# fixstars/cuda-bundle-adjustment

Measured on NVIDIA H100. Metric: LM edges/sec (10 iters), higher is better.
Workload: dtype f64

## Files before the change

### cuda-bundle-adjustment_b200/binding.py

```python
import ctypes as C
import dataclasses
import os

import numpy as np

HERE = os.path.dirname(os.path.abspath(__file__))
ROBUST_NONE, ROBUST_HUBER, ROBUST_TUKEY = 0, 1, 2
EDGE_MONOCULAR, EDGE_STEREO = 0, 1
PROFILE_ITEMS = ("0: Initialize Optimizer", "1: Build Structure", "2: Compute Error", "3: Build System",
                 "4: Schur Complement", "5: Symbolic Decomposition", "6: Numerical Decomposition", "7: Update Solution")


PCG_INFO_LEN = 16
PCG_INFO_FIELDS = ("kernel", "two_level", "aggs_per_cta", "G", "gs", "A", "maxRows", "capBlocks", "zhInSmem", "coarse_kernel",
                   "cinfo", "status", "iters", "coarse_rebuilds", "bj_retries", "bad_rebuilds")
PCG_KERNELS = ("none", "k_pcg", "k_pcg2", "k_pcg3", "k_pcg4", "k_pcg5", "k_pcg5_big", "k_pcg5t")
COARSE_KERNELS = ("none", "k_coarse_invert", "cluster2<8>", "cluster2<16>", "k_coarse_dense", "k_coarse_chol_cluster")


class CubaError(RuntimeError):
    pass


def library_path():
    return os.path.join(HERE, "libcuba_b200.so")


class _Config(C.Structure):
    _fields_ = [("device", C.c_int), ("use_fp32", C.c_int), ("pcg_max_iters", C.c_int), ("pcg_tol", C.c_double),
                ("deterministic", C.c_int), ("reserved", C.c_int * 7)]


class _Problem(C.Structure):
    _fields_ = [("Pall", C.c_int32), ("numP", C.c_int32), ("Lall", C.c_int32), ("numL", C.c_int32),
                ("q", C.c_void_p), ("t", C.c_void_p), ("cam", C.c_void_p), ("Xw", C.c_void_p),
                ("E2", C.c_int32), ("idx2", C.c_void_p), ("meas2", C.c_void_p), ("omega2", C.c_void_p),
                ("E3", C.c_int32), ("idx3", C.c_void_p), ("meas3", C.c_void_p), ("omega3", C.c_void_p)]


class _IterStat(C.Structure):
    _fields_ = [("iteration", C.c_int32), ("trials", C.c_int32), ("chi2", C.c_double), ("lambda_", C.c_double),
                ("pcg_iters", C.c_int32), ("pcg_failed", C.c_int32)]


class _Sizes(C.Structure):
    _fields_ = [(n, C.c_int32) for n in ("Pall", "numP", "Lall", "numL", "E2", "E3", "nhpl", "nblk", "nmul", "nblk_full")]


class _PoseBatch(C.Structure):
    _fields_ = [("B", C.c_int32), ("E2", C.c_int32), ("E3", C.c_int32), ("q", C.c_void_p), ("t", C.c_void_p), ("cam", C.c_void_p),
                ("ptr2", C.c_void_p), ("X2", C.c_void_p), ("meas2", C.c_void_p), ("omega2", C.c_void_p),
                ("ptr3", C.c_void_p), ("X3", C.c_void_p), ("meas3", C.c_void_p), ("omega3", C.c_void_p)]


class _PoseRound(C.Structure):
    _fields_ = [("iterations", C.c_int32), ("kernel_type", C.c_int32 * 2), ("delta", C.c_double * 2), ("restart", C.c_int32),
                ("chi2_mono", C.c_double), ("chi2_stereo", C.c_double), ("flags", C.c_int32)]


POSE_MAX_ROUNDS = 8


@dataclasses.dataclass
class PoseRound:
    iterations: int = 10
    kernel: tuple = (ROBUST_NONE, ROBUST_NONE)
    delta: tuple = (0.0, 0.0)
    restart: bool = True
    chi2_mono: float = 5.991
    chi2_stereo: float = 7.815
    depth: bool = False
    reinclude: bool = True


def orbslam2_pose_schedule():
    huber = dict(kernel=(ROBUST_HUBER, ROBUST_HUBER), delta=(5.991 ** 0.5, 7.815 ** 0.5))
    return [PoseRound(**(huber if r < 2 else {})) for r in range(4)]


class _Sim3Batch(C.Structure):
    _fields_ = [("B", C.c_int32), ("N", C.c_int32), ("ptr", C.c_void_p), ("q", C.c_void_p), ("t", C.c_void_p), ("s", C.c_void_p),
                ("cam1", C.c_void_p), ("cam2", C.c_void_p), ("fix_scale", C.c_void_p), ("X1", C.c_void_p), ("X2", C.c_void_p),
                ("obs1", C.c_void_p), ("obs2", C.c_void_p), ("omega1", C.c_void_p), ("omega2", C.c_void_p)]


class _Sim3Params(C.Structure):
    _fields_ = [("chi2", C.c_double), ("iterations", C.c_int32), ("iterations_bad", C.c_int32), ("iterations_good", C.c_int32),
                ("min_pairs", C.c_int32)]


@dataclasses.dataclass
class Sim3Params:
    chi2: float = 10.0
    iterations: int = 5
    iterations_bad: int = 10
    iterations_good: int = 5
    min_pairs: int = 10


_lib = None

_SYMBOLS = [
    "cuba_last_error", "cuba_version", "cuba_engine_create", "cuba_engine_destroy", "cuba_engine_set_robust_kernel",
    "cuba_comm_unique_id", "cuba_engine_set_comm", "cuba_engine_set_problem", "cuba_engine_set_structure_reuse", "cuba_engine_get_structure_reuses", "cuba_engine_set_state", "cuba_engine_get_sizes", "cuba_engine_reset_state", "cuba_engine_get_stream", "cuba_engine_flush_l2",
    "cuba_engine_optimize", "cuba_engine_get_state", "cuba_engine_get_chi2", "cuba_engine_set_edge_levels", "cuba_engine_get_edge_levels", "cuba_engine_classify_edges", "cuba_engine_optimize_poses", "cuba_engine_optimize_sim3", "cuba_engine_get_profile",
    "cuba_engine_get_launch_count", "cuba_get_transfer_bytes", "cuba_stage_linearize", "cuba_stage_max_diagonal", "cuba_stage_solve", "cuba_stage_update",
    "cuba_stage_commit", "cuba_stage_chi2", "cuba_debug_get_hpl_structure", "cuba_debug_get_hsc_structure",
    "cuba_debug_get_system", "cuba_debug_get_schur", "cuba_debug_get_delta", "cuba_debug_get_pcg_info", "cuba_debug_get_coarse", "cuba_debug_coarse_inverse", "cuba_debug_build_structure_host", "cuba_debug_pcg_partition", "cuba_debug_pcg5_plan", "cuba_debug_pcg5_plan_apc", "cuba_debug_dropin_problem", "cuba_debug_dropin_levels", "cuba_bench_stage",
]


def exported_symbols():
    return list(_SYMBOLS)


def load_library():
    global _lib
    if _lib is not None:
        return _lib
    path = library_path()
    if not os.path.exists(path):
        raise CubaError("%s not built: run `python -c 'import __graft_entry__ as g; g.build()'` (no CPU fallback exists)" % path)
    L = C.CDLL(path)
    L.cuba_last_error.restype = C.c_char_p
    vp, i, d = C.c_void_p, C.c_int, C.c_double
    sig = {
        "cuba_engine_create": [C.POINTER(_Config), C.POINTER(vp)],
        "cuba_engine_destroy": [vp],
        "cuba_engine_set_robust_kernel": [vp, i, i, d],
        "cuba_comm_unique_id": [vp],
        "cuba_engine_set_comm": [vp, i, i, vp],
        "cuba_engine_set_problem": [vp, C.POINTER(_Problem)],
        "cuba_engine_set_structure_reuse": [vp, i],
        "cuba_engine_get_structure_reuses": [vp, C.POINTER(C.c_longlong)],
        "cuba_engine_set_state": [vp, vp, vp, vp],
        "cuba_engine_get_sizes": [vp, C.POINTER(_Sizes)],
        "cuba_engine_reset_state": [vp],
        "cuba_engine_get_stream": [vp, C.POINTER(vp)],
        "cuba_engine_flush_l2": [vp],
        "cuba_engine_optimize": [vp, i, vp, C.POINTER(i)],
        "cuba_engine_get_state": [vp, vp, vp, vp],
        "cuba_engine_get_chi2": [vp, vp],
        "cuba_engine_set_edge_levels": [vp, vp],
        "cuba_engine_get_edge_levels": [vp, vp],
        "cuba_engine_classify_edges": [vp, d, d, i, vp],
        "cuba_engine_optimize_poses": [vp, C.POINTER(_PoseBatch), i, vp, vp, vp, vp, vp, vp, vp],
        "cuba_engine_optimize_sim3": [vp, C.POINTER(_Sim3Batch), C.POINTER(_Sim3Params), vp, vp, vp, vp, vp, vp, vp],
        "cuba_engine_get_profile": [vp, vp],
        "cuba_engine_get_launch_count": [vp, C.POINTER(C.c_longlong)],
        "cuba_get_transfer_bytes": [C.POINTER(C.c_longlong), C.POINTER(C.c_longlong)],
        "cuba_stage_linearize": [vp, C.POINTER(d)],
        "cuba_stage_max_diagonal": [vp, C.POINTER(d)],
        "cuba_stage_solve": [vp, d, C.POINTER(i), C.POINTER(i)],
        "cuba_stage_update": [vp, d, C.POINTER(d), C.POINTER(d)],
        "cuba_stage_commit": [vp, i],
        "cuba_stage_chi2": [vp, C.POINTER(d)],
        "cuba_debug_get_hpl_structure": [vp, vp, vp, vp],
        "cuba_debug_get_hsc_structure": [vp, vp, vp],
        "cuba_debug_get_system": [vp, vp, vp, vp, vp, vp],
        "cuba_debug_get_schur": [vp, vp, vp, vp],
        "cuba_debug_get_delta": [vp, vp, vp],
        "cuba_debug_get_pcg_info": [vp, vp, C.POINTER(d)],
        "cuba_debug_get_coarse": [vp, vp, vp, vp],
        "cuba_debug_coarse_inverse": [vp, vp, i, vp, vp],
        "cuba_debug_build_structure_host": [C.POINTER(_Problem), i, i, C.POINTER(_Sizes), vp, vp, vp, vp, vp, vp, vp, vp],
        "cuba_debug_pcg_partition": [C.POINTER(_Problem), i, i, vp],
        "cuba_debug_pcg5_plan": [C.POINTER(_Problem), i, i, i, vp],
        "cuba_debug_pcg5_plan_apc": [C.POINTER(_Problem), i, i, i, i, vp, C.POINTER(C.c_uint64)],
        "cuba_debug_dropin_problem": [vp, C.POINTER(_Problem)],
        "cuba_debug_dropin_levels": [vp, C.POINTER(C.POINTER(C.c_uint8)), C.POINTER(C.c_int32)],
        "cuba_bench_stage": [vp, i, i, i, d, C.POINTER(d)],
    }
    for name, args in sig.items():
        fn = getattr(L, name)
        fn.argtypes = args
        fn.restype = C.c_int
    _lib = L
    return L


def _check(rc):
    if rc != 0:
        raise CubaError("cuba error %d: %s" % (rc, load_library().cuba_last_error().decode()))


def _p(a):
    return None if a is None else a.ctypes.data_as(C.c_void_p)


def _problem_struct(prob):
    keep = [np.ascontiguousarray(prob.q, dtype=np.float64), np.ascontiguousarray(prob.t, dtype=np.float64),
            np.ascontiguousarray(prob.cam, dtype=np.float64), np.ascontiguousarray(prob.Xw, dtype=np.float64),
            np.ascontiguousarray(prob.idx2, dtype=np.int32), np.ascontiguousarray(prob.meas2, dtype=np.float64),
            np.ascontiguousarray(prob.omega2, dtype=np.float64), np.ascontiguousarray(prob.idx3, dtype=np.int32),
            np.ascontiguousarray(prob.meas3, dtype=np.float64), np.ascontiguousarray(prob.omega3, dtype=np.float64)]
    P = _Problem(prob.Pall, prob.numP, prob.Lall, prob.numL, _p(keep[0]), _p(keep[1]), _p(keep[2]), _p(keep[3]),
                 prob.E2, _p(keep[4]), _p(keep[5]), _p(keep[6]), prob.E3, _p(keep[7]), _p(keep[8]), _p(keep[9]))
    return P, keep


def transfer_bytes():
    a, b = C.c_longlong(0), C.c_longlong(0)
    _check(load_library().cuba_get_transfer_bytes(C.byref(a), C.byref(b)))
    return a.value, b.value


def build_structure_host(prob, rank=0, world=1):
    L = load_library()
    P, keep = _problem_struct(prob)
    sz = _Sizes()
    _check(L.cuba_debug_build_structure_host(C.byref(P), rank, world, C.byref(sz), None, None, None, None, None, None, None, None))
    out = {n: getattr(sz, n) for n, _ in _Sizes._fields_}
    arrs = {"hplColPtr": np.zeros(sz.numL + 1, np.int32), "hplRowInd": np.zeros(sz.nhpl, np.int32),
            "edge2Hpl": np.zeros(sz.E2 + sz.E3, np.int32), "hscRowPtr": np.zeros(sz.numP + 1, np.int32),
            "hscColInd": np.zeros(sz.nblk, np.int32), "fullRowPtr": np.zeros(sz.numP + 1, np.int32),
            "fullColInd": np.zeros(sz.nblk_full, np.int32), "shard": np.zeros(4, np.int32)}
    _check(L.cuba_debug_build_structure_host(C.byref(P), rank, world, C.byref(sz), *[_p(arrs[k]) for k in
           ("hplColPtr", "hplRowInd", "edge2Hpl", "hscRowPtr", "hscColInd", "fullRowPtr", "fullColInd", "shard")]))
    out.update(arrs)
    return out


def pcg_partition_host(prob, n_ctas=148, max_aggregates=74):
    L = load_library()
    P, keep = _problem_struct(prob)
    info = np.zeros(8, np.int32)
    _check(L.cuba_debug_pcg_partition(C.byref(P), int(n_ctas), int(max_aggregates), _p(info)))
    return dict(zip(("G", "gs", "A", "needMax", "maxRows", "blkMax", "maxNeedAgg", "coarse_list_size"), (int(v) for v in info)))


def pcg5_plan_host(prob, world=1, num_sms=148, max_aggregates=74):
    L = load_library()
    P, keep = _problem_struct(prob)
    info = np.zeros(8, np.int32)
    _check(L.cuba_debug_pcg5_plan(C.byref(P), int(world), int(num_sms), int(max_aggregates), _p(info)))
    return dict(zip(("ok", "G", "gs", "A", "needMax", "maxRows", "maxNeedAgg", "halo_rows"), (int(v) for v in info)))


def pcg5_plan_apc_host(prob, aggs_per_cta, world=1, num_sms=132, max_aggregates=148):
    L = load_library()
    P, keep = _problem_struct(prob)
    info = np.zeros(8, np.int32)
    h = C.c_uint64(0)
    _check(L.cuba_debug_pcg5_plan_apc(C.byref(P), int(world), int(num_sms), int(max_aggregates), int(aggs_per_cta), _p(info), C.byref(h)))
    out = dict(zip(("ok", "G", "gs", "A", "needMax", "maxRows", "maxNeedAgg", "halo_rows"), (int(v) for v in info)))
    out["hash"] = int(h.value)
    return out


class Engine:

    def __init__(self, device=-1, use_fp32=False, pcg_max_iters=0, pcg_tol=0.0, pcg_variant=0, structure_on_host=False, jh_variant=0, schur_variant=0,
                 coarse_refresh=0, two_level_switch=0, max_aggregates=0):
        self.L = load_library()
        res = (C.c_int * 7)()
        res[0] = int(pcg_variant)
        res[1] = int(bool(structure_on_host))
        res[2] = int(jh_variant)
        res[3] = int(schur_variant)
        res[4] = int(coarse_refresh)
        res[5] = int(two_level_switch)
        res[6] = int(max_aggregates)
        cfg = _Config(device, 2 if use_fp32 == "mixed" else int(use_fp32), int(pcg_max_iters), float(pcg_tol), 1, res)
        h = C.c_void_p()
        _check(self.L.cuba_engine_create(C.byref(cfg), C.byref(h)))
        self.h = h
        self.sizes = None
        self._stats = []

    def close(self):
        if getattr(self, "h", None):
            self.L.cuba_engine_destroy(self.h)
            self.h = None

    def __del__(self):
        try:
            self.close()
        except Exception:
            pass

    def set_robust_kernels(self, kernel_type, delta, edge_type):
        _check(self.L.cuba_engine_set_robust_kernel(self.h, int(edge_type), int(kernel_type), float(delta)))

    def set_comm(self, rank, world, unique_id=None):
        buf = None if unique_id is None else (C.c_char * 128).from_buffer_copy(bytes(unique_id))
        _check(self.L.cuba_engine_set_comm(self.h, rank, world, buf))

    @staticmethod
    def comm_unique_id():
        buf = (C.c_char * 128)()
        _check(load_library().cuba_comm_unique_id(buf))
        return bytes(buf)

    def initialize(self, prob):
        P, keep = _problem_struct(prob)
        _check(self.L.cuba_engine_set_problem(self.h, C.byref(P)))
        sz = _Sizes()
        _check(self.L.cuba_engine_get_sizes(self.h, C.byref(sz)))
        self.sizes = {n: getattr(sz, n) for n, _ in _Sizes._fields_}
        self._stats = []
        return self.sizes

    def set_structure_reuse(self, enable):
        _check(self.L.cuba_engine_set_structure_reuse(self.h, int(bool(enable))))

    def structure_reuses(self):
        n = C.c_longlong(0)
        _check(self.L.cuba_engine_get_structure_reuses(self.h, C.byref(n)))
        return n.value

    def set_state(self, q, t, Xw):
        q, t, Xw = (np.ascontiguousarray(a, dtype=np.float64) for a in (q, t, Xw))
        _check(self.L.cuba_engine_set_state(self.h, _p(q), _p(t), _p(Xw)))
# ... 58 lines not shown
    @staticmethod
    def _rounds_struct(rounds):
        rs = (_PoseRound * max(len(rounds), 1))()
        for k, r in enumerate(rounds):
            rs[k].iterations = int(r.iterations)
            rs[k].kernel_type[0], rs[k].kernel_type[1] = int(r.kernel[0]), int(r.kernel[1])
            rs[k].delta[0], rs[k].delta[1] = float(r.delta[0]), float(r.delta[1])
            rs[k].restart = int(bool(r.restart))
            rs[k].chi2_mono, rs[k].chi2_stereo = float(r.chi2_mono), float(r.chi2_stereo)
            rs[k].flags = (1 if r.depth else 0) | (2 if r.reinclude else 0)
        return rs

    def optimize_poses_flat(self, q, t, cam, ptr2, X2, meas2, omega2, ptr3, X3, meas3, omega3, rounds, B=None, E2=None, E3=None):
        f64 = lambda a, w: np.ascontiguousarray(np.asarray(a, dtype=np.float64).reshape(-1, w) if w > 1 else np.asarray(a, dtype=np.float64).reshape(-1))
        q, t, cam = f64(q, 4), f64(t, 3), f64(cam, 5)
        X2, meas2, omega2, X3, meas3, omega3 = f64(X2, 3), f64(meas2, 2), f64(omega2, 1), f64(X3, 3), f64(meas3, 3), f64(omega3, 1)
        ptr2 = np.ascontiguousarray(ptr2, dtype=np.int32); ptr3 = np.ascontiguousarray(ptr3, dtype=np.int32)
        B = len(q) if B is None else int(B)
        E2 = len(omega2) if E2 is None else int(E2)
        E3 = len(omega3) if E3 is None else int(E3)
        nb, R = max(B, 0), len(rounds)
        S = sum(max(int(r.iterations), 0) for r in rounds)
        out = dict(q=np.zeros((nb, 4)), t=np.zeros((nb, 3)), levels=np.zeros(max(E2, 0) + max(E3, 0), np.uint8),
                   counts=np.zeros((nb, R, 4), np.int32), stats=(_IterStat * max(nb * S, 1))(), nstats=np.zeros((nb, R), np.int32))
        batch = _PoseBatch(B, E2, E3, _p(q), _p(t), _p(cam), _p(ptr2), _p(X2), _p(meas2), _p(omega2), _p(ptr3), _p(X3), _p(meas3), _p(omega3))
        _check(self.L.cuba_engine_optimize_poses(self.h, C.byref(batch), R, self._rounds_struct(rounds), _p(out["q"]), _p(out["t"]),
                                                 _p(out["levels"]), _p(out["counts"]), out["stats"], _p(out["nstats"])))
        st = np.frombuffer(out["stats"], dtype=np.dtype([("iteration", "<i4"), ("trials", "<i4"), ("chi2", "<f8"), ("lambda_", "<f8"),
                                                          ("pcg_iters", "<i4"), ("pcg_failed", "<i4")]))
        out["stats"] = st[:nb * S].reshape(nb, S).copy()
        return out

    def optimize_poses(self, frames, rounds):
        n2 = np.array([len(f.omega2) for f in frames], np.int64); n3 = np.array([len(f.omega3) for f in frames], np.int64)
        ptr2 = np.concatenate([[0], np.cumsum(n2)]); ptr3 = np.concatenate([[0], np.cumsum(n3)])
        cat = lambda name, w: np.concatenate([np.asarray(getattr(f, name), np.float64).reshape(-1, w) for f in frames]) if frames else np.zeros((0, w))
        r = self.optimize_poses_flat(cat("q", 4), cat("t", 3), cat("cam", 5), ptr2, cat("X2", 3), cat("meas2", 2), cat("omega2", 1).ravel(),
                                     ptr3, cat("X3", 3), cat("meas3", 3), cat("omega3", 1).ravel(), rounds)
        off = np.concatenate([[0], np.cumsum([int(x.iterations) for x in rounds])])
        E2 = int(ptr2[-1])
        res = []
        for b in range(len(frames)):
            stats = []
            for k in range(len(rounds)):
                rows = r["stats"][b, off[k]:off[k] + r["nstats"][b, k]]
                stats.append([dict(iteration=int(s["iteration"]), trials=int(s["trials"]), chi2=float(s["chi2"]), lambda_=float(s["lambda_"]),
                                   pcg_iters=int(s["pcg_iters"]), pcg_failed=int(s["pcg_failed"])) for s in rows])
            res.append(dict(q=r["q"][b], t=r["t"][b], counts=r["counts"][b], stats=stats,
                            levels=np.concatenate([r["levels"][ptr2[b]:ptr2[b + 1]], r["levels"][E2 + ptr3[b]:E2 + ptr3[b + 1]]])))
        return res

    def optimize_sim3_flat(self, ptr, q, t, s, cam1, cam2, fix_scale, X1, X2, obs1, obs2, omega1, omega2, params=None, B=None, N=None):
        params = Sim3Params() if params is None else params
        f64 = lambda a, w: np.ascontiguousarray(np.asarray(a, dtype=np.float64).reshape(-1, w) if w > 1 else np.asarray(a, dtype=np.float64).reshape(-1))
        q, t, s, cam1, cam2 = f64(q, 4), f64(t, 3), f64(s, 1), f64(cam1, 4), f64(cam2, 4)
        X1, X2, obs1, obs2, omega1, omega2 = f64(X1, 3), f64(X2, 3), f64(obs1, 2), f64(obs2, 2), f64(omega1, 1), f64(omega2, 1)
        ptr = np.ascontiguousarray(ptr, dtype=np.int32)
        fix = None if fix_scale is None else np.ascontiguousarray(fix_scale, dtype=np.int32)
        B = len(s) if B is None else int(B)
        N = len(omega1) if N is None else int(N)
        nb = max(B, 0)
        S = max(int(params.iterations), 0) + max(int(params.iterations_bad), int(params.iterations_good), 0)
        out = dict(q=np.zeros((nb, 4)), t=np.zeros((nb, 3)), s=np.zeros(nb), levels=np.zeros(max(N, 0), np.uint8),
                   ninliers=np.zeros(nb, np.int32), stats=(_IterStat * max(nb * S, 1))(), nstats=np.zeros((nb, 2), np.int32))
        batch = _Sim3Batch(B, N, _p(ptr), _p(q), _p(t), _p(s), _p(cam1), _p(cam2), _p(fix), _p(X1), _p(X2), _p(obs1), _p(obs2),
                           _p(omega1), _p(omega2))
        prm = _Sim3Params(float(params.chi2), int(params.iterations), int(params.iterations_bad), int(params.iterations_good),
                          int(params.min_pairs))
        _check(self.L.cuba_engine_optimize_sim3(self.h, C.byref(batch), C.byref(prm), _p(out["q"]), _p(out["t"]), _p(out["s"]),
                                                _p(out["levels"]), _p(out["ninliers"]), out["stats"], _p(out["nstats"])))
        st = np.frombuffer(out["stats"], dtype=np.dtype([("iteration", "<i4"), ("trials", "<i4"), ("chi2", "<f8"), ("lambda_", "<f8"),
                                                          ("pcg_iters", "<i4"), ("pcg_failed", "<i4")]))
        out["stats"] = st[:nb * S].reshape(nb, S).copy()
        return out

    def optimize_sim3(self, problems, params=None):
        params = Sim3Params() if params is None else params
        n = np.array([len(p.omega1) for p in problems], np.int64)
        ptr = np.concatenate([[0], np.cumsum(n)])
        cat = lambda name, w: np.concatenate([np.asarray(getattr(p, name), np.float64).reshape(-1, w) for p in problems]) if problems else np.zeros((0, w))
        r = self.optimize_sim3_flat(ptr, cat("q", 4), cat("t", 3), cat("s", 1).ravel(), cat("cam1", 4), cat("cam2", 4),
                                    np.array([int(bool(p.fix_scale)) for p in problems], np.int32), cat("X1", 3), cat("X2", 3),
                                    cat("obs1", 2), cat("obs2", 2), cat("omega1", 1).ravel(), cat("omega2", 1).ravel(), params)
        off = (0, int(params.iterations))
        res = []
        for b in range(len(problems)):
            stats = []
            for k in range(2):
                rows = r["stats"][b, off[k]:off[k] + r["nstats"][b, k]]
                stats.append([dict(iteration=int(x["iteration"]), trials=int(x["trials"]), chi2=float(x["chi2"]), lambda_=float(x["lambda_"]),
                                   pcg_iters=int(x["pcg_iters"]), pcg_failed=int(x["pcg_failed"])) for x in rows])
            res.append(dict(q=r["q"][b], t=r["t"][b], s=float(r["s"][b]), levels=r["levels"][ptr[b]:ptr[b + 1]].copy(),
                            ninliers=int(r["ninliers"][b]), stats=stats))
        return res

    def launch_count(self):
        n = C.c_longlong(0)
        _check(self.L.cuba_engine_get_launch_count(self.h, C.byref(n)))
        return n.value

    def linearize(self):
        v = C.c_double(0)
        _check(self.L.cuba_stage_linearize(self.h, C.byref(v)))
        return v.value

    def max_diagonal(self):
        v = C.c_double(0)
        _check(self.L.cuba_stage_max_diagonal(self.h, C.byref(v)))
        return v.value

    def solve(self, lam):
        it, ok = C.c_int(0), C.c_int(0)
        _check(self.L.cuba_stage_solve(self.h, float(lam), C.byref(it), C.byref(ok)))
        return it.value, bool(ok.value)

    def update(self, lam):
        chi, sc = C.c_double(0), C.c_double(0)
        _check(self.L.cuba_stage_update(self.h, float(lam), C.byref(chi), C.byref(sc)))
        return chi.value, sc.value

    def commit(self, accept):
        _check(self.L.cuba_stage_commit(self.h, int(bool(accept))))

    def chi2(self):
        v = C.c_double(0)
        _check(self.L.cuba_stage_chi2(self.h, C.byref(v)))
        return v.value

    def hpl_structure(self):
        s = self.sizes
        colPtr = np.zeros(s["numL"] + 1, np.int32); rowInd = np.zeros(s["nhpl"], np.int32); e2h = np.zeros(s["E2"] + s["E3"], np.int32)
        _check(self.L.cuba_debug_get_hpl_structure(self.h, _p(colPtr), _p(rowInd), _p(e2h)))
        return colPtr, rowInd, e2h

    def hsc_structure(self):
        s = self.sizes
        rowPtr = np.zeros(s["numP"] + 1, np.int32); colInd = np.zeros(s["nblk"], np.int32)
        _check(self.L.cuba_debug_get_hsc_structure(self.h, _p(rowPtr), _p(colInd)))
        return rowPtr, colInd

    def system(self):
        s = self.sizes
        Hpp = np.zeros((s["numP"], 36)); bp = np.zeros((s["numP"], 6)); Hll = np.zeros((s["numL"], 9)); bl = np.zeros((s["numL"], 3))
        Hpl = np.zeros((s["nhpl"], 18))
        _check(self.L.cuba_debug_get_system(self.h, _p(Hpp), _p(bp), _p(Hll), _p(bl), _p(Hpl)))
        return Hpp, bp, Hll, bl, Hpl

    def schur(self):
        s = self.sizes
        Hsc = np.zeros((s["nblk"], 36)); bsc = np.zeros((s["numP"], 6)); inv = np.zeros((s["numL"], 9))
        _check(self.L.cuba_debug_get_schur(self.h, _p(Hsc), _p(bsc), _p(inv)))
        return Hsc, bsc, inv

    def delta(self):
        s = self.sizes
        xp = np.zeros((s["numP"], 6)); xl = np.zeros((s["numL"], 3))
        _check(self.L.cuba_debug_get_delta(self.h, _p(xp), _p(xl)))
        return xp, xl

    def pcg_info(self):
        info = np.zeros(PCG_INFO_LEN, np.int32)
        lam = C.c_double(0)
        _check(self.L.cuba_debug_get_pcg_info(self.h, _p(info), C.byref(lam)))
        out = dict(zip(PCG_INFO_FIELDS, (int(v) for v in info)))
        out["kernel"] = PCG_KERNELS[out["kernel"]]
        out["coarse_kernel"] = COARSE_KERNELS[out["coarse_kernel"]]
        out["two_level"] = bool(out["two_level"])
        out["coarse_lambda"] = lam.value
        return out

    def coarse(self):
        A = self.pcg_info()["A"]
        agg = np.zeros(self.sizes["numP"], np.int32); AcP = np.zeros((A * (A + 1) // 2, 36)); AcInv = np.zeros((6 * A, 6 * A), np.float32)
        _check(self.L.cuba_debug_get_coarse(self.h, _p(agg), _p(AcP), _p(AcInv)))
        return agg, AcP, AcInv

    def coarse_inverse(self, AcP):
        AcP = np.ascontiguousarray(AcP, dtype=np.float64)
        nb = AcP.shape[0]
        A = int(round(((8 * nb + 1) ** 0.5 - 1) / 2))
        assert A * (A + 1) // 2 == nb and AcP.shape[1:] == (36,), AcP.shape
        AcInv = np.zeros((6 * A, 6 * A), np.float32)
        info = C.c_int(-1)
        _check(self.L.cuba_debug_coarse_inverse(self.h, _p(AcP), A, _p(AcInv), C.byref(info)))
        return AcInv, info.value

    def bench_stage(self, stage, reps=10, flush_l2=True, lam=1.0):
        ms = C.c_double(0)
        _check(self.L.cuba_bench_stage(self.h, int(stage), int(reps), int(bool(flush_l2)), float(lam), C.byref(ms)))
        return ms.value
```

### cuda-bundle-adjustment_b200/build.py

```python
import os
import subprocess

HERE = os.path.dirname(os.path.abspath(__file__))
CSRC = os.path.join(HERE, "csrc")
LIB = os.path.join(HERE, "libcuba_b200.so")
SOURCES = ["cuba_engine.cu", "cuba_structure.cpp", "cuba_api.cpp"]
HEADERS = ["cuba_kernels.cuh", "cuba_jh4.cuh", "cuba_levels.cuh", "cuba_pose_batch.cuh", "cuba_sim3_batch.cuh", "cuba_schur3.cuh", "cuba_schur5.cuh", "cuba_pcg2.cuh", "cuba_pcg3.cuh", "cuba_pcg4.cuh", "cuba_pcg5.cuh", "cuba_pcg5t.cuh", "cuba_coarse_dense.cuh", "cuba_peer_reduce.cuh", "cuba_schur2.cuh", "cuba_structure_gpu.cuh", "cuba_math.cuh", "cuba_structure.h",
           "../../include/cuba_b200.h", "../../include/cuba_b200_levels.h", "../../include/cuba_b200_pose.h", "../../include/cuba_b200_sim3.h", "../../include/cuda_bundle_adjustment.h", "../../include/cuda_bundle_adjustment_types.h"]
NVCC = os.environ.get("NVCC", "/usr/local/cuda/bin/nvcc")
FLAGS = (["-DCUBA_JH4_DEBUG"] if os.environ.get("CUBA_JH4_DEBUG") else []) + ["-O3", "-std=c++17", "-gencode", "arch=compute_90a,code=sm_90a", "-lineinfo",
         "-Xcompiler", "-fPIC,-Wall,-Wno-unused-function", "-shared"]


def needs_build():
    if not os.path.exists(LIB):
        return True
    t = os.path.getmtime(LIB)
    deps = [os.path.join(CSRC, s) for s in SOURCES + HEADERS]
    return any(os.path.exists(d) and os.path.getmtime(d) > t for d in deps)


def build(force=False, verbose=False):
    if not force and not needs_build():
        return LIB
    srcs = [os.path.join(CSRC, s) for s in SOURCES if os.path.exists(os.path.join(CSRC, s))]
    cmd = [NVCC] + FLAGS + (["-Xptxas", "-v"] if verbose else []) + ["-I", os.path.join(HERE, "..", "include"), "-o", LIB] + srcs + ["-ldl"]
    res = subprocess.run(cmd, capture_output=True, text=True)
    if res.returncode != 0:
        raise RuntimeError("nvcc failed:\n" + res.stdout + res.stderr)
    if verbose:
        print(res.stdout + res.stderr)
    return LIB


if __name__ == "__main__":
    import sys
    print(build(force=True, verbose="-v" in sys.argv))
```

### cuda-bundle-adjustment_b200/csrc/cuba_engine.cu

```cuda
#include <cuda_runtime.h>
#include <dlfcn.h>

#include <algorithm>
#include <chrono>
#include <cmath>
#include <cstdio>
#include <cstring>
#include <memory>
#include <string>
#include <vector>

#include "../../include/cuba_b200.h"
#include "cuba_kernels.cuh"
#include "cuba_pcg2.cuh"
#include "cuba_pcg3.cuh"
#include "cuba_pcg4.cuh"
#include "cuba_pcg5.cuh"
#include "cuba_pcg5t.cuh"
#include "cuba_coarse_dense.cuh"
#include "cuba_peer_reduce.cuh"
#include "cuba_schur2.cuh"
#include "cuba_jh4.cuh"
#include "cuba_levels.cuh"
#include "cuba_pose_batch.cuh"
#include "cuba_sim3_batch.cuh"
#include "cuba_schur3.cuh"
#include "cuba_schur5.cuh"
#include "cuba_structure.h"
#include "cuba_structure_gpu.cuh"

namespace cuba_b200 {

static thread_local std::string g_err;
static int fail(int code, const std::string& msg) { g_err = msg; return code; }

#define CUDA_TRY(expr)                                                                                      \
	do {                                                                                                    \
		cudaError_t _e = (expr);                                                                            \
		if (_e != cudaSuccess) {                                                                            \
			char _b[512];                                                                                   \
			snprintf(_b, sizeof(_b), "%s:%d: %s -> %s", __FILE__, __LINE__, #expr, cudaGetErrorString(_e)); \
			return fail(CUBA_ERR_CUDA, _b);                                                                 \
		}                                                                                                   \
	} while (0)

#define KLAUNCH(kernel, n, ...)                                                             \
	do {                                                                                     \
		if ((n) > 0) {                                                                       \
			kernel<<<sgpu::grid_for(n), sgpu::BLK, 0, stream>>>(__VA_ARGS__);                 \
			launches++;                                                                      \
			CUDA_TRY(cudaGetLastError());                                                    \
		}                                                                                    \
	} while (0)

static thread_local long long g_h2dBytes = 0, g_d2hBytes = 0;

struct PinnedArena {
	char* p = nullptr; size_t cap = 0, off = 0;
	~PinnedArena() { if (p) cudaFreeHost(p); }
	void reset() { off = 0; }
	void* put(const void* src, size_t bytes)
	{
		const size_t o = (off + 255) & ~(size_t)255;
		if (o + bytes > cap) {
			if (off != 0) return nullptr;
			if (p) cudaFreeHost(p);
			cap = std::max<size_t>(2 * (o + bytes), (size_t)1 << 20);
			if (cudaMallocHost((void**)&p, cap) != cudaSuccess) { p = nullptr; cap = 0; return nullptr; }
		}
		memcpy(p + o, src, bytes);
		off = o + bytes;
		return p + o;
	}
};

struct PinnedBuf {
	char* p = nullptr; size_t cap = 0;
	PinnedBuf() {}
	PinnedBuf(const PinnedBuf&) = delete;
	PinnedBuf& operator=(const PinnedBuf&) = delete;
	~PinnedBuf() { if (p) cudaFreeHost(p); }
	cudaError_t grow(size_t bytes)
	{
		if (p && bytes <= cap) return cudaSuccess;
		if (p) cudaFreeHost(p);
		p = nullptr; cap = 0;
		const cudaError_t e = cudaMallocHost((void**)&p, std::max<size_t>(bytes, 256));
		if (e == cudaSuccess) cap = std::max<size_t>(bytes, 256);
		else p = nullptr;
		return e;
	}
};

template <typename U>
struct DBuf {
	U* p = nullptr; size_t n = 0, cap = 0;
	bool view = false;
	DBuf() {}
	DBuf(const DBuf&) = delete;
	DBuf& operator=(const DBuf&) = delete;
	~DBuf() { release(); }
	void release() { if (p && !view) cudaFree(p); p = nullptr; n = 0; cap = 0; view = false; }
	void alias(U* q, size_t count) { release(); p = q; n = count; cap = count; view = true; }
	cudaError_t alloc(size_t count)
	{
		if (p && count <= cap && !view) { n = count; return cudaSuccess; }
		release();
		n = count; cap = count ? count : 1;
		return cudaMalloc((void**)&p, sizeof(U) * cap);
	}
	cudaError_t upload(const U* h, size_t count, cudaStream_t s)
	{
		cudaError_t e = alloc(count);
		if (e != cudaSuccess || !count) return e;
		g_h2dBytes += (long long)(sizeof(U) * count);
		return cudaMemcpyAsync(p, h, sizeof(U) * count, cudaMemcpyHostToDevice, s);
	}
	cudaError_t upload(const std::vector<U>& h, cudaStream_t s) { return upload(h.data(), h.size(), s); }
	cudaError_t upload(const std::vector<U>& h, cudaStream_t s, PinnedArena& arena)
	{
		const void* src = h.empty() ? nullptr : arena.put(h.data(), sizeof(U) * h.size());
		return upload(src ? (const U*)src : h.data(), h.size(), s);
	}
	operator U*() const { return p; }
};

struct Nccl {
	void* lib = nullptr;
	typedef struct { char internal[128]; } UniqueId;
	int (*GetUniqueId)(UniqueId*) = nullptr;
	int (*CommInitRank)(void**, int, UniqueId, int) = nullptr;
	int (*CommDestroy)(void*) = nullptr;
	int (*AllReduce)(const void*, void*, size_t, int, int, void*, cudaStream_t) = nullptr;
	int (*AllGather)(const void*, void*, size_t, int, void*, cudaStream_t) = nullptr;
	int (*Broadcast)(const void*, void*, size_t, int, int, void*, cudaStream_t) = nullptr;
	int (*GroupStart)() = nullptr;
	int (*GroupEnd)() = nullptr;
	const char* (*GetErrorString)(int) = nullptr;
	bool load(std::string& why)
	{
		if (lib) return true;
		const char* names[] = { "libnccl.so.2", "libnccl.so" };
		for (const char* nme : names) { lib = dlopen(nme, RTLD_NOW | RTLD_GLOBAL); if (lib) break; }
		if (!lib) { why = std::string("dlopen libnccl.so.2 failed: ") + dlerror(); return false; }
		GetUniqueId = (int (*)(UniqueId*))dlsym(lib, "ncclGetUniqueId");
		CommInitRank = (int (*)(void**, int, UniqueId, int))dlsym(lib, "ncclCommInitRank");
		CommDestroy = (int (*)(void*))dlsym(lib, "ncclCommDestroy");
		AllReduce = (int (*)(const void*, void*, size_t, int, int, void*, cudaStream_t))dlsym(lib, "ncclAllReduce");
		AllGather = (int (*)(const void*, void*, size_t, int, void*, cudaStream_t))dlsym(lib, "ncclAllGather");
		Broadcast = (int (*)(const void*, void*, size_t, int, int, void*, cudaStream_t))dlsym(lib, "ncclBroadcast");
		GroupStart = (int (*)())dlsym(lib, "ncclGroupStart");
		GroupEnd = (int (*)())dlsym(lib, "ncclGroupEnd");
		GetErrorString = (const char* (*)(int))dlsym(lib, "ncclGetErrorString");
		if (!GetUniqueId || !CommInitRank || !CommDestroy || !AllReduce || !AllGather || !Broadcast || !GroupStart || !GroupEnd) { why = "libnccl lacks expected symbols"; return false; }
		return true;
	}
};
static Nccl g_nccl;
enum { NCCL_INT8 = 0, NCCL_FLOAT32 = 7, NCCL_FLOAT64 = 8, NCCL_SUM = 0, NCCL_MAX = 2 };

struct Scalars { double v[8]; unsigned long long maxdiag; PcgStatus pcg; };

struct DevGuard {
	int prev = -1, dev;
	explicit DevGuard(int d) : dev(d) { if (cudaGetDevice(&prev) != cudaSuccess) prev = -1; if (prev != dev) cudaSetDevice(dev); }
	~DevGuard() { if (prev >= 0 && prev != dev) cudaSetDevice(prev); }
};

struct EngineBase {
	virtual ~EngineBase() {}
	cuba_config cfg{};
	int rk_type[2] = { 0, 0 };
	double rk_delta[2] = { 0, 0 };
	int rank = 0, world = 1;
	bool structureReuse = true;
	long long structureReuses = 0;
	int devOrdinal = 0;
	void* comm = nullptr;
	bool haveProblem = false;
	long long launches = 0;
	double prof[CUBA_PROF_NUM] = { 0 };

	virtual int set_problem(const cuba_problem* p) = 0;
	virtual int set_state(const double* q, const double* t, const double* Xw) = 0;
	virtual int get_sizes(cuba_sizes* out) const = 0;
	virtual int reset_state() = 0;
	virtual int get_stream(void** s) = 0;
	virtual int flush_l2() = 0;
	virtual int optimize(int niter, cuba_iter_stat* stats, int* nstats) = 0;
	virtual int get_state(double* q, double* t, double* Xw) = 0;
	virtual int get_chi2(double* out) = 0;
	virtual int get_profile(double* sec) = 0;
	virtual int stage_linearize(double* chi) = 0;
	virtual int stage_max_diagonal(double* md) = 0;
	virtual int stage_solve(double lambda, int* iters, int* ok) = 0;
	virtual int stage_update(double lambda, double* chi, double* scale) = 0;
	virtual int stage_commit(int accept) = 0;
	virtual int stage_chi2(double* chi) = 0;
	virtual int dbg_hpl_structure(int32_t* colPtr, int32_t* rowInd, int32_t* e2h) = 0;
	virtual int dbg_hsc_structure(int32_t* rowPtr, int32_t* colInd) = 0;
	virtual int dbg_system(double* Hpp, double* bp, double* Hll, double* bl, double* Hpl) = 0;
	virtual int dbg_schur(double* Hsc, double* bsc, double* invHll) = 0;
	virtual int dbg_delta(double* xp, double* xl) = 0;
	virtual int bench_stage(int stage, int reps, int flush, double lambda, double* ms) = 0;
	virtual int dbg_pcg_timing(long long* out, int maxCtas) = 0;
	virtual int dbg_pcg_info(int32_t* info, double* coarseLambda) = 0;
	virtual int dbg_coarse(int32_t* rowAgg, double* AcP, float* AcInv) = 0;
	virtual int dbg_coarse_inverse(const double* AcP, int A, float* AcInv, int* info) = 0;
	virtual int set_edge_levels(const uint8_t* levels) = 0;
	virtual int get_edge_levels(uint8_t* levels) = 0;
	virtual int classify_edges(double chi2Mono, double chi2Stereo, int flags, int32_t* counts) = 0;
	virtual int optimize_poses(const cuba_pose_batch* bt, const pb::Schedule& s, double* qOut, double* tOut, uint8_t* levelsOut,
		int32_t* counts, cuba_iter_stat* stats, int32_t* nstats) = 0;
	virtual int optimize_sim3(const cuba_sim3_batch* bt, const s3::Params& p, double* qOut, double* tOut, double* sOut, uint8_t* levelsOut,
		int32_t* ninliers, cuba_iter_stat* stats, int32_t* nstats) = 0;
};

template <typename T>
struct Engine : EngineBase {
	Structure S;
	cudaStream_t stream = nullptr;
	int numSMs = 0;
	int ntiles = 0, nPoseBlocks = 0, nChiBlocks = 0;
	int tileSize = TILE;
	int jhMinBlocks = 2;
	bool jhV2 = true;
	bool jhV3 = true;
	int jh3Grid = 0, nChiLin = 0;
	bool jhV4 = true;
	int ntW = 0, jh4Grid = 0, jh4HasBig = 0, jh4MinB = 4, jh4Nst = 2;
	const void* jh4AttrSet = nullptr;
	int* jh4Host = nullptr;
	bool jh4Pending = false;
	DBuf<int> w_levels, w_start, w_pieces, w_base, w_tilePose, w_tilePieces, w_pieceCount, w_flag;
	DBuf<jh4::WTile> w_tile;
	DBuf<jh4::Rec> w_rec;
	DBuf<double> w_bigPartial;
	DBuf<TileInfo> tileInfo;
	bool useSchur2 = true;
	bool useSchur5 = false;
	int s5Ntiles = 0;
	DBuf<int> s5TileLm;
	DBuf<TileInfo> s5TileInfo;
	DBuf<int4> s5SegRec;
	DBuf<unsigned int> s5Off;
	int s2Nseg = 0, s2Nvalid = 0;
	DBuf<unsigned long long> s2_key, s2_keyS, s2_key3, s2_key3S;
	DBuf<int> s2_val, s2_valS, s2_head, s2_segId, s2_segStart, s2_segTile, s2_segDest, s2_val3, s2_val3S, s2_segRank, s2_rankDest, s2_tileSegPtr, s2_destSegPtr, s2_p2i, s2_p2j;
	DBuf<schur2::Counts> s2_counts;
	DBuf<T> s2_partial;
	DBuf<int> tilePose0, tilePoseN;
	int cur = 0;
	bool trialValid = false;
	DBuf<T> pose[2], Xw[2], cam, pose0, Xw0;
	DBuf<T> e_mx, e_my, e_mz, e_om, p_mx, p_my, p_mz, p_om;
	DBuf<int> tilePtr;
	DBuf<int> e_ip, e_il, e_hpl, e_user, lmPtr, tileLm, hplLm, posePtr, p_il;
	DBuf<T> Hpp, bp, Hll, bl, Hpl, invHll, fVal, bsc, xp, xl;
	DBuf<T> uVal;
	DBuf<float> HplF;
	bool mixed = false;
	bool upperReduce = false;
	DBuf<int> prodPtr, prodI, prodJ, prodL, blkRow, blkCol, u2f, u2fT, fRowPtr, fColInd;
	bool useSchur3 = true;
	DBuf<T> pr, pz, pq, pp0, pp1, Minv;
	DBuf<double> pcgPartial;
	int pcgGrid = 0;
	DBuf<T> fHat, Linv, vR0, vR1, vS0, vS1, vW0, vW1, vP, vY;
	DBuf<int> fLocal, ctaRow, needPtr, needCol;
	DBuf<double> pcg2Partial;
	DBuf<GridBar> gridBar;
	DBuf<long long> pcgTiming;
	DBuf<unsigned long long> llFlags;
	int pcg2Grid = 0, pcg2Cap = 0, pcg2NeedMax = 0, pcg2MaxRows = 0;
	DBuf<T> cZx, cZhat;
	DBuf<float> cAcInv;
	DBuf<double> cAcP, cPart, cU, cLp, cLd, cWp;
	DBuf<int> cAggRow, cNaPtr, cNaList, cNeedAgg, cInfo, cRowOf, cCbPtr, cCbList;
	int pcg4A = 0, pcg4Gs = 1, pcg4MaxNeedAgg = 0, pcg4Cap = 0, pcg4SliceInSmem = 0, pcg4ZhInSmem = 0;
	size_t pcg4Smem = 0, pcg4InvSmem = 0;
	bool pcg4Ok = false, tlActive = false, pcg4Cluster = false;
	PinnedArena arena;
	bool coarseValid = false;
	int coarseAge = 0;
	double coarseLambda = 0, curLambda = 0;
	bool pcg3Ok = false;
	size_t pcg2Smem = 0;
	DBuf<double> chiPartial, scalePartialL, scalePartialP, chiSq;
	bool lvOn = false;
	long long lvIncluded = 0;
	DBuf<T> e_om0;
	DBuf<unsigned char> lvLevel;
	DBuf<int> lvPartial;
	DBuf<double> lvCount;
	DBuf<double> pbIn, pbOut;
	PinnedBuf pbHostIn, pbHostOut;
	DBuf<double> s3In, s3Out;
	PinnedBuf s3HostIn, s3HostOut;
	DBuf<Scalars> dScal;
	Scalars* hScal = nullptr;
	DBuf<double> flushBuf;
	std::vector<std::pair<int, std::pair<cudaEvent_t, cudaEvent_t>>> profEvents;
	std::vector<cudaEvent_t> eventPool;

	~Engine() override
	{
		DevGuard guard(devOrdinal);
		if (stream) cudaStreamSynchronize(stream);
		p5CloseMappings(); uCloseMappings();
		for (auto& pe : profEvents) { cudaEventDestroy(pe.second.first); cudaEventDestroy(pe.second.second); }
		for (auto ev : eventPool) cudaEventDestroy(ev);
		if (hScal) cudaFreeHost(hScal);
		if (hMeta) cudaFreeHost(hMeta);
		if (jh4Host) cudaFreeHost(jh4Host);
		if (stream) cudaStreamDestroy(stream);
		if (comm && g_nccl.CommDestroy) g_nccl.CommDestroy(comm);
	}

	int init()
	{
		int ndev = 0;
		cudaError_t e = cudaGetDeviceCount(&ndev);
		if (e != cudaSuccess || ndev <= 0)
			return fail(CUBA_ERR_CUDA, std::string("no CUDA device available (") + cudaGetErrorString(e) + "); this library has no CPU fallback");
		if (cfg.device >= 0) CUDA_TRY(cudaSetDevice(cfg.device));
		int dev = 0;
		CUDA_TRY(cudaGetDevice(&dev));
		devOrdinal = dev;
		CUDA_TRY(cudaDeviceGetAttribute(&numSMs, cudaDevAttrMultiProcessorCount, dev));
		CUDA_TRY(cudaStreamCreateWithFlags(&stream, cudaStreamNonBlocking));
		CUDA_TRY(cudaMallocHost((void**)&hScal, sizeof(Scalars)));
		memset(hScal, 0, sizeof(Scalars));
		CUDA_TRY(dScal.alloc(1));
		CUDA_TRY(cudaMemsetAsync(dScal.p, 0, sizeof(Scalars), stream));
		return CUBA_OK;
	}

	cudaEvent_t newEvent()
	{
		cudaEvent_t ev;
		if (!eventPool.empty()) { ev = eventPool.back(); eventPool.pop_back(); return ev; }
		cudaEventCreate(&ev);
		return ev;
	}
	struct ProfScope {
		Engine* e; int item; cudaEvent_t a, b;
		ProfScope(Engine* e_, int item_) : e(e_), item(item_) { a = e->newEvent(); b = e->newEvent(); cudaEventRecord(a, e->stream); }
		~ProfScope() { cudaEventRecord(b, e->stream); e->profEvents.push_back({ item, { a, b } }); }
	};
	void resolveProfile()
	{
		cudaStreamSynchronize(stream);
		for (auto& pe : profEvents) {
			float ms = 0;
			if (cudaEventElapsedTime(&ms, pe.second.first, pe.second.second) == cudaSuccess) prof[pe.first] += 1e-3 * ms;
			eventPool.push_back(pe.second.first); eventPool.push_back(pe.second.second);
		}
		profEvents.clear();
	}

	RobustParams rkParams() const
	{
		RobustParams r;
		for (int i = 0; i < 2; i++) { r.type[i] = rk_type[i]; r.delta[i] = rk_delta[i]; }
		return r;
	}

	int allreduce(void* buf, size_t count, bool isT)
	{
		if (world <= 1 || !comm) return CUBA_OK;
		const int dt = isT ? (sizeof(T) == 8 ? NCCL_FLOAT64 : NCCL_FLOAT32) : NCCL_FLOAT64;
		const int rc = g_nccl.AllReduce(buf, buf, count, dt, NCCL_SUM, comm, stream);
		if (rc != 0) return fail(CUBA_ERR_COMM, std::string("ncclAllReduce failed: ") + (g_nccl.GetErrorString ? g_nccl.GetErrorString(rc) : "?"));
		return CUBA_OK;
	}

	DBuf<double> rawQ, rawT, rawC, rawX;
	int upload_state(const double* q, const double* t, const double* c, const double* X)
	{
		const int Pall = S.Pall, Lall = S.Lall;
		CUDA_TRY(rawQ.upload(q, 4 * (size_t)Pall, stream)); CUDA_TRY(rawT.upload(t, 3 * (size_t)Pall, stream));
		CUDA_TRY(rawX.upload(X, 3 * (size_t)Lall, stream));
		if (c) CUDA_TRY(rawC.upload(c, 5 * (size_t)Pall, stream));
		CUDA_TRY(pose0.alloc(8 * (size_t)Pall)); CUDA_TRY(Xw0.alloc(4 * (size_t)Lall));
		for (int b = 0; b < 2; b++) { CUDA_TRY(pose[b].alloc(8 * (size_t)Pall)); CUDA_TRY(Xw[b].alloc(4 * (size_t)Lall)); }
		if (c) CUDA_TRY(cam.alloc(8 * (size_t)Pall));
		const int n = std::max(Pall, Lall);
		if (n > 0) {
			k_pack_state<T><<<(n + 255) / 256, 256, 0, stream>>>(rawQ.p, rawT.p, c ? rawC.p : nullptr, rawX.p, Pall, Lall,
				pose0.p, pose[0].p, pose[1].p, c ? cam.p : nullptr, Xw0.p, Xw[0].p, Xw[1].p);
			launches++;
			CUDA_TRY(cudaGetLastError());
		}
		return CUBA_OK;
	}

	std::vector<std::pair<const char*, std::chrono::steady_clock::time_point>> marks;
	void tmark(const char* name) { if (markOn) marks.push_back({ name, std::chrono::steady_clock::now() }); }
	bool markOn = false;
	int set_problem(const cuba_problem* p) override
	{
		markOn = getenv("CUBA_SETUP_TIMING") != nullptr; marks.clear(); tmark("start");
		if (!p) return fail(CUBA_ERR_INVALID, "set_problem: null problem");
		if (p->Pall < 0 || p->Lall < 0 || p->numP < 0 || p->numL < 0 || p->numP > p->Pall || p->numL > p->Lall || p->E2 < 0 || p->E3 < 0)
			return fail(CUBA_ERR_INVALID, "set_problem: invalid sizes");
		if ((p->Pall > 0 && (!p->q || !p->t || !p->cam)) || (p->Lall > 0 && !p->Xw) || (p->E2 > 0 && (!p->idx2 || !p->meas2 || !p->omega2)) ||
			(p->E3 > 0 && (!p->idx3 || !p->meas3 || !p->omega3)))
			return fail(CUBA_ERR_INVALID, "set_problem: null array with a non-zero count");
		const auto t0 = std::chrono::steady_clock::now();
		lastPcgKernel = CUBA_PCG_KERNEL_NONE; p5Rebuilds = 0; bjRetries = 0;
		lvOn = false;
		if (structureReuse && reusable && haveProblem && cfg.reserved[1] != 1 && same_topology(p)) {
			int rc = refresh_values(p); if (rc) return rc;
			structureReuses++;
			prof[CUBA_PROF_BUILD_STRUCTURE] += std::chrono::duration<double>(std::chrono::steady_clock::now() - t0).count();
			return CUBA_OK;
		}
// ... 161 lines not shown
	int build_on_gpu(const cuba_problem* p)
	{
		using namespace sgpu;
		S = Structure();
		const int Pall = p->Pall, numP = p->numP, Lall = p->Lall, numL = p->numL, E2 = p->E2, E3 = p->E3, E = E2 + E3;
		S.Pall = Pall; S.numP = numP; S.Lall = Lall; S.numL = numL; S.E2 = E2; S.E3 = E3; S.E = E;
		CUDA_TRY(g_idx2.upload(p->idx2, 2 * (size_t)E2, stream)); CUDA_TRY(g_idx3.upload(p->idx3, 2 * (size_t)E3, stream));
		CUDA_TRY(g_meas2.upload(p->meas2, 2 * (size_t)E2, stream)); CUDA_TRY(g_meas3.upload(p->meas3, 3 * (size_t)E3, stream));
		CUDA_TRY(g_om2.upload(p->omega2, (size_t)E2, stream)); CUDA_TRY(g_om3.upload(p->omega3, (size_t)E3, stream));
		CUDA_TRY(g_meta.alloc(1));
		CUDA_TRY(cudaMemsetAsync(g_meta.p, 0, sizeof(Meta), stream));
		CUDA_TRY(g_key.alloc(E)); CUDA_TRY(g_keyS.alloc(E)); CUDA_TRY(g_val.alloc(E)); CUDA_TRY(g_valS.alloc(E));
		KLAUNCH(k_make_keys, E, E2, g_idx2.p, E3, g_idx3.p, Pall, numP, Lall, numL, g_key.p, g_val.p, g_meta.p);
		int rc = sortPairs(g_key.p, g_keyS.p, g_val.p, g_valS.p, E, 32 + bits_for((unsigned long long)std::max(Lall, 1))); if (rc) return rc;
		CUDA_TRY(g_lmPtrG.alloc((size_t)Lall + 1));
		KLAUNCH(k_ptr_from_high, Lall + 1, g_keyS.p, E, Lall, g_lmPtrG.p);
		KLAUNCH(k_check_nonempty, numL, g_lmPtrG.p, numL, g_meta.p);
		CUDA_TRY(g_ff.alloc(E)); CUDA_TRY(g_hplG.alloc(E));
		KLAUNCH(k_flag_freefree, E, g_keyS.p, E, numP, numL, g_ff.p);
		rc = exclusiveSum(g_ff.p, g_hplG.p, E); if (rc) return rc;
		k_shard_meta<<<1, 32, 0, stream>>>(g_lmPtrG.p, Lall, E, rank, world, g_ff.p, g_hplG.p, g_meta.p);
		launches++;
		CUDA_TRY(cudaGetLastError());
		tmark("queued to sync 1");
		rc = fetchMeta(); if (rc) return rc;
		tmark("sync 1");
		S.nhpl = hMeta->nhpl; S.lmBeg = hMeta->lmBeg; S.lmEnd = hMeta->lmEnd; S.eLocal = hMeta->kEnd - hMeta->kBeg;
		S.hplBase = hMeta->hplBase; S.nhplLocal = hMeta->hplEnd - hMeta->hplBase;
		for (int r = 0; r < 9; r++) shardBound[r] = hMeta->bounds[r];
		shardBoundValid = true;
		const int kBeg = hMeta->kBeg, kEnd = hMeta->kEnd, eL = S.eLocal, nhpl = S.nhpl;
		savedKBeg = kBeg;
		CUDA_TRY(g_hplRowInd.alloc(nhpl)); CUDA_TRY(g_hplLmG.alloc(nhpl)); CUDA_TRY(g_edge2Hpl.alloc(E)); CUDA_TRY(g_hplColPtr.alloc((size_t)numL + 1));
		KLAUNCH(k_hpl_global, E, g_keyS.p, g_valS.p, g_ff.p, g_hplG.p, E, g_hplRowInd.p, g_hplLmG.p, g_edge2Hpl.p);
		KLAUNCH(k_hpl_colptr, numL + 1, g_lmPtrG.p, g_hplG.p, E, numL, nhpl, g_hplColPtr.p);
		CUDA_TRY(e_user.alloc(eL)); CUDA_TRY(e_ip.alloc(eL)); CUDA_TRY(e_il.alloc(eL)); CUDA_TRY(e_hpl.alloc(eL));
		CUDA_TRY(e_mx.alloc(eL)); CUDA_TRY(e_my.alloc(eL)); CUDA_TRY(e_mz.alloc(eL)); CUDA_TRY(e_om.alloc(eL));
		KLAUNCH(k_edge_stream<T>, eL, g_keyS.p, g_valS.p, g_ff.p, g_hplG.p, kBeg, eL, S.hplBase, E2, g_meas2.p, g_om2.p, g_meas3.p, g_om3.p,
			e_user.p, e_ip.p, e_il.p, e_hpl.p, e_mx.p, e_my.p, e_mz.p, e_om.p);
		CUDA_TRY(lmPtr.alloc((size_t)Lall + 1));
		KLAUNCH(k_local_lmptr, Lall + 1, g_lmPtrG.p, Lall, kBeg, kEnd, lmPtr.p);
		CUDA_TRY(hplLm.alloc(S.nhplLocal));
		if (S.nhplLocal > 0) CUDA_TRY(cudaMemcpyAsync(hplLm.p, g_hplLmG.p + S.hplBase, sizeof(int) * (size_t)S.nhplLocal, cudaMemcpyDeviceToDevice, stream));
		CUDA_TRY(tilePtr.alloc((size_t)numL + 2));
		KLAUNCH(k_tile_ptr, numL + 2, lmPtr.p, numL, eL, tilePtr.p);
		const int tb = std::min(S.lmBeg, numL), te = std::min(S.lmEnd, numL) + (S.lmEnd > numL ? 1 : 0);
		const int window = tileSize == 128 ? JH3_WINDOW : tileSize - 16;
		const int nt = (eL + window - 1) / window;
		CUDA_TRY(tileLm.alloc((size_t)nt + 1));
		KLAUNCH(k_tiles, nt + 1, tilePtr.p, tb, te, window, nt, tileLm.p);
		ntiles = nt;
		CUDA_TRY(g_k32.alloc(eL)); CUDA_TRY(g_k32S.alloc(eL)); CUDA_TRY(g_pval.alloc(eL)); CUDA_TRY(g_psrc.alloc(eL));
		KLAUNCH(k_pose_keys, eL, e_ip.p, eL, numP, g_k32.p, g_pval.p);
		rc = sortPairs(g_k32.p, g_k32S.p, g_pval.p, g_psrc.p, eL, bits_for((unsigned long long)numP)); if (rc) return rc;
		CUDA_TRY(posePtr.alloc((size_t)numP + 1));
		KLAUNCH(k_ptr_from_u32, numP + 1, g_k32S.p, eL, numP, posePtr.p);
		CUDA_TRY(p_il.alloc(eL)); CUDA_TRY(p_mx.alloc(eL)); CUDA_TRY(p_my.alloc(eL)); CUDA_TRY(p_mz.alloc(eL)); CUDA_TRY(p_om.alloc(eL));
		KLAUNCH(k_pose_stream<T>, eL, g_psrc.p, posePtr.p, numP, eL, e_ip.p, e_il.p, e_mx.p, e_my.p, e_mz.p, e_om.p, p_il.p, p_mx.p, p_my.p, p_mz.p, p_om.p);
		CUDA_TRY(g_cnt.alloc((size_t)nhpl + 1)); CUDA_TRY(g_off.alloc((size_t)nhpl + 1));
		CUDA_TRY(cudaMemsetAsync(g_cnt.p, 0, sizeof(int) * ((size_t)nhpl + 1), stream));
		KLAUNCH(k_prod_count, nhpl, g_hplLmG.p, g_hplColPtr.p, nhpl, g_cnt.p);
		rc = exclusiveSum(g_cnt.p, g_off.p, nhpl + 1); if (rc) return rc;
		long long nmul = 0;
		{
			int last = 0;
			CUDA_TRY(cudaMemcpyAsync(&last, g_off.p + nhpl, sizeof(int), cudaMemcpyDeviceToHost, stream));
			tmark("queued to sync 2");
			CUDA_TRY(cudaStreamSynchronize(stream));
			tmark("sync 2");
			nmul = last;
		}
		S.nmul = nmul;
		const long long N = nmul + numP;
		if (N > 0x7fffffffLL) return fail(CUBA_ERR_INVALID, "build_structure: more than 2^31 block products");
		S.nmulLocal = N;
		CUDA_TRY(g_pkey.alloc((size_t)N)); CUDA_TRY(g_pkeyS.alloc((size_t)N)); CUDA_TRY(g_pkeyVal.alloc((size_t)N)); CUDA_TRY(g_pvalS.alloc((size_t)N));
		CUDA_TRY(g_pi.alloc((size_t)N)); CUDA_TRY(g_pj.alloc((size_t)N));
		KLAUNCH(k_prod_emit, nhpl, g_hplLmG.p, g_hplColPtr.p, g_hplRowInd.p, g_off.p, nhpl, S.lmBeg, S.lmEnd, S.hplBase, g_pkey.p, g_pkeyVal.p, g_pi.p, g_pj.p);
		KLAUNCH(k_prod_diag, numP, numP, nmul, g_pkey.p, g_pkeyVal.p, g_pi.p, g_pj.p);
		rc = sortPairs(g_pkey.p, g_pkeyS.p, g_pkeyVal.p, g_pvalS.p, (int)N, 32 + bits_for((unsigned long long)std::max(numP, 1))); if (rc) return rc;
		CUDA_TRY(g_head.alloc((size_t)N + 1)); CUDA_TRY(g_blkId.alloc((size_t)N + 1));
		KLAUNCH(k_heads, N, g_pkeyS.p, (int)N, g_head.p);
		rc = exclusiveSum(g_head.p, g_blkId.p, (int)N); if (rc) return rc;
		k_nblk<<<1, 32, 0, stream>>>(g_head.p, g_blkId.p, (int)N, g_meta.p);
		launches++;
		tmark("queued to sync 3");
		rc = fetchMeta(); if (rc) return rc;
		tmark("sync 3");
		const int nblk = hMeta->nblk;
		S.nblk = nblk;
		CUDA_TRY(blkRow.alloc(nblk)); CUDA_TRY(blkCol.alloc(nblk)); CUDA_TRY(prodPtr.alloc((size_t)nblk + 1));
		CUDA_TRY(prodI.alloc((size_t)N)); CUDA_TRY(prodJ.alloc((size_t)N));
		KLAUNCH(k_blocks, N + 1, g_pkeyS.p, g_pvalS.p, g_head.p, g_blkId.p, g_pi.p, g_pj.p, (int)N, blkRow.p, blkCol.p, prodPtr.p, prodI.p, prodJ.p);
		CUDA_TRY(g_hscRowPtr.alloc((size_t)numP + 1));
		KLAUNCH(k_rowptr_from_rows, numP + 1, blkRow.p, nblk, numP, g_hscRowPtr.p);
		int* dLocalCount = nullptr;
		if (world > 1) {
			CUDA_TRY(g_head.alloc((size_t)N + 1)); CUDA_TRY(g_blkId.alloc((size_t)N + 1));
			KLAUNCH(k_local_flag, N + 1, prodI.p, prodJ.p, (int)N, g_head.p);
			rc = exclusiveSum(g_head.p, g_blkId.p, (int)N + 1); if (rc) return rc;
			KLAUNCH(k_compact_products, N, prodI.p, prodJ.p, g_head.p, g_blkId.p, (int)N, g_pi.p, g_pj.p);
			KLAUNCH(k_remap_ptr, nblk + 1, g_blkId.p, nblk, prodPtr.p);
			CUDA_TRY(cudaMemcpyAsync(prodI.p, g_pi.p, sizeof(int) * (size_t)N, cudaMemcpyDeviceToDevice, stream));
			CUDA_TRY(cudaMemcpyAsync(prodJ.p, g_pj.p, sizeof(int) * (size_t)N, cudaMemcpyDeviceToDevice, stream));
			dLocalCount = g_blkId.p + N;
		}
		const int nfull = 2 * nblk - numP;
		S.nfull = nfull;
		CUDA_TRY(g_fkey.alloc(2 * (size_t)nblk)); CUDA_TRY(g_fkeyS.alloc(2 * (size_t)nblk)); CUDA_TRY(g_fval.alloc(2 * (size_t)nblk)); CUDA_TRY(g_fvalS.alloc(2 * (size_t)nblk));
		KLAUNCH(k_full_entries, nblk, blkRow.p, blkCol.p, nblk, numP, g_fkey.p, g_fval.p);
		rc = sortPairs(g_fkey.p, g_fkeyS.p, g_fval.p, g_fvalS.p, 2 * nblk, 32 + bits_for((unsigned long long)std::max(numP, 1))); if (rc) return rc;
		CUDA_TRY(fColInd.alloc(nfull)); CUDA_TRY(u2f.alloc(nblk)); CUDA_TRY(u2fT.alloc(nblk)); CUDA_TRY(fRowPtr.alloc((size_t)numP + 1));
		KLAUNCH(k_full_finish, nfull, g_fkeyS.p, g_fvalS.p, nfull, blkRow.p, blkCol.p, fColInd.p, u2f.p, u2fT.p);
		KLAUNCH(k_ptr_from_high, numP + 1, g_fkeyS.p, nfull, numP, fRowPtr.p);
		S.fRowPtr.resize((size_t)numP + 1); S.fColInd.resize(nfull);
		g_d2hBytes += (long long)(sizeof(int) * ((size_t)numP + 1 + nfull));
		CUDA_TRY(cudaMemcpyAsync(S.fRowPtr.data(), fRowPtr.p, sizeof(int) * ((size_t)numP + 1), cudaMemcpyDeviceToHost, stream));
		if (nfull > 0) CUDA_TRY(cudaMemcpyAsync(S.fColInd.data(), fColInd.p, sizeof(int) * (size_t)nfull, cudaMemcpyDeviceToHost, stream));
		int localCount = (int)N;
		if (dLocalCount) CUDA_TRY(cudaMemcpyAsync(&localCount, dLocalCount, sizeof(int), cudaMemcpyDeviceToHost, stream));
		tmark("queued to sync 4");
		CUDA_TRY(cudaStreamSynchronize(stream));
		tmark("sync 4");
		S.nmulLocal = localCount;
		return CUBA_OK;
	}

	int ensureHostStructure()
	{
		if (hostStructureValid) return CUBA_OK;
		auto dl = [&](std::vector<int>& dst, const int* src, size_t n) -> cudaError_t {
			dst.resize(n);
			return n ? cudaMemcpyAsync(dst.data(), src, sizeof(int) * n, cudaMemcpyDeviceToHost, stream) : cudaSuccess;
		};
		CUDA_TRY(dl(S.hplColPtr, g_hplColPtr.p, (size_t)S.numL + 1)); CUDA_TRY(dl(S.hplRowInd, g_hplRowInd.p, S.nhpl));
		CUDA_TRY(dl(S.edge2Hpl, g_edge2Hpl.p, S.E)); CUDA_TRY(dl(S.hscRowPtr, g_hscRowPtr.p, (size_t)S.numP + 1));
		CUDA_TRY(dl(S.hscColInd, blkCol.p, S.nblk)); CUDA_TRY(dl(S.u2f, u2f.p, S.nblk)); CUDA_TRY(dl(S.u2fT, u2fT.p, S.nblk));
		CUDA_TRY(cudaStreamSynchronize(stream));
		hostStructureValid = true;
		return CUBA_OK;
	}

	int alloc_system()
	{
		const int eL = S.eLocal;
		const size_t nP = S.numP, nL = S.numL;
		CUDA_TRY(Hpp.alloc(42 * nP + 2)); bp.alias(Hpp.p + 36 * nP, 6 * nP);
		CUDA_TRY(Hll.alloc(9 * nL)); CUDA_TRY(bl.alloc(3 * nL));
		mixed = cfg.use_fp32 == 2 && sizeof(T) == 8 && jhV4;
		if (mixed) { CUDA_TRY(HplF.alloc(20 * (size_t)std::max(S.nhplLocal, 1))); CUDA_TRY(Hpl.alloc(1)); }
		else CUDA_TRY(Hpl.alloc(18 * (size_t)S.nhplLocal));
		CUDA_TRY(invHll.alloc(9 * nL));
		CUDA_TRY(fVal.alloc(36 * (size_t)S.nfull + 6 * nP)); bsc.alias(fVal.p + 36 * (size_t)S.nfull, 6 * nP);
		upperReduce = world > 1 && (cfg.reserved[3] == 0 || cfg.reserved[3] == 3 || cfg.use_fp32 == 2) && S.numP > 0 && S.numL > 0;
		if (upperReduce) {
			uCount = 36 * (size_t)S.nblk + 6 * nP;
			const size_t need = ((uCount + 1) & ~(size_t)1) + 64;
			if (!uVal.p || need > uVal.cap) {
				if (uMappedFor) { CUDA_TRY(cudaStreamSynchronize(stream)); uCloseMappings(); }
				CUDA_TRY(uVal.alloc(std::max(need, (size_t)1 << 18)));
				CUDA_TRY(cudaMemsetAsync(uVal.p, 0, sizeof(T) * uVal.cap, stream));
				uEpoch = 0;
			}
			bsc.alias(uVal.p + 36 * (size_t)S.nblk, 6 * nP);
			uPeerOk = false;
			if (!getenv("CUBA_NCCL_HSC") && comm) {
				CUDA_TRY(cudaMemsetAsync(uVal.p + ((uCount + 1) & ~(size_t)1), 0, sizeof(T) * 64, stream));
				uEpoch = 0;
				int rcx = allreduce(&dScal.p->v[7], 1, false); if (rcx) return rcx;
				bool ok = false;
				rcx = ipcExchange((void*)uVal.p, uPeerBase, uMappedFor, ok); if (rcx) return rcx;
				uPeerOk = ok;
				CUDA_TRY(gridBar.alloc(1));
			}
		}
		CUDA_TRY(xp.alloc(6 * nP)); CUDA_TRY(xl.alloc(3 * nL));
		CUDA_TRY(pr.alloc(6 * nP)); CUDA_TRY(pz.alloc(6 * nP)); CUDA_TRY(pq.alloc(6 * nP)); CUDA_TRY(pp0.alloc(6 * nP)); CUDA_TRY(pp1.alloc(6 * nP));
		CUDA_TRY(Minv.alloc(36 * nP));
		if (nL) CUDA_TRY(cudaMemsetAsync(Hll.p, 0, sizeof(T) * 9 * nL, stream));
		if (nL) CUDA_TRY(cudaMemsetAsync(bl.p, 0, sizeof(T) * 3 * nL, stream));
		if (nL) CUDA_TRY(cudaMemsetAsync(xl.p, 0, sizeof(T) * 3 * nL, stream));
		if (nP) CUDA_TRY(cudaMemsetAsync(xp.p, 0, sizeof(T) * 6 * nP, stream));
		if (nP) CUDA_TRY(cudaMemsetAsync(Hpp.p, 0, sizeof(T) * 36 * nP, stream));
		if (nP) CUDA_TRY(cudaMemsetAsync(bp.p, 0, sizeof(T) * 6 * nP, stream));
		CUDA_TRY(tilePose0.alloc((size_t)std::max(ntiles, 1))); CUDA_TRY(tilePoseN.alloc((size_t)std::max(ntiles, 1)));
		if (ntiles > 0) {
			k_tile_info<<<ntiles, 128, 0, stream>>>(tilePtr.p, tileLm.p, e_ip.p, ntiles, tilePose0.p, tilePoseN.p);
			launches++;
			CUDA_TRY(cudaGetLastError());
			CUDA_TRY(tileInfo.alloc((size_t)ntiles));
			k_tile_info3<<<ntiles, 128, 0, stream>>>(tilePtr.p, tileLm.p, e_ip.p, e_hpl.p, S.eLocal, S.nhplLocal, ntiles, tileInfo.p);
			launches++;
			CUDA_TRY(cudaGetLastError());
		}
		CUDA_TRY(cudaFuncSetAttribute(k_linearize_landmark3, cudaFuncAttributeMaxDynamicSharedMemorySize, (int)sizeof(Jh3Smem)));
		jh3Grid = std::max(1, std::min(ntiles, numSMs * 4));
		useSchur2 = cfg.reserved[3] == 2 && S.numP > 0 && S.numL > 0 && ntiles > 0;
		useSchur5 = cfg.reserved[3] == 5 && cfg.reserved[1] != 1 && sizeof(T) == 8 && S.numP > 0 && S.numL > 0 && ntiles > 0 && S.eLocal > 0;
		useSchur3 = cfg.reserved[3] == 0 || cfg.reserved[3] == 3 || cfg.reserved[3] == 4 || cfg.use_fp32 == 2;
		if (cfg.use_fp32 == 2) { useSchur2 = false; useSchur5 = false; }
		if (useSchur3 && S.nmulLocal > 0) {
			CUDA_TRY(prodL.alloc((size_t)S.nmulLocal));
			KLAUNCH(schur3::k_prod_landmark, S.nmulLocal, prodI.p, hplLm.p, (int)S.nmulLocal, prodL.p);
		}
		if (useSchur5) {
			const int tb5 = std::min(S.lmBeg, S.numL), te5 = std::min(S.lmEnd, S.numL) + (S.lmEnd > S.numL ? 1 : 0);
			s5Ntiles = (S.eLocal + schur5::WINDOW - 1) / schur5::WINDOW;
			CUDA_TRY(s5TileLm.alloc((size_t)s5Ntiles + 1)); CUDA_TRY(s5TileInfo.alloc((size_t)s5Ntiles));
			KLAUNCH(sgpu::k_tiles, s5Ntiles + 1, tilePtr.p, tb5, te5, schur5::WINDOW, s5Ntiles, s5TileLm.p);
			k_tile_info3<<<s5Ntiles, 128, 0, stream>>>(tilePtr.p, s5TileLm.p, e_ip.p, e_hpl.p, S.eLocal, S.nhplLocal, s5Ntiles, s5TileInfo.p);
			launches++;
			CUDA_TRY(cudaGetLastError());
			int rc = setup_schur2(s5TileInfo.p, s5Ntiles); if (rc) return rc;
			if (useSchur5) {
				CUDA_TRY(s5SegRec.alloc((size_t)std::max(s2Nseg, 1)));
				KLAUNCH(schur5::k_seg_records, s2Nseg, s2_segStart.p, s2_segDest.p, s2_segRank.p, s2_segTile.p, blkRow.p, blkCol.p, s5TileInfo.p, s2_p2i.p, s2_p2j.p, s2Nseg, s5SegRec.p);
				CUDA_TRY(s5Off.alloc((size_t)std::max(s2Nvalid, 1)));
				KLAUNCH(schur5::k_prod_offsets, s2Nvalid, s2_segStart.p, s2_segTile.p, s5TileInfo.p, s2_p2i.p, s2_p2j.p, s2Nseg, s2Nvalid, s5Off.p);
				CUDA_TRY(cudaFuncSetAttribute(schur5::k_schur_tiles_mma, cudaFuncAttributeMaxDynamicSharedMemorySize, (int)sizeof(schur5::Smem)));
			}
		}
		else if (useSchur2) { int rc = setup_schur2(tileInfo.p, ntiles); if (rc) return rc; }
		tmark("alloc + tile info queued");
		if (jhV4) { int rc = setup_jh4(); if (rc) return rc; }
		tmark("jh4 queued");
		if (S.numP > 0) { int rc = setup_pcg2(); if (rc) return rc; }
		if (S.numP > 0 && S.numL > 0) { int rc = setup_pcg5(); if (rc) return rc; }
		tmark("pcg partition (host)");
		if (jhV4) { int rc = setup_jh4_finish(); if (rc) return rc; }
		tmark("jh4 finish");
		nChiLin = jhV4 ? jh4Grid : (jhV3 ? jh3Grid : ntiles);
		nPoseBlocks = (S.numP + RED_BLOCK - 1) / RED_BLOCK;
		nChiBlocks = std::max(1, std::min((eL + RED_BLOCK - 1) / RED_BLOCK, numSMs * 8));
		CUDA_TRY(chiPartial.alloc((size_t)std::max(std::max(ntiles, nChiBlocks), jh4Grid) + 1));
		CUDA_TRY(scalePartialL.alloc((size_t)std::max(ntiles, (S.numL + RED_BLOCK - 1) / RED_BLOCK) + 1));
		CUDA_TRY(scalePartialP.alloc((size_t)nPoseBlocks + 1));
		CUDA_TRY(chiSq.alloc((size_t)S.E));
		{
			int perSM = 0;
			CUDA_TRY(cudaOccupancyMaxActiveBlocksPerMultiprocessor(&perSM, k_pcg<T>, PCG_BLOCK, 0));
			if (perSM < 1) return fail(CUBA_ERR_CUDA, "k_pcg cannot be resident");
			const int wantWarps = std::max(1, S.numP);
			const int wantBlocks = (wantWarps + PCG_BLOCK / 32 - 1) / (PCG_BLOCK / 32);
			pcgGrid = std::max(1, std::min(wantBlocks, numSMs * std::min(perSM, 2)));
			CUDA_TRY(pcgPartial.alloc(2 * (size_t)pcgGrid));
		}
		return CUBA_OK;
	}

	int set_state(const double* q, const double* t, const double* X) override
	{
		if (!haveProblem) return fail(CUBA_ERR_STATE, "set_state before set_problem");
		const int rc = upload_state(q, t, nullptr, X); if (rc) return rc;
		CUDA_TRY(cudaStreamSynchronize(stream));
		trialValid = false;
		return CUBA_OK;
	}

	int reset_state() override
	{
		if (!haveProblem) return fail(CUBA_ERR_STATE, "reset_state before set_problem");
		for (int b = 0; b < 2; b++) {
			CUDA_TRY(cudaMemcpyAsync(pose[b].p, pose0.p, sizeof(T) * 8 * (size_t)S.Pall, cudaMemcpyDeviceToDevice, stream));
			CUDA_TRY(cudaMemcpyAsync(Xw[b].p, Xw0.p, sizeof(T) * 4 * (size_t)S.Lall, cudaMemcpyDeviceToDevice, stream));
		}
		trialValid = false;
		return CUBA_OK;
	}
	int get_stream(void** s) override { *s = (void*)stream; return CUBA_OK; }
	int flush_l2() override
	{
		const size_t flushN = (size_t)40 << 20;
		CUDA_TRY(flushBuf.alloc(flushN));
		k_fill<<<numSMs * 8, 256, 0, stream>>>(flushBuf.p, flushN, 1.0);
		launches++;
		CUDA_TRY(cudaGetLastError());
		return CUBA_OK;
	}

	int get_sizes(cuba_sizes* o) const override
	{
		if (!haveProblem) return fail(CUBA_ERR_STATE, "get_sizes before set_problem");
		o->Pall = S.Pall; o->numP = S.numP; o->Lall = S.Lall; o->numL = S.numL; o->E2 = S.E2; o->E3 = S.E3;
		o->nhpl = S.nhpl; o->nblk = S.nblk; o->nmul = (int32_t)S.nmul; o->nblk_full = S.nfull;
		return CUBA_OK;
	}

	ChiArgs<T> chiArgs(int buf)
	{
		ChiArgs<T> a;
		a.pose = pose[buf]; a.cam = cam; a.Xw = Xw[buf];
		a.mx = e_mx; a.my = e_my; a.mz = e_mz; a.om = e_om; a.ip = e_ip; a.il = e_il;
		a.E = S.eLocal; a.rk = rkParams(); a.chiPartial = chiPartial;
		return a;
	}

	int launch_linearize_landmark()
	{
		if (ntiles <= 0) return CUBA_OK;
		LinLmArgs<T> a;
		a.pose = pose[cur]; a.cam = cam; a.Xw = Xw[cur];
		a.mx = e_mx; a.my = e_my; a.mz = e_mz; a.om = e_om; a.ip = e_ip; a.il = e_il; a.hpl = e_hpl;
		a.lmPtr = tilePtr; a.tileLm = tileLm; a.numP = S.numP; a.numL = S.numL;
		a.Hpl = Hpl; a.Hll = Hll; a.bl = bl; a.chiPartial = chiPartial; a.rk = rkParams();
		if (jhV4) {
			if constexpr (sizeof(T) == 8) {
				if (ntW <= 0) return CUBA_OK;
				jh4::Args b;
				b.pose = pose[cur]; b.cam = cam; b.Xw = Xw[cur];
				b.rec = w_rec; b.tile = w_tile; b.tilePose = w_tilePose; b.tilePieces = w_tilePieces; b.pieceCount = w_pieceCount; b.ntiles = ntW; b.numL = S.numL;
				b.Hpl = Hpl; b.HplF = mixed ? HplF.p : nullptr; b.Hll = Hll; b.bl = bl; b.bigPartial = w_bigPartial; b.chiPartial = chiPartial; b.rk = rkParams();
				const void* fn = nullptr; size_t smem = 0;
#define JH4_PICK(MB, NS, DB) { fn = (const void*)jh4::k_linearize_landmark4<MB, NS, DB>; smem = (size_t)NS * jh4::WARPS * sizeof(jh4::StageOf<MB, NS>); }
				int dbg = 0;
#ifdef CUBA_JH4_DEBUG
				dbg = getenv("CUBA_JH4_DBG") ? atoi(getenv("CUBA_JH4_DBG")) : 0;
				if (jh4Nst == 3) { switch (dbg) { case 1: JH4_PICK(4, 3, 1) break; case 2: JH4_PICK(4, 3, 2) break; case 4: JH4_PICK(4, 3, 4) break; case 6: JH4_PICK(4, 3, 6) break;
					case 7: JH4_PICK(4, 3, 7) break; case 8: JH4_PICK(4, 3, 8) break; case 15: JH4_PICK(4, 3, 15) break; default: dbg = 0; } }
				else { switch (dbg) { case 8: JH4_PICK(5, 2, 8) break; case 7: JH4_PICK(5, 2, 7) break; default: dbg = 0; } }
#endif
				if (mixed) { fn = (const void*)jh4::k_linearize_landmark4<4, 2, 0, true>; smem = (size_t)2 * jh4::WARPS * sizeof(jh4::StageOf<4, 2>); }
				if (!fn) {
					if (jh4Nst == 3) JH4_PICK(4, 3, 0)
					else if (jh4MinB == 4) JH4_PICK(4, 2, 0)
					else if (jh4MinB == 5) JH4_PICK(5, 2, 0)
					else JH4_PICK(6, 2, 0)
				}
				if (fn != jh4AttrSet) { CUDA_TRY(cudaFuncSetAttribute(fn, cudaFuncAttributeMaxDynamicSharedMemorySize, (int)smem)); jh4AttrSet = fn; }
				void* kargs[] = { (void*)&b };
				CUDA_TRY(cudaLaunchKernel(fn, dim3(jh4Grid), dim3(jh4::WARPS * 32), kargs, smem, stream));
#ifdef CUBA_JH4_DEBUG
				if (dbg & 8) {
					const int nw = jh4Grid * jh4::WARPS;
					std::vector<double> h(11 * (size_t)nw);
					cudaMemcpyAsync(h.data(), w_bigPartial.p, sizeof(double) * h.size(), cudaMemcpyDeviceToHost, stream);
					cudaStreamSynchronize(stream);
					double acc[8] = { 0 };
					for (int w = 0; w < nw; w++) for (int i = 0; i < 8; i++) acc[i] += h[8 * (size_t)w + i];
					static int once = 0;
					if (once++ == 3) {
						const char* nm[8] = { "cpasync_wait", "mbar_wait", "lds_inputs", "math+hpl_staging", "fence+bulk_store", "wait_read+issue", "reduce+stores", "rotate(descr)" };
						double tot = 0; for (int i = 0; i < 8; i++) tot += acc[i];
						for (int i = 0; i < 8; i++) fprintf(stderr, "jh4 phase %-18s %9.0f cycles/warp  %5.1f %%\n", nm[i], acc[i] / nw, 100 * acc[i] / tot);
						fprintf(stderr, "jh4 total %9.0f cycles/warp, %d warps, %d tiles\n", tot / nw, nw, ntW);
						double s0 = 1e300, s1 = 0, l0 = 1e300, l1 = 0, e0 = 1e300, e1 = 0;
						for (int w = 0; w < nw; w++) {
							const double* g = h.data() + 8 * (size_t)nw + 3 * (size_t)w;
							s0 = std::min(s0, g[0]); s1 = std::max(s1, g[0]); l0 = std::min(l0, g[1]); l1 = std::max(l1, g[1]); e0 = std::min(e0, g[2]); e1 = std::max(e1, g[2]);
						}
						fprintf(stderr, "jh4 globaltimer (ns, rel. first start): start %.0f..%.0f  loop entry %.0f..%.0f  loop exit %.0f..%.0f\n", 0.0, s1 - s0, l0 - s0, l1 - s0, e0 - s0, e1 - s0);
					}
				}
#endif
			}
		}
		else if (jhV3) {
			if constexpr (sizeof(T) == 8) {
				LinLm3Args b;
				b.base = a; b.info = tileInfo; b.ntiles = ntiles;
				k_linearize_landmark3<<<jh3Grid, JH3_TL, sizeof(Jh3Smem), stream>>>(b);
			}
		}
		else if (jhV2) {
			LinLm2Args<T> b;
			b.base = a; b.tilePose0 = tilePose0; b.tilePoseN = tilePoseN; b.eLocal = S.eLocal; b.nhplLocal = S.nhplLocal;
			k_linearize_landmark2<T><<<ntiles, JH2_TL, 0, stream>>>(b);
		}
		else if (tileSize == 128 && jhMinBlocks >= 6) k_linearize_landmark<T, 128, 6><<<ntiles, 128, 0, stream>>>(a);
		else if (tileSize == 128) k_linearize_landmark<T, 128, 4><<<ntiles, 128, 0, stream>>>(a);
		else if (jhMinBlocks >= 3) k_linearize_landmark<T, 256, 3><<<ntiles, 256, 0, stream>>>(a);
		else k_linearize_landmark<T, 256, 2><<<ntiles, 256, 0, stream>>>(a);
		launches++;
		CUDA_TRY(cudaGetLastError());
		return CUBA_OK;
	}
	int launch_linearize_pose()
	{
		if (S.numP <= 0) return CUBA_OK;
		LinPoseArgs<T> a;
		a.pose = pose[cur]; a.cam = cam; a.Xw = Xw[cur];
		a.mx = p_mx; a.my = p_my; a.mz = p_mz; a.om = p_om; a.il = p_il; a.posePtr = posePtr;
		a.Hpp = Hpp; a.bp = bp; a.rk = rkParams();
		k_linearize_pose<T><<<S.numP, POSE_BLOCK, 0, stream>>>(a);
		launches++;
		CUDA_TRY(cudaGetLastError());
		return CUBA_OK;
	}
	int launch_sum(const double* p0, int n0, const double* p1, int n1, const double* p2, int n2, int slot)
	{
		k_sum_partials<<<1, RED_BLOCK, 0, stream>>>(p0, n0, p1, n1, p2, n2, &dScal.p->v[slot]);
		launches++;
		CUDA_TRY(cudaGetLastError());
		return CUBA_OK;
	}
	int fetchScalars()
	{
		g_d2hBytes += (long long)sizeof(Scalars);
		CUDA_TRY(cudaMemcpyAsync(hScal, dScal.p, sizeof(Scalars), cudaMemcpyDeviceToHost, stream));
		CUDA_TRY(cudaStreamSynchronize(stream));
		return CUBA_OK;
	}

	int stage_linearize(double* chi) override
	{
		if (!haveProblem) return fail(CUBA_ERR_STATE, "linearize before set_problem");
		{
			ProfScope ps(this, CUBA_PROF_BUILD_SYSTEM);
			int rc = launch_linearize_landmark(); if (rc) return rc;
			rc = launch_linearize_pose(); if (rc) return rc;
			rc = launch_sum(chiPartial, ntiles > 0 ? nChiLin : 0, nullptr, 0, nullptr, 0, 0); if (rc) return rc;
			if (world > 1) {
				if constexpr (sizeof(T) == 8) {
					T* slot = Hpp.p + 42 * (size_t)S.numP;
					CUDA_TRY(cudaMemcpyAsync(slot, &dScal.p->v[0], sizeof(double), cudaMemcpyDeviceToDevice, stream));
					rc = allreduce(Hpp.p, 42 * (size_t)S.numP + 1, true); if (rc) return rc;
					CUDA_TRY(cudaMemcpyAsync(&dScal.p->v[0], slot, sizeof(double), cudaMemcpyDeviceToDevice, stream));
				} else {
					if (S.numP > 0) { rc = allreduce(Hpp.p, 42 * (size_t)S.numP, true); if (rc) return rc; }
					rc = allreduce(&dScal.p->v[0], 1, false); if (rc) return rc;
				}
			}
		}
		int rc = fetchScalars(); if (rc) return rc;
		if (chi) *chi = hScal->v[0];
		return CUBA_OK;
	}

	int stage_chi2(double* chi) override
	{
		if (!haveProblem) return fail(CUBA_ERR_STATE, "chi2 before set_problem");
		int rc = launch_chi2(cur, 0); if (rc) return rc;
		rc = fetchScalars(); if (rc) return rc;
		if (chi) *chi = hScal->v[0];
		return CUBA_OK;
	}

	int launch_chi2(int buf, int slot, bool reduce = true)
	{
		ProfScope ps(this, CUBA_PROF_COMPUTE_ERROR);
		if (S.eLocal > 0) {
			k_chi2<T><<<nChiBlocks, RED_BLOCK, 0, stream>>>(chiArgs(buf));
			launches++;
			CUDA_TRY(cudaGetLastError());
		}
		int rc = launch_sum(chiPartial, S.eLocal > 0 ? nChiBlocks : 0, nullptr, 0, nullptr, 0, slot); if (rc) return rc;
		if (world > 1 && reduce) { rc = allreduce(&dScal.p->v[slot], 1, false); if (rc) return rc; }
		return CUBA_OK;
	}

	int stage_max_diagonal(double* md) override
	{
		if (!haveProblem) return fail(CUBA_ERR_STATE, "max_diagonal before set_problem");
		CUDA_TRY(cudaMemsetAsync(&dScal.p->maxdiag, 0, sizeof(unsigned long long), stream));
		const int n = S.numP * 6 + S.numL * 3;
		if (n > 0) {
			const int grid = std::max(1, std::min((n + 255) / 256, numSMs * 4));
			k_max_diagonal<T><<<grid, 256, 0, stream>>>(Hpp, S.numP, Hll, S.numL, &dScal.p->maxdiag);
			launches++;
			CUDA_TRY(cudaGetLastError());
		}
		if (world > 1) {
			const int rcn = comm ? g_nccl.AllReduce(&dScal.p->maxdiag, &dScal.p->maxdiag, 1, NCCL_FLOAT64, NCCL_MAX, comm, stream) : 0;
			if (rcn != 0) return fail(CUBA_ERR_COMM, "ncclAllReduce(max) failed");
		}
		int rc = fetchScalars(); if (rc) return rc;
		double m;
		memcpy(&m, &hScal->maxdiag, sizeof(double));
		if (md) *md = m;
		return CUBA_OK;
	}

	int launch_schur(T lambda)
	{
		ProfScope ps(this, CUBA_PROF_SCHUR_COMPLEMENT);
		if (useSchur2 || useSchur5) {
			schur2::TileArgs<T> ta;
			ta.Hpl = Hpl; ta.Hll = Hll; ta.bl = bl; ta.info = tileInfo; ta.hplLm = hplLm;
			ta.tileSegPtr = s2_tileSegPtr; ta.segStart = s2_segStart; ta.segDest = s2_segDest; ta.segRank = s2_segRank; ta.p2i = s2_p2i; ta.p2j = s2_p2j;
			ta.blkRow = blkRow; ta.blkCol = blkCol; ta.numL = S.numL; ta.lambda = lambda; ta.invHll = invHll; ta.partial = s2_partial;
			if (useSchur5) {
				if constexpr (sizeof(T) == 8) {
					schur5::Args sa;
					sa.Hpl = Hpl; sa.Hll = Hll; sa.bl = bl; sa.info = s5TileInfo; sa.hplLm = hplLm; sa.tileSegPtr = s2_tileSegPtr; sa.segRec = s5SegRec; sa.off = s5Off;
					sa.p2i = s2_p2i; sa.p2j = s2_p2j; sa.numL = S.numL; sa.lambda = lambda; sa.invHll = invHll; sa.partial = s2_partial;
					schur5::k_schur_tiles_mma<<<s5Ntiles, schur5::WARPS * 32, sizeof(schur5::Smem), stream>>>(sa);
				}
			}
			else schur2::k_schur_tiles<T><<<ntiles, schur2::TL, 0, stream>>>(ta);
			launches++;
			CUDA_TRY(cudaGetLastError());
			schur2::ReduceArgs<T> ra;
			ra.partial = s2_partial; ra.destSegPtr = s2_destSegPtr; ra.Hpp = Hpp; ra.bp = bp;
			ra.blkRow = blkRow; ra.blkCol = blkCol; ra.u2f = u2f; ra.u2fT = u2fT; ra.nblk = S.nblk; ra.lambda = lambda;
			ra.addDiag = rank == 0 ? 1 : 0; ra.fVal = fVal; ra.bsc = bsc;
			schur2::k_schur_reduce<T><<<(S.nblk + 3) / 4, 128, 0, stream>>>(ra);
			launches++;
			CUDA_TRY(cudaGetLastError());
			if (world > 1) {
				int rc = allreduce(fVal.p, 36 * (size_t)S.nfull + 6 * (size_t)S.numP, true); if (rc) return rc;
			}
			return CUBA_OK;
		}
		{
			const int l0 = std::min(S.lmBeg, S.numL), l1 = std::min(S.lmEnd, S.numL);
			if (l1 > l0) {
				k_inv_hll<T><<<(l1 - l0 + 255) / 256, 256, 0, stream>>>(Hll.p + 9 * (size_t)l0, l1 - l0, lambda, invHll.p + 9 * (size_t)l0);
				launches++;
				CUDA_TRY(cudaGetLastError());
			}
		}
		if (useSchur3 && S.numP > 0 && S.numL > 0) {
			schur3::Args<T> a;
			a.Hpl = Hpl; a.invHll = invHll; a.bl = bl; a.Hpp = Hpp; a.bp = bp;
			a.prodPtr = prodPtr; a.prodI = prodI; a.prodJ = prodJ; a.prodL = prodL;
			a.blkRow = blkRow; a.blkCol = blkCol; a.u2f = u2f; a.u2fT = u2fT; a.nblk = S.nblk;
			a.lambda = lambda; a.addDiag = rank == 0 ? 1 : 0; a.fVal = fVal; a.bsc = bsc; a.uVal = upperReduce ? uVal.p : nullptr;
			if (mixed) {
				if constexpr (sizeof(T) == 8) {
					schur3::Args<double, float> m;
					m.Hpl = HplF; m.invHll = invHll; m.bl = bl; m.Hpp = Hpp; m.bp = bp; m.prodPtr = prodPtr; m.prodI = prodI; m.prodJ = prodJ; m.prodL = prodL;
					m.blkRow = blkRow; m.blkCol = blkCol; m.u2f = u2f; m.u2fT = u2fT; m.nblk = S.nblk; m.lambda = lambda; m.addDiag = a.addDiag; m.fVal = fVal; m.bsc = bsc; m.uVal = a.uVal;
					schur3::k_schur3<double, float><<<(S.nblk + schur3::WARPS - 1) / schur3::WARPS, schur3::WARPS * 32, 0, stream>>>(m);
				}
			}
			else if (cfg.reserved[3] != 4) schur3::k_schur3<T><<<(S.nblk + schur3::WARPS - 1) / schur3::WARPS, schur3::WARPS * 32, 0, stream>>>(a);
			else schur3::k_schur4<T><<<(S.nblk + schur3::WARPS - 1) / schur3::WARPS, schur3::WARPS * 32, 0, stream>>>(a);
			launches++;
			CUDA_TRY(cudaGetLastError());
			if (upperReduce) {
				static const bool timing = getenv("CUBA_SCHUR_TIMING") != nullptr;
				cudaEvent_t ev[3];
				if (timing) { for (auto& e : ev) cudaEventCreate(&e); cudaEventRecord(ev[0], stream); }
				int rc = uPeerOk ? launch_peer_allreduce() : allreduce(uVal.p, 36 * (size_t)S.nblk + 6 * (size_t)S.numP, true); if (rc) return rc;
				if (timing) cudaEventRecord(ev[1], stream);
				KLAUNCH(schur3::k_expand_upper<T>, 36LL * S.nblk, uVal.p, u2f.p, u2fT.p, blkRow.p, blkCol.p, S.nblk, fVal.p);
				if (timing) {
					cudaEventRecord(ev[2], stream); cudaEventSynchronize(ev[2]);
					float a1 = 0, a2 = 0; cudaEventElapsedTime(&a1, ev[0], ev[1]); cudaEventElapsedTime(&a2, ev[1], ev[2]);
					static int count = 0;
					if (rank == 0 && (count++ % 16) == 8) fprintf(stderr, "schur split: all-reduce (%s) %.3f ms, expand %.3f ms, %zu elements\n", uPeerOk ? "peer" : "nccl", a1, a2, uCount);
					for (auto& e : ev) cudaEventDestroy(e);
				}
			}
			else if (world > 1) {
				int rc = allreduce(fVal.p, 36 * (size_t)S.nfull + 6 * (size_t)S.numP, true); if (rc) return rc;
			}
		}
		else if (S.numP > 0 && S.numL > 0) {
			SchurArgs<T> a;
			a.Hpl = Hpl; a.invHll = invHll; a.bl = bl; a.Hpp = Hpp; a.bp = bp;
			a.prodPtr = prodPtr; a.prodI = prodI; a.prodJ = prodJ; a.hplLm = hplLm;
			a.blkRow = blkRow; a.blkCol = blkCol; a.u2f = u2f; a.u2fT = u2fT; a.nblk = S.nblk;
			a.lambda = lambda; a.addDiag = rank == 0 ? 1 : 0; a.fVal = fVal; a.bsc = bsc;
			const int wpb = SCHUR_BLOCK / 32;
			k_schur<T><<<(S.nblk + wpb - 1) / wpb, SCHUR_BLOCK, 0, stream>>>(a);
			launches++;
			CUDA_TRY(cudaGetLastError());
			if (world > 1) {
				int rc = allreduce(fVal.p, 36 * (size_t)S.nfull + 6 * (size_t)S.numP, true); if (rc) return rc;
			}
		}
		return CUBA_OK;
	}

	int setup_jh4()
	{
		ntW = 0; jh4Grid = 0; jh4HasBig = 0;
		if constexpr (sizeof(T) == 8) {
			using namespace jh4;
			const int lb = S.lmBeg, N = S.lmEnd - S.lmBeg;
			if (N <= 0 || S.eLocal <= 0) return CUBA_OK;
			int K = 1;
			while ((1LL << K) <= (long long)N) K++;
			CUDA_TRY(w_levels.alloc((size_t)K * ((size_t)N + 1)));
			CUDA_TRY(w_start.alloc((size_t)N + 1)); CUDA_TRY(w_pieces.alloc((size_t)N + 1)); CUDA_TRY(w_base.alloc((size_t)N + 1));
			CUDA_TRY(w_flag.alloc(1));
			CUDA_TRY(cudaMemsetAsync(w_flag.p, 0, sizeof(int), stream));
			KLAUNCH(jh4::k_next, N + 1, lmPtr.p, lb, N, w_levels.p);
			for (int k = 1; k < K; k++)
				KLAUNCH(jh4::k_lift, N + 1, w_levels.p + (size_t)(k - 1) * ((size_t)N + 1), N, w_levels.p + (size_t)k * ((size_t)N + 1));
			KLAUNCH(jh4::k_starts, N + 1, w_levels.p, K, N, lmPtr.p, lb, w_start.p, w_pieces.p, w_flag.p);
			int rc = exclusiveSum(w_pieces.p, w_base.p, N + 1); if (rc) return rc;
			if (!jh4Host) CUDA_TRY(cudaMallocHost((void**)&jh4Host, 2 * sizeof(int)));
			CUDA_TRY(cudaMemcpyAsync(&jh4Host[0], w_base.p + N, sizeof(int), cudaMemcpyDeviceToHost, stream));
			CUDA_TRY(cudaMemcpyAsync(&jh4Host[1], w_flag.p, sizeof(int), cudaMemcpyDeviceToHost, stream));
			jh4Pending = true;
		}
		return CUBA_OK;
	}
	int setup_jh4_finish()
	{
		if (!jh4Pending) return CUBA_OK;
		jh4Pending = false;
		if constexpr (sizeof(T) == 8) {
			using namespace jh4;
			const int lb = S.lmBeg, N = S.lmEnd - S.lmBeg;
			CUDA_TRY(cudaStreamSynchronize(stream));
			const int big = jh4Host[1];
			ntW = jh4Host[0]; jh4HasBig = big;
			if (ntW <= 0) return CUBA_OK;
			CUDA_TRY(w_tile.alloc(ntW)); CUDA_TRY(w_rec.alloc(ntW)); CUDA_TRY(w_tilePose.alloc(32 * (size_t)ntW)); CUDA_TRY(w_tilePieces.alloc(ntW)); CUDA_TRY(w_pieceCount.alloc(ntW));
			CUDA_TRY(cudaMemsetAsync(w_pieceCount.p, 0, sizeof(int) * (size_t)ntW, stream));
			CUDA_TRY(w_bigPartial.alloc(std::max<size_t>(big ? 12 * (size_t)ntW : 12, 11 * (size_t)numSMs * 6 * jh4::WARPS)));
			KLAUNCH(jh4::k_emit, (long long)N * 32, w_start.p, w_pieces.p, w_base.p, N, lmPtr.p, lb, w_levels.p,
				e_mx.p, e_my.p, e_mz.p, e_om.p, e_ip.p, e_il.p, e_hpl.p, w_tile.p, w_rec.p, w_tilePose.p, w_tilePieces.p);
			jh4Grid = std::max(1, std::min((ntW + WARPS - 1) / WARPS, numSMs * jh4MinB));
		}
		return CUBA_OK;
	}

	int setup_schur2(const TileInfo* tinfo, int nt)
	{
		using namespace schur2;
		const int N = (int)S.nmulLocal, nblk = S.nblk;
		if (N <= 0) { useSchur2 = false; useSchur5 = false; return CUBA_OK; }
		CUDA_TRY(s2_key.alloc(N)); CUDA_TRY(s2_keyS.alloc(N)); CUDA_TRY(s2_val.alloc(N)); CUDA_TRY(s2_valS.alloc(N));
		CUDA_TRY(s2_head.alloc(N)); CUDA_TRY(s2_segId.alloc(N)); CUDA_TRY(s2_counts.alloc(1));
		KLAUNCH(schur2::k_keys, N, prodPtr.p, nblk, prodI.p, N, tinfo, nt, s2_key.p, s2_val.p);
		int rc = sortPairs(s2_key.p, s2_keyS.p, s2_val.p, s2_valS.p, N, 64); if (rc) return rc;
		KLAUNCH(schur2::k_heads, N, s2_keyS.p, N, s2_head.p);
		rc = exclusiveSum(s2_head.p, s2_segId.p, N); if (rc) return rc;
		schur2::k_counts<<<1, 32, 0, stream>>>(s2_keyS.p, s2_head.p, s2_segId.p, N, s2_counts.p);
		launches++;
		schur2::Counts hc;
		CUDA_TRY(cudaMemcpyAsync(&hc, s2_counts.p, sizeof(hc), cudaMemcpyDeviceToHost, stream));
		CUDA_TRY(cudaStreamSynchronize(stream));
		const int nseg = hc.nseg;
		s2Nseg = nseg; s2Nvalid = hc.nvalid;
		CUDA_TRY(s2_segStart.alloc((size_t)nseg + 1)); CUDA_TRY(s2_segTile.alloc(nseg)); CUDA_TRY(s2_segDest.alloc(nseg));
		CUDA_TRY(s2_key3.alloc(nseg)); CUDA_TRY(s2_key3S.alloc(nseg)); CUDA_TRY(s2_val3.alloc(nseg)); CUDA_TRY(s2_val3S.alloc(nseg));
		CUDA_TRY(s2_segRank.alloc(nseg)); CUDA_TRY(s2_rankDest.alloc(nseg));
		CUDA_TRY(s2_tileSegPtr.alloc((size_t)nt + 1)); CUDA_TRY(s2_destSegPtr.alloc((size_t)nblk + 1));
		CUDA_TRY(s2_p2i.alloc(N)); CUDA_TRY(s2_p2j.alloc(N));
		KLAUNCH(schur2::k_segments, N + 1, s2_keyS.p, s2_valS.p, s2_head.p, s2_segId.p, prodI.p, prodJ.p, N, nseg, hc.nvalid,
			s2_segStart.p, s2_segTile.p, s2_segDest.p, s2_p2i.p, s2_p2j.p, s2_key3.p, s2_val3.p);
		KLAUNCH(schur2::k_ptr_from_field, nt + 1, s2_segTile.p, nseg, nt, s2_tileSegPtr.p);
		rc = sortPairs(s2_key3.p, s2_key3S.p, s2_val3.p, s2_val3S.p, nseg, 32 + sgpu::bits_for((unsigned long long)std::max(nblk, 1))); if (rc) return rc;
		KLAUNCH(schur2::k_rank, nseg, s2_key3S.p, s2_val3S.p, nseg, s2_segRank.p, s2_rankDest.p);
		KLAUNCH(schur2::k_ptr_from_field, nblk + 1, s2_rankDest.p, nseg, nblk, s2_destSegPtr.p);
		CUDA_TRY(s2_partial.alloc((size_t)schur2::PW * std::max(nseg, 1)));
		return CUBA_OK;
	}

	int setup_pcg2()
	{
		const int numP = S.numP;
		int smemMax = 0;
		CUDA_TRY(cudaDeviceGetAttribute(&smemMax, cudaDevAttrMaxSharedMemoryPerBlockOptin, devOrdinal));
		const size_t budget = (size_t)smemMax > 8192 ? (size_t)smemMax - 6144 : 0;
		const size_t matBytes = (size_t)S.nfull * (36 * sizeof(T) + 4);
		int G = std::max((numP + 7) / 8, (int)((matBytes + budget - 1) / std::max<size_t>(budget, 1)));
		G = std::max(1, std::min(G, std::min(numSMs, numP)));
		PcgPartition& PP = hostPP;
		build_pcg_partition(numP, S.nfull, S.fRowPtr, S.fColInd, G, PP);
		const std::vector<int>& rows = PP.rows; const std::vector<int>& nptr = PP.nptr; const std::vector<int>& ncol = PP.ncol; const std::vector<int>& local = PP.local;
		const int needMax = PP.needMax, blkMax = PP.blkMax, maxRows = PP.maxRows;
		const size_t needBytes = (size_t)needMax * (12 * sizeof(T) + 8) + (size_t)maxRows * (12 * sizeof(T) + 4) + ((size_t)maxRows + 1) * 4
			+ (size_t)PCG3_CHUNK * 6 * sizeof(T);
		pcg3Ok = maxRows * 6 <= PCG3_BLOCK && 2 * G <= 2 * PCG3_BLOCK;
		size_t cap = budget > needBytes ? (budget - needBytes) / (36 * sizeof(T) + 4) : 0;
		cap = std::min<size_t>(cap, (size_t)blkMax);
		pcg2Grid = G; pcg2Cap = (int)cap; pcg2NeedMax = needMax; pcg2MaxRows = maxRows;
		pcg2Smem = (size_t)cap * 36 * sizeof(T) + needBytes + (size_t)cap * 4 + 16;
		CUDA_TRY(cudaFuncSetAttribute(k_pcg2<T>, cudaFuncAttributeMaxDynamicSharedMemorySize, (int)pcg2Smem));
		CUDA_TRY(cudaFuncSetAttribute(k_pcg3<T>, cudaFuncAttributeMaxDynamicSharedMemorySize, (int)pcg2Smem));
		CUDA_TRY(llFlags.alloc(2 * (2 * 6 * (size_t)numP) + 2 * (2 * PCG3_REPL * 2 * (size_t)G) + 2));
		int perSM = 0;
		CUDA_TRY(cudaOccupancyMaxActiveBlocksPerMultiprocessor(&perSM, k_pcg2<T>, PCG2_BLOCK, pcg2Smem));
		if (perSM < 1) return fail(CUBA_ERR_CUDA, "k_pcg2 cannot be resident with the requested shared memory");
		arena.reset();
		CUDA_TRY(ctaRow.upload(rows, stream, arena)); CUDA_TRY(needPtr.upload(nptr, stream, arena)); CUDA_TRY(needCol.upload(ncol, stream, arena));
		CUDA_TRY(fLocal.upload(local, stream, arena));
		const size_t n6 = 6 * (size_t)numP;
		CUDA_TRY(fHat.alloc(36 * (size_t)S.nfull)); CUDA_TRY(Linv.alloc(36 * (size_t)numP));
		CUDA_TRY(vR0.alloc(n6)); CUDA_TRY(vR1.alloc(n6)); CUDA_TRY(vS0.alloc(n6)); CUDA_TRY(vS1.alloc(n6));
		CUDA_TRY(vW0.alloc(n6)); CUDA_TRY(vW1.alloc(n6)); CUDA_TRY(vP.alloc(n6)); CUDA_TRY(vY.alloc(n6));
		CUDA_TRY(pcg2Partial.alloc(4 * (size_t)G));
		CUDA_TRY(gridBar.alloc(1));
		CUDA_TRY(cudaMemsetAsync(gridBar.p, 0, sizeof(GridBar), stream));
		tmark("  pcg2 partition + uploads");
		pcg4Ok = false;
		if (cfg.reserved[0] == 3 || sizeof(T) != 8 || numP > 80 * numSMs * (world > 1 && numP >= 2048 ? world : 1)) {
			const int maxAgg = (cfg.reserved[6] > 0 && cfg.reserved[6] < PCG4_MAXAGG) ? cfg.reserved[6] : PCG4_MAXAGG;
			CoarsePartition CP;
			build_coarse_partition(numP, PP, maxAgg, CP);
			const int gs = CP.gs, A = CP.A, nc = 6 * A;
			pcg4Cluster = A > PCG4_MAXAGG1;
			pcg4A = A; pcg4Gs = gs; pcg4MaxNeedAgg = CP.maxNeedAgg;
			size_t fixed4 = (size_t)needMax * (12 * sizeof(T) + 8) + (size_t)maxRows * (6 * sizeof(T) + 8) + 8 + 2 * (size_t)nc * sizeof(T)
				+ (size_t)pcg4MaxNeedAgg * (6 * sizeof(T) + 4) + 64;
			const size_t matAll = (size_t)blkMax * (36 * sizeof(T) + 4);
			const size_t zhBytes = (size_t)needMax * 36 * sizeof(T);
			const size_t sliceBytes = (((size_t)pcg4MaxNeedAgg * 6 * nc + 1) & ~(size_t)1) * sizeof(float);
			pcg4ZhInSmem = budget >= fixed4 + matAll + zhBytes ? 1 : 0;
			if (pcg4ZhInSmem) fixed4 += zhBytes;
			pcg4SliceInSmem = budget >= fixed4 + matAll + sliceBytes ? 1 : 0;
			if (pcg4SliceInSmem) fixed4 += sliceBytes;
			size_t cap4 = budget > fixed4 ? (budget - fixed4) / (36 * sizeof(T) + 4) : 0;
			cap4 = std::min<size_t>(cap4, (size_t)blkMax);
			pcg4Cap = (int)cap4;
			pcg4Smem = (size_t)cap4 * (36 * sizeof(T) + 4) + fixed4;
			if (getenv("CUBA_PCG_VERBOSE")) fprintf(stderr, "pcg4: G %d A %d gs %d needMax %d maxRows %d blkMax %d maxNeedAgg %d zhInSmem %d sliceInSmem %d cap %d smem %zu\n",
				G, A, gs, needMax, maxRows, blkMax, pcg4MaxNeedAgg, pcg4ZhInSmem, pcg4SliceInSmem, pcg4Cap, pcg4Smem);
			const size_t nblkPz = (size_t)A * (A + 1) / 2;
			pcg4InvSmem = pcg4Cluster ? (((nblkPz + PCG4_CL - 1) / PCG4_CL + 2 * (size_t)A) * 36 * sizeof(double) + 2 * nblkPz + 16)
			                          : ((nblkPz + 2 * (size_t)A) * 36 * sizeof(double));
			pcg4Ok = budget > fixed4 && nc + 64 <= PCG4_BLOCK && pcg4InvSmem + 1024 <= (size_t)smemMax && numP >= 2 * A;
			if (pcg4Ok) {
				CUDA_TRY(cudaFuncSetAttribute(k_pcg4<T>, cudaFuncAttributeMaxDynamicSharedMemorySize, (int)pcg4Smem));
				if (pcg4Cluster) CUDA_TRY(cudaFuncSetAttribute(k_coarse_chol_cluster, cudaFuncAttributeMaxDynamicSharedMemorySize, (int)pcg4InvSmem));
				else CUDA_TRY(cudaFuncSetAttribute(k_coarse_invert<T>, cudaFuncAttributeMaxDynamicSharedMemorySize, (int)pcg4InvSmem));
				int perSM4 = 0;
				CUDA_TRY(cudaOccupancyMaxActiveBlocksPerMultiprocessor(&perSM4, k_pcg4<T>, PCG4_BLOCK, pcg4Smem));
				if (perSM4 < 1) pcg4Ok = false;
			}
			if (pcg4Ok) {
				CUDA_TRY(cAggRow.upload(CP.aggRow, stream, arena)); CUDA_TRY(cNaPtr.upload(CP.naPtr, stream, arena)); CUDA_TRY(cNaList.upload(CP.naList, stream, arena));
				CUDA_TRY(cNeedAgg.upload(CP.needAgg, stream, arena));
				build_coarse_lists(numP, S.nfull, S.fRowPtr, S.fColInd, CP);
				CUDA_TRY(cRowOf.upload(CP.rowOf, stream, arena)); CUDA_TRY(cCbPtr.upload(CP.cbPtr, stream, arena)); CUDA_TRY(cCbList.upload(CP.cbList, stream, arena));
				CUDA_TRY(cZx.alloc(36 * (size_t)numP)); CUDA_TRY(cZhat.alloc(36 * (size_t)numP)); CUDA_TRY(cU.alloc(36 * (size_t)S.nfull));
				CUDA_TRY(cAcP.alloc((size_t)A * (A + 1) / 2 * 36)); CUDA_TRY(cAcInv.alloc((size_t)nc * nc));
				CUDA_TRY(cLp.alloc((size_t)A * (A + 1) / 2 * 36)); CUDA_TRY(cWp.alloc((size_t)A * (A + 1) / 2 * 36)); CUDA_TRY(cLd.alloc((size_t)A * 36));
				CUDA_TRY(cPart.alloc(2 * (size_t)G * PCG4_PSTRIDE)); CUDA_TRY(cInfo.alloc(1));
				CUDA_TRY(cudaMemsetAsync(cPart.p, 0, sizeof(double) * cPart.n, stream));
			}
			tlActive = false; coarseValid = false; coarseAge = 0;
		}
		return CUBA_OK;
	}

	int launch_pcg4()
	{
		ProfScope ps(this, CUBA_PROF_DECOMP_NUMERICAL);
		const int numP = S.numP, A = pcg4A, nblkP = A * (A + 1) / 2;
		KLAUNCH(k_coarse_basis<T>, numP, pose[cur].p, numP, cZx.p);
		const int refreshEvery = cfg.reserved[4] > 0 ? cfg.reserved[4] : 8;
		const double lamRatio = (coarseValid && coarseLambda > 0 && curLambda > 0) ? std::max(curLambda / coarseLambda, coarseLambda / curLambda) : 1.0;
		if (!coarseValid || coarseAge >= refreshEvery || lamRatio > 300.0) {
			KLAUNCH(k_coarse_project<T>, 36LL * S.nfull, fVal.p, cRowOf.p, fColInd.p, S.nfull, cZx.p, cU.p);
			KLAUNCH(k_coarse_assemble, (long long)nblkP * 36, cCbPtr.p, cCbList.p, cU.p, nblkP, cAcP.p);
			if (pcg4Cluster) {
				k_coarse_chol_cluster<<<PCG4_CL, 1024, pcg4InvSmem, stream>>>(cAcP.p, A, cLp.p, cLd.p, cAcInv.p, cInfo.p);
				k_coarse_trinv<<<A, 256, (size_t)A * 36 * sizeof(double), stream>>>(cLp.p, cLd.p, A, cWp.p, cInfo.p);
				k_coarse_wtw<<<(nblkP * 36 + 255) / 256, 256, 0, stream>>>(cWp.p, A, cAcInv.p, cInfo.p);
				launches += 2;
			}
			else k_coarse_invert<T><<<1, 1024, pcg4InvSmem, stream>>>(cAcP.p, A, cAcInv.p, cInfo.p);
			launches++;
			CUDA_TRY(cudaGetLastError());
			coarseValid = true; coarseAge = 0; coarseLambda = curLambda;
		}
		coarseAge++;
		Pcg4Args<T> b;
		Pcg2Args<T>& a = b.base;
		a.fRowPtr = fRowPtr; a.fColInd = fColInd; a.fLocal = fLocal; a.fVal = fVal; a.fHat = fHat;
		a.ctaRow = ctaRow; a.needPtr = needPtr; a.needCol = needCol; a.b = bsc; a.numP = S.numP; a.Linv = Linv;
		a.R0 = vR0; a.R1 = vR1; a.S0 = vS0; a.S1 = vS1; a.W0 = vW0; a.W1 = vW1; a.P = vP; a.Y = vY; a.x = xp;
		a.partial = pcg2Partial; a.bar = gridBar; a.capBlocks = pcg4Cap; a.needMax = pcg2NeedMax; a.maxRows = pcg2MaxRows;
		a.maxIters = cfg.pcg_max_iters > 0 ? cfg.pcg_max_iters : std::max(200, 40 * S.numP);
// ... 837 lines not shown
		a.ptr2 = (const int*)(pbIn.p + oPtr); a.ptr3 = a.ptr2 + B + 1;
		a.poseOut = pbOut.p;
		a.stats = stats ? (pb::IterStat*)(pbOut.p + oStat) : nullptr;
		a.counts = (int*)(pbOut.p + oInt); a.nstats = a.counts + 4 * B * R;
		a.level = (unsigned char*)(pbOut.p + oLev);
		pb::k_pose_batch<<<(unsigned)B, pb::BLOCK, 0, stream>>>(a, s);
		launches++;
		CUDA_TRY(cudaGetLastError());
		CUDA_TRY(cudaMemcpyAsync(pbHostOut.p, pbOut.p, sizeof(double) * nOut, cudaMemcpyDeviceToHost, stream));
		g_d2hBytes += (long long)(sizeof(double) * nOut);
		CUDA_TRY(cudaStreamSynchronize(stream));
		const double* o = (const double*)pbHostOut.p;
		for (size_t b = 0; b < B; b++) {
			for (int k = 0; k < 4; k++) qOut[4 * b + k] = o[8 * b + k];
			for (int k = 0; k < 3; k++) tOut[3 * b + k] = o[8 * b + 4 + k];
		}
		if (stats && nStat) memcpy(stats, o + oStat, sizeof(cuba_iter_stat) * nStat);
		const int32_t* oi = (const int32_t*)(o + oInt);
		if (counts) memcpy(counts, oi, sizeof(int32_t) * 4 * B * R);
		if (nstats) memcpy(nstats, oi + 4 * B * R, sizeof(int32_t) * B * R);
		if (levelsOut) {
			const unsigned char* lv = (const unsigned char*)(o + oLev);
			for (size_t b = 0; b < B; b++) {
				for (size_t i = (size_t)bt->ptr2[b]; i < (size_t)bt->ptr2[b + 1]; i++) levelsOut[i] = lv[(size_t)bt->ptr3[b] + i];
				for (size_t j = (size_t)bt->ptr3[b]; j < (size_t)bt->ptr3[b + 1]; j++) levelsOut[E2 + j] = lv[(size_t)bt->ptr2[b + 1] + j];
			}
		}
		return CUBA_OK;
	}

	int optimize_sim3(const cuba_sim3_batch* bt, const s3::Params& p, double* qOut, double* tOut, double* sOut, uint8_t* levelsOut,
		int32_t* ninliers, cuba_iter_stat* stats, int32_t* nstats) override
	{
		static_assert(sizeof(pb::IterStat) == sizeof(cuba_iter_stat) && sizeof(pb::IterStat) == 32, "cuba_iter_stat layout");
		const size_t B = (size_t)bt->B, N = (size_t)bt->N;
		if (B == 0) return CUBA_OK;
		const size_t nStat = stats ? B * (size_t)p.statPer : 0;
		const size_t oPair = s3::PROB * B, oPtr = oPair + s3::PAIR * N, nIn = oPtr + (B + 2) / 2;
		const size_t oStat = 8 * B, oInt = oStat + 4 * nStat, oLev = oInt + (3 * B + 1) / 2, nOut = oLev + (N + 7) / 8;
		CUDA_TRY(s3HostIn.grow(sizeof(double) * nIn)); CUDA_TRY(s3HostOut.grow(sizeof(double) * nOut));
		CUDA_TRY(s3In.alloc(nIn)); CUDA_TRY(s3Out.alloc(nOut));
		double* h = (double*)s3HostIn.p;
		for (size_t b = 0; b < B; b++) {
			double* d = h + s3::PROB * b;
			for (int k = 0; k < 4; k++) d[k] = bt->q[4 * b + k];
			for (int k = 0; k < 3; k++) d[4 + k] = bt->t[3 * b + k];
			d[7] = bt->s[b];
			for (int k = 0; k < 4; k++) { d[8 + k] = bt->cam1[4 * b + k]; d[12 + k] = bt->cam2[4 * b + k]; }
			d[16] = bt->fix_scale && bt->fix_scale[b] ? 1.0 : 0.0;
			d[17] = d[18] = d[19] = 0;
		}
		for (size_t i = 0; i < N; i++) {
			double* d = h + oPair + s3::PAIR * i;
			for (int k = 0; k < 3; k++) { d[k] = bt->X1[3 * i + k]; d[3 + k] = bt->X2[3 * i + k]; }
			d[6] = bt->obs1[2 * i]; d[7] = bt->obs1[2 * i + 1]; d[8] = bt->obs2[2 * i]; d[9] = bt->obs2[2 * i + 1];
			d[10] = bt->omega1[i]; d[11] = bt->omega2[i];
		}
		memcpy(h + oPtr, bt->ptr, sizeof(int32_t) * (B + 1));
		CUDA_TRY(cudaMemcpyAsync(s3In.p, h, sizeof(double) * nIn, cudaMemcpyHostToDevice, stream));
		g_h2dBytes += (long long)(sizeof(double) * nIn);
		s3::Args a;
		a.B = (int)B;
		a.prob = s3In.p; a.pair = s3In.p + oPair; a.ptr = (const int*)(s3In.p + oPtr);
		a.Sout = s3Out.p;
		a.stats = stats ? (pb::IterStat*)(s3Out.p + oStat) : nullptr;
		a.ninliers = (int*)(s3Out.p + oInt); a.nstats = a.ninliers + B;
		a.level = (unsigned char*)(s3Out.p + oLev);
		s3::k_sim3_batch<<<(unsigned)B, s3::BLOCK, 0, stream>>>(a, p);
		launches++;
		CUDA_TRY(cudaGetLastError());
		CUDA_TRY(cudaMemcpyAsync(s3HostOut.p, s3Out.p, sizeof(double) * nOut, cudaMemcpyDeviceToHost, stream));
		g_d2hBytes += (long long)(sizeof(double) * nOut);
		CUDA_TRY(cudaStreamSynchronize(stream));
		const double* o = (const double*)s3HostOut.p;
		for (size_t b = 0; b < B; b++) {
			for (int k = 0; k < 4; k++) qOut[4 * b + k] = o[8 * b + k];
			for (int k = 0; k < 3; k++) tOut[3 * b + k] = o[8 * b + 4 + k];
			sOut[b] = o[8 * b + 7];
		}
		if (stats && nStat) memcpy(stats, o + oStat, sizeof(cuba_iter_stat) * nStat);
		const int32_t* oi = (const int32_t*)(o + oInt);
		if (ninliers) memcpy(ninliers, oi, sizeof(int32_t) * B);
		if (nstats) memcpy(nstats, oi + B, sizeof(int32_t) * 2 * B);
		if (levelsOut && N) memcpy(levelsOut, (const unsigned char*)(o + oLev), N);
		return CUBA_OK;
	}

	int get_profile(double* sec) override
	{
		resolveProfile();
		for (int i = 0; i < CUBA_PROF_NUM; i++) sec[i] = prof[i];
		return CUBA_OK;
	}

	int dbg_hpl_structure(int32_t* colPtr, int32_t* rowInd, int32_t* e2h) override
	{
		if (!haveProblem) return fail(CUBA_ERR_STATE, "no problem");
		{ const int rc0 = ensureHostStructure(); if (rc0) return rc0; }
		if (colPtr) memcpy(colPtr, S.hplColPtr.data(), sizeof(int) * S.hplColPtr.size());
		if (rowInd) memcpy(rowInd, S.hplRowInd.data(), sizeof(int) * S.hplRowInd.size());
		if (e2h) memcpy(e2h, S.edge2Hpl.data(), sizeof(int) * S.edge2Hpl.size());
		return CUBA_OK;
	}
	int dbg_hsc_structure(int32_t* rowPtr, int32_t* colInd) override
	{
		if (!haveProblem) return fail(CUBA_ERR_STATE, "no problem");
		{ const int rc0 = ensureHostStructure(); if (rc0) return rc0; }
		if (rowPtr) memcpy(rowPtr, S.hscRowPtr.data(), sizeof(int) * S.hscRowPtr.size());
		if (colInd) memcpy(colInd, S.hscColInd.data(), sizeof(int) * S.hscColInd.size());
		return CUBA_OK;
	}
	int download(const T* d, size_t n, double* out)
	{
		std::vector<T> h(n);
		CUDA_TRY(cudaMemcpyAsync(h.data(), d, sizeof(T) * n, cudaMemcpyDeviceToHost, stream));
		CUDA_TRY(cudaStreamSynchronize(stream));
		for (size_t i = 0; i < n; i++) out[i] = (double)h[i];
		return CUBA_OK;
	}
	int dbg_system(double* oHpp, double* obp, double* oHll, double* obl, double* oHpl) override
	{
		if (!haveProblem) return fail(CUBA_ERR_STATE, "no problem");
		int rc;
		if (oHpp && (rc = download(Hpp, 36 * (size_t)S.numP, oHpp))) return rc;
		if (obp && (rc = download(bp, 6 * (size_t)S.numP, obp))) return rc;
		if (oHll && (rc = download(Hll, 9 * (size_t)S.numL, oHll))) return rc;
		if (obl && (rc = download(bl, 3 * (size_t)S.numL, obl))) return rc;
		if (oHpl) {
			memset(oHpl, 0, sizeof(double) * 18 * (size_t)S.nhpl);
			if (mixed) {
				std::vector<float> hf(20 * (size_t)S.nhplLocal);
				CUDA_TRY(cudaMemcpyAsync(hf.data(), HplF.p, sizeof(float) * hf.size(), cudaMemcpyDeviceToHost, stream));
				CUDA_TRY(cudaStreamSynchronize(stream));
				for (size_t b = 0; b < (size_t)S.nhplLocal; b++) for (int e = 0; e < 18; e++) oHpl[18 * ((size_t)S.hplBase + b) + e] = (double)hf[20 * b + e];
			}
			else if ((rc = download(Hpl, 18 * (size_t)S.nhplLocal, oHpl + 18 * (size_t)S.hplBase))) return rc;
		}
		return CUBA_OK;
	}
	int dbg_schur(double* oHsc, double* obsc, double* oinv) override
	{
		if (!haveProblem) return fail(CUBA_ERR_STATE, "no problem");
		int rc;
		if ((rc = ensureHostStructure())) return rc;
		if (oHsc) {
			std::vector<double> full(36 * (size_t)S.nfull);
			if ((rc = download(fVal, full.size(), full.data()))) return rc;
			for (int k = 0; k < S.nblk; k++) memcpy(oHsc + 36 * (size_t)k, full.data() + 36 * (size_t)S.u2f[k], sizeof(double) * 36);
		}
		if (obsc && (rc = download(bsc, 6 * (size_t)S.numP, obsc))) return rc;
		if (oinv && (rc = download(invHll, 9 * (size_t)S.numL, oinv))) return rc;
		return CUBA_OK;
	}
	int dbg_delta(double* oxp, double* oxl) override
	{
		if (!haveProblem) return fail(CUBA_ERR_STATE, "no problem");
		int rc;
		if (oxp && (rc = download(xp, 6 * (size_t)S.numP, oxp))) return rc;
		if (oxl && (rc = download(xl, 3 * (size_t)S.numL, oxl))) return rc;
		return CUBA_OK;
	}

	int dbg_pcg_timing(long long* out, int maxCtas) override
	{
		const int n = std::min(maxCtas, pcg2Grid);
		if (!pcgTiming.p || n <= 0) return 0;
		cudaMemcpyAsync(out, pcgTiming.p, sizeof(long long) * 8 * (size_t)n, cudaMemcpyDeviceToHost, stream);
		cudaStreamSynchronize(stream);
		return n;
	}

	int dbg_pcg_info(int32_t* info, double* coarseLambda) override
	{
		if (!haveProblem) return fail(CUBA_ERR_STATE, "no problem");
		CUDA_TRY(cudaStreamSynchronize(stream));
		PcgStatus ps{};
		CUDA_TRY(cudaMemcpy(&ps, &dScal.p->pcg, sizeof(ps), cudaMemcpyDeviceToHost));
		int last = -1, bad = 0;
		if (p5Ok && p5A > 0 && p5Rebuilds > 0) {
			const int nlog = (int)std::min<long long>(p5Rebuilds, P5_INFO_LOG);
			std::vector<int> log(nlog);
			CUDA_TRY(cudaMemcpy(log.data(), cInfo.p + 1, sizeof(int) * nlog, cudaMemcpyDeviceToHost));
			for (int v : log) if (v != 0) bad++;
			last = log[(int)((p5Rebuilds - 1) % P5_INFO_LOG)];
		}
		int coarseKernel = CUBA_COARSE_KERNEL_NONE;
		if (lastPcgTwoLevel && lastPcgKernel == CUBA_PCG_KERNEL_PCG4) coarseKernel = pcg4Cluster ? CUBA_COARSE_KERNEL_PCG4_CLUSTER : CUBA_COARSE_KERNEL_INVERT;
		else if (lastPcgTwoLevel && p5Ok)
			coarseKernel = p5Dense ? CUBA_COARSE_KERNEL_DENSE : p5Cluster == 16 ? CUBA_COARSE_KERNEL_CLUSTER16 : p5Cluster == 8 ? CUBA_COARSE_KERNEL_CLUSTER8 : CUBA_COARSE_KERNEL_INVERT;
		const bool tuned = p5Ok && p5Tuned;
		const int32_t v[CUBA_PCG_INFO_LEN] = {
			lastPcgKernel, lastPcgKernel != CUBA_PCG_KERNEL_NONE && lastPcgTwoLevel ? 1 : 0,
			p5Ok ? p5Apc : 0, p5Ok ? p5G : 0, p5Ok ? p5Gs : 0, p5Ok ? p5A : 0,
			p5Ok ? (tuned ? p5tDims.maxRows : p5Dims.maxRows) : 0, p5Ok ? (tuned ? p5tDims.capBlocks : p5Dims.capBlocks) : 0,
			p5Ok ? (tuned ? p5tDims.zhInSmem : p5Dims.zhInSmem) : 0,
			coarseKernel, last, ps.status, ps.iters, (int32_t)p5Rebuilds, (int32_t)bjRetries, bad };
		if (info) memcpy(info, v, sizeof(v));
		if (coarseLambda) *coarseLambda = p5CoarseValid ? p5CoarseLambda : 0.0;
		return CUBA_OK;
	}
	int dbg_coarse(int32_t* rowAgg, double* oAcP, float* oAcInv) override
	{
		if (!haveProblem) return fail(CUBA_ERR_STATE, "no problem");
		if (!p5Ok || p5A < 1 || !p5CoarseValid) return fail(CUBA_ERR_STATE, "debug_get_coarse: no coarse level of k_pcg5 has been built");
		const int A = p5A, nc = 6 * A;
		CUDA_TRY(cudaStreamSynchronize(stream));
		if (rowAgg) {
			std::vector<int> ptr(A + 1);
			CUDA_TRY(cudaMemcpy(ptr.data(), p5AggRow.p, sizeof(int) * (A + 1), cudaMemcpyDeviceToHost));
			for (int i = 0; i < S.numP; i++) rowAgg[i] = -1;
			for (int ag = 0; ag < A; ag++) for (int i = ptr[ag]; i < ptr[ag + 1] && i < S.numP; i++) rowAgg[i] = ag;
		}
		if (oAcP) CUDA_TRY(cudaMemcpy(oAcP, p5AcP.p, sizeof(double) * 36 * ((size_t)A * (A + 1) / 2), cudaMemcpyDeviceToHost));
		if (oAcInv) CUDA_TRY(cudaMemcpy(oAcInv, p5AcInv.p, sizeof(float) * (size_t)nc * nc, cudaMemcpyDeviceToHost));
		return CUBA_OK;
	}
	int dbg_coarse_inverse(const double* hAcP, int A, float* hAcInv, int* hInfo) override
	{
		if (A < 1 || !hAcP || !hAcInv || !hInfo) return fail(CUBA_ERR_INVALID, "debug_coarse_inverse: A < 1 or a NULL pointer");
		const size_t nc = 6 * (size_t)A, nblkP = (size_t)A * (A + 1) / 2;
		DBuf<double> dAcP, dT;
		DBuf<float> dInv;
		DBuf<int> dInfo;
		DBuf<GridBar> dBar;
		CUDA_TRY(dAcP.alloc(36 * nblkP)); CUDA_TRY(dInv.alloc(nc * nc)); CUDA_TRY(dInfo.alloc(1)); CUDA_TRY(dBar.alloc(1));
		CUDA_TRY(dT.alloc(2 * cdense::tiles((int)((nc + cdense::NB - 1) / cdense::NB)) * cdense::TT));
		CUDA_TRY(cudaMemcpyAsync(dAcP.p, hAcP, sizeof(double) * 36 * nblkP, cudaMemcpyHostToDevice, stream));
		CUDA_TRY(cudaMemsetAsync(dBar.p, 0, sizeof(GridBar), stream));
		CUDA_TRY(cudaMemsetAsync(dInfo.p, 0xff, sizeof(int), stream));
		int rc = launch_coarse_dense(dAcP, A, dT, dInv, dInfo, dBar); if (rc) return rc;
		CUDA_TRY(cudaMemcpyAsync(hAcInv, dInv.p, sizeof(float) * nc * nc, cudaMemcpyDeviceToHost, stream));
		CUDA_TRY(cudaMemcpyAsync(hInfo, dInfo.p, sizeof(int), cudaMemcpyDeviceToHost, stream));
		CUDA_TRY(cudaStreamSynchronize(stream));
		return CUBA_OK;
	}

	int bench_stage(int stage, int reps, int flush, double lambda, double* ms) override
	{
		if (!haveProblem) return fail(CUBA_ERR_STATE, "bench before set_problem");
		if (reps < 1) reps = 1;
		const size_t flushN = (size_t)40 << 20;
		if (flush) CUDA_TRY(flushBuf.alloc(flushN));
		cudaEvent_t a, b;
		CUDA_TRY(cudaEventCreate(&a)); CUDA_TRY(cudaEventCreate(&b));
		double total = 0;
		const T lam = (T)lambda;
		for (int r = 0; r < reps; r++) {
			if (flush) { k_fill<<<numSMs * 8, 256, 0, stream>>>(flushBuf.p, flushN, (double)r); launches++; }
			CUDA_TRY(cudaEventRecord(a, stream));
			int rc = CUBA_OK;
			switch (stage) {
			case 0: rc = launch_linearize_landmark(); if (!rc) rc = launch_linearize_pose(); break;
			case 1: rc = launch_linearize_landmark(); break;
			case 2: rc = launch_linearize_pose(); break;
			case 3: rc = launch_schur(lam); break;
			case 4: curLambda = lambda; rc = launch_pcg(); break;
			case 5: rc = launch_backsub(lam); if (!rc) rc = stage_update_nofetch(lam); break;
			case 6: rc = launch_chi2(cur, 0); break;
			case 7:
				if (!p5Ok || p5A < 1) rc = fail(CUBA_ERR_STATE, "bench_stage: no two-level k_pcg5 plan");
				else rc = launch_coarse_setup(p5A, p5Cluster, p5InvSmem, p5CbPtr, p5CbList, p5AcP, p5AcInv, p5Lp, p5Ld, p5Wp, p5Dense);
				break;
			default: rc = fail(CUBA_ERR_INVALID, "bench_stage: unknown stage");
			}
			if (rc) return rc;
			CUDA_TRY(cudaEventRecord(b, stream));
			CUDA_TRY(cudaEventSynchronize(b));
			float t = 0;
			CUDA_TRY(cudaEventElapsedTime(&t, a, b));
			total += t;
		}
		cudaEventDestroy(a); cudaEventDestroy(b);
		resolveProfile();
		if (ms) *ms = total / reps;
		return CUBA_OK;
	}
	int stage_update_nofetch(T lam)
	{
		if (S.numP > 0) {
			k_update_poses<T><<<nPoseBlocks, RED_BLOCK, 0, stream>>>(xp, bp, S.numP, lam, pose[cur], pose[cur ^ 1], scalePartialP);
			launches++;
			CUDA_TRY(cudaGetLastError());
		}
		return launch_chi2(cur ^ 1, 1);
	}
};

}

using namespace cuba_b200;

struct cuba_engine { std::unique_ptr<EngineBase> impl; };

extern "C" {

const char* cuba_last_error(void) { return g_err.c_str(); }
int cuba_version(void) { return 100; }

int cuba_engine_create(const cuba_config* cfg, cuba_engine** out)
{
	if (!out) return fail(CUBA_ERR_INVALID, "create: null out");
	cuba_config c;
	memset(&c, 0, sizeof(c));
	c.device = -1; c.deterministic = 1;
	if (cfg) c = *cfg;
	std::unique_ptr<EngineBase> impl;
// ... 53 lines not shown
int cuba_engine_set_state(cuba_engine* e, const double* q, const double* t, const double* Xw)
{
	ENGINE_OR_FAIL(e);
	if (!q || !t || !Xw) return fail(CUBA_ERR_INVALID, "set_state: null array");
	return e->impl->set_state(q, t, Xw);
}
int cuba_engine_reset_state(cuba_engine* e) { ENGINE_OR_FAIL(e); return e->impl->reset_state(); }
int cuba_engine_get_stream(cuba_engine* e, void** s) { ENGINE_OR_FAIL(e); if (!s) return fail(CUBA_ERR_INVALID, "null out"); return e->impl->get_stream(s); }
int cuba_engine_flush_l2(cuba_engine* e) { ENGINE_OR_FAIL(e); return e->impl->flush_l2(); }
int cuba_engine_get_sizes(const cuba_engine* e, cuba_sizes* out) { ENGINE_OR_FAIL(e); if (!out) return fail(CUBA_ERR_INVALID, "null out"); return e->impl->get_sizes(out); }
int cuba_engine_optimize(cuba_engine* e, int niter, cuba_iter_stat* stats, int* nstats) { ENGINE_OR_FAIL(e); return e->impl->optimize(niter, stats, nstats); }
int cuba_engine_get_state(cuba_engine* e, double* q, double* t, double* Xw) { ENGINE_OR_FAIL(e); return e->impl->get_state(q, t, Xw); }
int cuba_engine_get_chi2(cuba_engine* e, double* per_edge) { ENGINE_OR_FAIL(e); if (!per_edge) return fail(CUBA_ERR_INVALID, "null out"); return e->impl->get_chi2(per_edge); }
int cuba_engine_set_edge_levels(cuba_engine* e, const uint8_t* levels) { ENGINE_OR_FAIL(e); return e->impl->set_edge_levels(levels); }
int cuba_engine_get_edge_levels(cuba_engine* e, uint8_t* levels)
{
	ENGINE_OR_FAIL(e);
	if (!levels) return fail(CUBA_ERR_INVALID, "null out");
	return e->impl->get_edge_levels(levels);
}
int cuba_engine_classify_edges(cuba_engine* e, double chi2_mono, double chi2_stereo, int flags, int32_t* counts)
{
	ENGINE_OR_FAIL(e);
	if (flags & ~(CUBA_CLASSIFY_DEPTH | CUBA_CLASSIFY_REINCLUDE)) return fail(CUBA_ERR_INVALID, "classify_edges: unknown flag");
	return e->impl->classify_edges(chi2_mono, chi2_stereo, flags, counts);
}
static int pose_frames_ok(int B, int E, const int32_t* ptr, const double* X, const double* meas, const double* om, const char* what)
{
	if (E < 0) return fail(CUBA_ERR_INVALID, std::string("optimize_poses: negative edge count ") + what);
	if (!ptr) return fail(CUBA_ERR_INVALID, std::string("optimize_poses: null ptr") + what);
	if (ptr[0] != 0) return fail(CUBA_ERR_INVALID, std::string("optimize_poses: ptr") + what + "[0] != 0");
	for (int b = 0; b < B; b++)
		if (ptr[b + 1] < ptr[b]) return fail(CUBA_ERR_INVALID, std::string("optimize_poses: ptr") + what + " decreases");
	if (ptr[B] != E) return fail(CUBA_ERR_INVALID, std::string("optimize_poses: ptr") + what + "[B] is not the edge count");
	if (E > 0 && (!X || !meas || !om)) return fail(CUBA_ERR_INVALID, std::string("optimize_poses: null edge array ") + what);
	for (int i = 0; i < E; i++)
		if (!std::isfinite(om[i])) return fail(CUBA_ERR_INVALID, std::string("optimize_poses: non-finite omega") + what);
	return CUBA_OK;
}

int cuba_engine_optimize_poses(cuba_engine* e, const cuba_pose_batch* bt, int nrounds, const cuba_pose_round* rounds,
	double* q_out, double* t_out, uint8_t* levels_out, int32_t* counts, cuba_iter_stat* stats, int32_t* nstats)
{
	ENGINE_OR_FAIL(e);
	if (!bt) return fail(CUBA_ERR_INVALID, "optimize_poses: null batch");
	if (bt->B < 0) return fail(CUBA_ERR_INVALID, "optimize_poses: B < 0");
	if (nrounds < 1 || nrounds > CUBA_POSE_MAX_ROUNDS || !rounds) return fail(CUBA_ERR_INVALID, "optimize_poses: nrounds outside 1..CUBA_POSE_MAX_ROUNDS");
	static_assert(CUBA_POSE_MAX_ROUNDS == pb::MAX_ROUNDS, "round limit");
	pb::Schedule s;
	memset(&s, 0, sizeof(s));
	s.n = nrounds;
	long long off = 0;
	for (int r = 0; r < nrounds; r++) {
		const cuba_pose_round& R = rounds[r];
		if (R.iterations < 0) return fail(CUBA_ERR_INVALID, "optimize_poses: negative iterations");
		if (R.flags & ~(CUBA_CLASSIFY_DEPTH | CUBA_CLASSIFY_REINCLUDE)) return fail(CUBA_ERR_INVALID, "optimize_poses: unknown flag");
		for (int k = 0; k < 2; k++) {
			if (R.kernel_type[k] < CUBA_ROBUST_NONE || R.kernel_type[k] > CUBA_ROBUST_TUKEY) return fail(CUBA_ERR_INVALID, "optimize_poses: unknown kernel type");
			if (!std::isfinite(R.delta[k])) return fail(CUBA_ERR_INVALID, "optimize_poses: non-finite delta");
			s.rk[r].type[k] = R.kernel_type[k]; s.rk[r].delta[k] = R.delta[k];
		}
		s.r[r].iterations = R.iterations; s.r[r].restart = R.restart != 0; s.r[r].flags = R.flags;
		s.r[r].chi2[0] = R.chi2_mono; s.r[r].chi2[1] = R.chi2_stereo;
		s.statOff[r] = (int)off;
		off += R.iterations;
		if (off > INT32_MAX) return fail(CUBA_ERR_INVALID, "optimize_poses: too many iterations");
	}
	s.statOff[nrounds] = (int)off;
	const int B = bt->B;
	if (B == 0) return CUBA_OK;
	if (!bt->q || !bt->t || !bt->cam || !q_out || !t_out) return fail(CUBA_ERR_INVALID, "optimize_poses: null pose array");
	if ((long long)bt->E2 + bt->E3 > INT32_MAX) return fail(CUBA_ERR_INVALID, "optimize_poses: too many edges");
	int rc = pose_frames_ok(B, bt->E2, bt->ptr2, bt->X2, bt->meas2, bt->omega2, "2"); if (rc) return rc;
	rc = pose_frames_ok(B, bt->E3, bt->ptr3, bt->X3, bt->meas3, bt->omega3, "3"); if (rc) return rc;
	return e->impl->optimize_poses(bt, s, q_out, t_out, levels_out, counts, stats, nstats);
}

static bool all_finite(const double* p, size_t n)
{
	for (size_t i = 0; i < n; i++)
		if (!std::isfinite(p[i])) return false;
	return true;
}

int cuba_engine_optimize_sim3(cuba_engine* e, const cuba_sim3_batch* bt, const cuba_sim3_params* params, double* q_out, double* t_out,
	double* s_out, uint8_t* levels_out, int32_t* ninliers, cuba_iter_stat* stats, int32_t* nstats)
{
	ENGINE_OR_FAIL(e);
	if (!bt || !params) return fail(CUBA_ERR_INVALID, "optimize_sim3: null batch or params");
	const cuba_sim3_params& P = *params;
	if (!std::isfinite(P.chi2) || !(P.chi2 > 0)) return fail(CUBA_ERR_INVALID, "optimize_sim3: chi2 not finite and positive");
	if (P.iterations < 0 || P.iterations_bad < 0 || P.iterations_good < 0) return fail(CUBA_ERR_INVALID, "optimize_sim3: negative iterations");
	if (P.min_pairs < 0) return fail(CUBA_ERR_INVALID, "optimize_sim3: negative min_pairs");
	if ((long long)P.iterations + std::max(P.iterations_bad, P.iterations_good) > INT32_MAX)
		return fail(CUBA_ERR_INVALID, "optimize_sim3: too many iterations");
	if (bt->B < 0) return fail(CUBA_ERR_INVALID, "optimize_sim3: B < 0");
	if (bt->N < 0) return fail(CUBA_ERR_INVALID, "optimize_sim3: N < 0");
	const int B = bt->B;
	if (B == 0) return CUBA_OK;
	const size_t nb = (size_t)B, N = (size_t)bt->N;
	if (!bt->ptr) return fail(CUBA_ERR_INVALID, "optimize_sim3: null ptr");
	if (bt->ptr[0] != 0) return fail(CUBA_ERR_INVALID, "optimize_sim3: ptr[0] != 0");
	for (int b = 0; b < B; b++)
		if (bt->ptr[b + 1] < bt->ptr[b]) return fail(CUBA_ERR_INVALID, "optimize_sim3: ptr decreases");
	if (bt->ptr[B] != bt->N) return fail(CUBA_ERR_INVALID, "optimize_sim3: ptr[B] is not the pair count");
	if (!bt->q || !bt->t || !bt->s || !bt->cam1 || !bt->cam2 || !q_out || !t_out || !s_out)
		return fail(CUBA_ERR_INVALID, "optimize_sim3: null problem array");
	if (N > 0 && (!bt->X1 || !bt->X2 || !bt->obs1 || !bt->obs2 || !bt->omega1 || !bt->omega2))
		return fail(CUBA_ERR_INVALID, "optimize_sim3: null pair array");
	if (!all_finite(bt->q, 4 * nb) || !all_finite(bt->t, 3 * nb) || !all_finite(bt->s, nb) || !all_finite(bt->cam1, 4 * nb) ||
		!all_finite(bt->cam2, 4 * nb))
		return fail(CUBA_ERR_INVALID, "optimize_sim3: non-finite S12 or intrinsics");
	for (size_t b = 0; b < nb; b++)
		if (!(bt->s[b] > 0)) return fail(CUBA_ERR_INVALID, "optimize_sim3: s <= 0");
	if (!all_finite(bt->X1, 3 * N) || !all_finite(bt->X2, 3 * N) || !all_finite(bt->obs1, 2 * N) || !all_finite(bt->obs2, 2 * N) ||
		!all_finite(bt->omega1, N) || !all_finite(bt->omega2, N))
		return fail(CUBA_ERR_INVALID, "optimize_sim3: non-finite pair");
	s3::Params p;
	p.chi2 = P.chi2; p.delta = std::sqrt(P.chi2);
	p.iterations = P.iterations; p.iterationsBad = P.iterations_bad; p.iterationsGood = P.iterations_good; p.minPairs = P.min_pairs;
	p.statPer = P.iterations + std::max(P.iterations_bad, P.iterations_good);
	return e->impl->optimize_sim3(bt, p, q_out, t_out, s_out, levels_out, ninliers, stats, nstats);
}

int cuba_engine_get_profile(cuba_engine* e, double* sec) { ENGINE_OR_FAIL(e); if (!sec) return fail(CUBA_ERR_INVALID, "null out"); return e->impl->get_profile(sec); }
int cuba_debug_get_pcg_timing(cuba_engine* e, long long* out, int maxCtas)
{
	if (!e || !e->impl) return -1;
	DevGuard guard(e->impl->devOrdinal);
	return e->impl->dbg_pcg_timing(out, maxCtas);
}
int cuba_get_transfer_bytes(long long* h2d, long long* d2h) { if (h2d) *h2d = g_h2dBytes; if (d2h) *d2h = g_d2hBytes; return CUBA_OK; }
int cuba_engine_get_launch_count(cuba_engine* e, long long* count) { ENGINE_OR_FAIL(e); if (count) *count = e->impl->launches; return CUBA_OK; }

int cuba_stage_linearize(cuba_engine* e, double* chi2) { ENGINE_OR_FAIL(e); return e->impl->stage_linearize(chi2); }
int cuba_stage_max_diagonal(cuba_engine* e, double* md) { ENGINE_OR_FAIL(e); return e->impl->stage_max_diagonal(md); }
int cuba_stage_solve(cuba_engine* e, double lambda, int* iters, int* ok)
{
	ENGINE_OR_FAIL(e);
	int it = 0, k = 1;
	const int rc = e->impl->stage_solve(lambda, &it, &k);
	if (iters) *iters = it;
	if (ok) *ok = k;
	return rc;
}
int cuba_stage_update(cuba_engine* e, double lambda, double* chi, double* scale) { ENGINE_OR_FAIL(e); return e->impl->stage_update(lambda, chi, scale); }
int cuba_stage_commit(cuba_engine* e, int accept) { ENGINE_OR_FAIL(e); return e->impl->stage_commit(accept); }
int cuba_stage_chi2(cuba_engine* e, double* chi) { ENGINE_OR_FAIL(e); return e->impl->stage_chi2(chi); }

int cuba_debug_get_hpl_structure(cuba_engine* e, int32_t* colPtr, int32_t* rowInd, int32_t* e2h) { ENGINE_OR_FAIL(e); return e->impl->dbg_hpl_structure(colPtr, rowInd, e2h); }
int cuba_debug_get_hsc_structure(cuba_engine* e, int32_t* rowPtr, int32_t* colInd) { ENGINE_OR_FAIL(e); return e->impl->dbg_hsc_structure(rowPtr, colInd); }
int cuba_debug_get_system(cuba_engine* e, double* Hpp, double* bp, double* Hll, double* bl, double* Hpl) { ENGINE_OR_FAIL(e); return e->impl->dbg_system(Hpp, bp, Hll, bl, Hpl); }
int cuba_debug_get_schur(cuba_engine* e, double* Hsc, double* bsc, double* invHll) { ENGINE_OR_FAIL(e); return e->impl->dbg_schur(Hsc, bsc, invHll); }
int cuba_debug_get_delta(cuba_engine* e, double* xp, double* xl) { ENGINE_OR_FAIL(e); return e->impl->dbg_delta(xp, xl); }
int cuba_debug_get_pcg_info(cuba_engine* e, int32_t* info, double* coarse_lambda) { ENGINE_OR_FAIL(e); return e->impl->dbg_pcg_info(info, coarse_lambda); }
int cuba_debug_get_coarse(cuba_engine* e, int32_t* aggRow, double* AcP, float* AcInv) { ENGINE_OR_FAIL(e); return e->impl->dbg_coarse(aggRow, AcP, AcInv); }
int cuba_debug_coarse_inverse(cuba_engine* e, const double* AcP, int A, float* AcInv, int* info) { ENGINE_OR_FAIL(e); return e->impl->dbg_coarse_inverse(AcP, A, AcInv, info); }
int cuba_debug_build_structure_host(const cuba_problem* p, int rank, int world, cuba_sizes* sizes,
	int32_t* hplColPtr, int32_t* hplRowInd, int32_t* edge2Hpl, int32_t* hscRowPtr, int32_t* hscColInd,
	int32_t* fullRowPtr, int32_t* fullColInd, int32_t* shard)
{
	if (!p) return fail(CUBA_ERR_INVALID, "null problem");
	Structure S;
	const char* err = "";
	if (!build_structure(p->Pall, p->numP, p->Lall, p->numL, p->E2, p->idx2, p->E3, p->idx3, rank, world, TILE, S, &err))
		return fail(CUBA_ERR_INVALID, err);
	if (sizes) {
		sizes->Pall = S.Pall; sizes->numP = S.numP; sizes->Lall = S.Lall; sizes->numL = S.numL; sizes->E2 = S.E2; sizes->E3 = S.E3;
		sizes->nhpl = S.nhpl; sizes->nblk = S.nblk; sizes->nmul = (int32_t)S.nmul; sizes->nblk_full = S.nfull;
	}
	auto cp = [](int32_t* dst, const std::vector<int>& v) { if (dst && !v.empty()) memcpy(dst, v.data(), sizeof(int) * v.size()); };
	cp(hplColPtr, S.hplColPtr); cp(hplRowInd, S.hplRowInd); cp(edge2Hpl, S.edge2Hpl);
	cp(hscRowPtr, S.hscRowPtr); cp(hscColInd, S.hscColInd); cp(fullRowPtr, S.fRowPtr); cp(fullColInd, S.fColInd);
	if (shard) { shard[0] = S.lmBeg; shard[1] = S.lmEnd; shard[2] = S.eLocal; shard[3] = (int32_t)S.nmulLocal; }
	if ((int)S.tileLm.size() < 1 || S.tileLm.front() != S.lmBeg || S.tileLm.back() != S.lmEnd) return fail(CUBA_ERR_INVALID, "structure self-check: tiles");
	for (size_t t = 0; t + 1 < S.tileLm.size(); t++) {
		const int nl = S.tileLm[t + 1] - S.tileLm[t];
		const int ne = S.lmPtr[S.tileLm[t + 1]] - S.lmPtr[S.tileLm[t]];
		if (nl < 1 || nl > TILE || (ne > TILE && nl != 1)) return fail(CUBA_ERR_INVALID, "structure self-check: tile size");
	}
	for (int k = 0; k < S.nblk; k++)
		for (int n = S.prodPtr[k]; n < S.prodPtr[k + 1]; n++) {
			const int i = S.prodI[n] + S.hplBase, j = S.prodJ[n] + S.hplBase;
			if (S.hplRowInd[i] != S.blkRow[k] || S.hplRowInd[j] != S.blkCol[k] || S.hplLm[S.prodI[n]] != S.hplLm[S.prodJ[n]] || i > j)
				return fail(CUBA_ERR_INVALID, "structure self-check: product list");
		}
	return CUBA_OK;
}

int cuba_debug_pcg_partition(const cuba_problem* p, int nCtas, int maxAgg, int32_t* info)
{
	if (!p || nCtas < 1 || maxAgg < 1) return fail(CUBA_ERR_INVALID, "pcg_partition: bad arguments");
	Structure S;
	const char* err = "";
	if (!build_structure(p->Pall, p->numP, p->Lall, p->numL, p->E2, p->idx2, p->E3, p->idx3, 0, 1, TILE, S, &err)) return fail(CUBA_ERR_INVALID, err);
	if (S.numP < 1) return fail(CUBA_ERR_INVALID, "pcg_partition: no free pose");
	const int G = std::max(1, std::min(nCtas, S.numP));
	PcgPartition P; CoarsePartition C;
	build_pcg_partition(S.numP, S.nfull, S.fRowPtr, S.fColInd, G, P);
	build_coarse_partition(S.numP, P, maxAgg, C);
	build_coarse_lists(S.numP, S.nfull, S.fRowPtr, S.fColInd, C);
	const char* bad = check_pcg_partition(S.numP, S.nfull, S.fRowPtr, S.fColInd, P, C);
	if (bad) return fail(CUBA_ERR_INVALID, std::string("pcg_partition self-check: ") + bad);
	if (info) { info[0] = P.G; info[1] = C.gs; info[2] = C.A; info[3] = P.needMax; info[4] = P.maxRows; info[5] = P.blkMax; info[6] = C.maxNeedAgg; info[7] = (int32_t)C.cbList.size(); }
	return CUBA_OK;
}

int cuba_debug_pcg5_plan(const cuba_problem* p, int world, int numSMs, int maxAgg, int32_t* info)
{
	return cuba_debug_pcg5_plan_apc(p, world, numSMs, maxAgg, 1, info, nullptr);
}

int cuba_debug_pcg5_plan_apc(const cuba_problem* p, int world, int numSMs, int maxAgg, int aggsPerCta, int32_t* info, uint64_t* hash)
{
	if (!p || world < 1 || world > 8 || numSMs < 1 || maxAgg < 1 || aggsPerCta < 1 || aggsPerCta > 3) return fail(CUBA_ERR_INVALID, "pcg5_plan: bad arguments");
	Structure S;
	const char* err = "";
	if (!build_structure(p->Pall, p->numP, p->Lall, p->numL, p->E2, p->idx2, p->E3, p->idx3, 0, 1, TILE, S, &err)) return fail(CUBA_ERR_INVALID, err);
	Pcg5Plan plan;
	build_pcg5_plan(S.numP, S.nfull, S.fRowPtr, S.fColInd, world, numSMs, maxAgg, 2 * PCG5_BLOCK / 6, plan, nullptr, aggsPerCta);
	if (info) for (int i = 0; i < 8; i++) info[i] = 0;
	if (hash) *hash = 0;
	if (!plan.ok) return CUBA_OK;
	const char* bad = check_pcg5_plan(S.numP, S.nfull, S.fRowPtr, S.fColInd, plan);
	if (bad) return fail(CUBA_ERR_INVALID, std::string("pcg5_plan self-check: ") + bad);
	if (info) {
		int halo = 0;
		for (unsigned char m : plan.rowPeers) if (m) halo++;
		info[0] = 1; info[1] = plan.G; info[2] = plan.gs; info[3] = plan.A; info[4] = plan.P.needMax; info[5] = plan.P.maxRows; info[6] = plan.C.maxNeedAgg; info[7] = halo;
	}
	if (hash) {
		uint64_t h = 1469598103934665603ull;
		auto mix = [&h](const void* data, size_t bytes) {
			const unsigned char* b = (const unsigned char*)data;
			for (size_t i = 0; i < bytes; i++) { h ^= b[i]; h *= 1099511628211ull; }
		};
		auto vec = [&mix](const std::vector<int>& v) { const uint64_t n = v.size(); mix(&n, sizeof n); mix(v.data(), v.size() * sizeof(int)); };
		const int scal[] = { plan.G, plan.gs, plan.A, plan.P.needMax, plan.P.blkMax, plan.P.maxRows, plan.C.maxNeedAgg };
		mix(scal, sizeof scal);
		for (const std::vector<int>* v : { &plan.P.rows, &plan.P.nptr, &plan.P.ncol, &plan.P.local, &plan.C.aggRow, &plan.C.rowAgg, &plan.C.naPtr,
			&plan.C.naList, &plan.C.needAgg, &plan.C.rowOf, &plan.C.cbPtr, &plan.C.cbList }) vec(*v);
		mix(plan.rowPeers.data(), plan.rowPeers.size());
		*hash = h;
	}
	return CUBA_OK;
}

int cuba_bench_stage(cuba_engine* e, int stage, int reps, int flush, double lambda, double* ms) { ENGINE_OR_FAIL(e); return e->impl->bench_stage(stage, reps, flush, lambda, ms); }

}
```

### cuda-bundle-adjustment_b200/csrc/cuba_structure_gpu.cuh

```cuda
#pragma once

#include <cub/cub.cuh>
#include <cuda_runtime.h>
#include <stdint.h>

namespace cuba_b200 {
namespace sgpu {

constexpr int BLK = 256;
inline int grid_for(long long n) { return (int)((n + BLK - 1) / BLK); }

struct Meta {
	int error;
	int nhpl;
	int lmBeg, lmEnd, kBeg, kEnd, hplBase, hplEnd;
	long long nmul;
	int nblk;
	int npe;
	int bounds[9];
};

__global__ void k_make_keys(int E2, const int* __restrict__ idx2, int E3, const int* __restrict__ idx3, int Pall, int numP, int Lall, int numL,
	unsigned long long* key, int* val, Meta* meta)
{
// ... 87 lines not shown
	const int l = blockIdx.x * blockDim.x + threadIdx.x;
	if (l > numL) return;
	const int k = lmPtrG[l];
	hplColPtr[l] = k < E ? hplG[k] : nhpl;
}

template <typename T>
__global__ void k_edge_stream(const unsigned long long* __restrict__ keys, const int* __restrict__ val, const int* __restrict__ ff,
	const int* __restrict__ hplG, int kBeg, int eLocal, int hplBase, int E2,
	const double* __restrict__ meas2, const double* __restrict__ om2, const double* __restrict__ meas3, const double* __restrict__ om3,
	int* e_user, int* e_ip, int* e_il, int* e_hpl, T* mx, T* my, T* mz, T* om)
{
	const int e = blockIdx.x * blockDim.x + threadIdx.x;
	if (e >= eLocal) return;
	const int k = kBeg + e, u = val[k];
	const bool stereo = u >= E2;
	e_user[e] = u;
	e_ip[e] = (int)(keys[k] & 0xffffffffu) | (stereo ? (int)0x80000000u : 0);
	e_il[e] = (int)(keys[k] >> 32);
	e_hpl[e] = ff[k] ? hplG[k] - hplBase : -1 - (hplG[k] - hplBase);
	if (!stereo) { mx[e] = (T)meas2[2 * (size_t)u]; my[e] = (T)meas2[2 * (size_t)u + 1]; mz[e] = T(0); om[e] = (T)om2[u]; }
	else { const size_t s = (size_t)(u - E2); mx[e] = (T)meas3[3 * s]; my[e] = (T)meas3[3 * s + 1]; mz[e] = (T)meas3[3 * s + 2]; om[e] = (T)om3[s]; }
}

__global__ void k_local_lmptr(const int* __restrict__ lmPtrG, int Lall, int kBeg, int kEnd, int* lmPtr)
{
	const int l = blockIdx.x * blockDim.x + threadIdx.x;
	if (l > Lall) return;
	int v = lmPtrG[l];
	v = v < kBeg ? kBeg : (v > kEnd ? kEnd : v);
	lmPtr[l] = v - kBeg;
}

__global__ void k_tiles(const int* __restrict__ lmPtr, int lmBeg, int lmEnd, int tile, int nt, int* tileLm)
{
	const int t = blockIdx.x * blockDim.x + threadIdx.x;
	if (t > nt) return;
	if (t == nt) { tileLm[t] = lmEnd; return; }
	const int target = t * tile;
	int lo = lmBeg, hi = lmEnd;
	while (lo < hi) { const int mid = (lo + hi) >> 1; if (lmPtr[mid] < target) lo = mid + 1; else hi = mid; }
	tileLm[t] = lo;
}

__global__ void k_pose_keys(const int* __restrict__ e_ip, int eLocal, int numP, unsigned int* key, int* val)
{
	const int e = blockIdx.x * blockDim.x + threadIdx.x;
	if (e >= eLocal) return;
	const int ip = e_ip[e] & 0x7fffffff;
	key[e] = ip < numP ? (unsigned)ip : (unsigned)numP;
	val[e] = e;
}

template <typename T>
__global__ void k_pose_stream(const int* __restrict__ src, const int* __restrict__ posePtr, int numP, int eLocal,
	const int* __restrict__ e_ip, const int* __restrict__ e_il,
	const T* __restrict__ mx, const T* __restrict__ my, const T* __restrict__ mz, const T* __restrict__ om,
	int* p_il, T* pmx, T* pmy, T* pmz, T* pom)
{
	const int k = blockIdx.x * blockDim.x + threadIdx.x;
	if (k >= eLocal || k >= posePtr[numP]) return;
	const int e = src[k];
	p_il[k] = e_il[e] | (e_ip[e] & (int)0x80000000u);
	pmx[k] = mx[e]; pmy[k] = my[e]; pmz[k] = mz[e]; pom[k] = om[e];
}

__global__ void k_prod_count(const int* __restrict__ hplLmG, const int* __restrict__ hplColPtr, int nhpl, int* cnt)
{
	const int i = blockIdx.x * blockDim.x + threadIdx.x;
	if (i >= nhpl) return;
	cnt[i] = hplColPtr[hplLmG[i] + 1] - i;
}

__global__ void k_prod_emit(const int* __restrict__ hplLmG, const int* __restrict__ hplColPtr, const int* __restrict__ hplRowInd,
	const int* __restrict__ off, int nhpl, int lmBeg, int lmEnd, int hplBase, unsigned long long* pkey, int* pval, int* pi, int* pj)
{
	const int i = blockIdx.x * blockDim.x + threadIdx.x;
	if (i >= nhpl) return;
	const int l = hplLmG[i];
	const int cend = hplColPtr[l + 1];
	const bool local = l >= lmBeg && l < lmEnd;
	const unsigned long long hi = (unsigned long long)(unsigned)hplRowInd[i] << 32;
	int n = off[i];
	for (int j = i; j < cend; j++, n++) {
		pkey[n] = hi | (unsigned)hplRowInd[j];
		pval[n] = n;
		pi[n] = local ? i - hplBase : -1;
		pj[n] = j - hplBase;
	}
}

__global__ void k_prod_diag(int numP, long long nmul, unsigned long long* pkey, int* pval, int* pi, int* pj)
{
	const int p = blockIdx.x * blockDim.x + threadIdx.x;
	if (p >= numP) return;
	const long long n = nmul + p;
	pkey[n] = ((unsigned long long)(unsigned)p << 32) | (unsigned)p;
	pval[n] = (int)n; pi[n] = -1; pj[n] = -1;
}

__global__ void k_heads(const unsigned long long* __restrict__ keys, int n, int* head)
{
	const int i = blockIdx.x * blockDim.x + threadIdx.x;
	if (i >= n) return;
	head[i] = (i == 0 || keys[i] != keys[i - 1]) ? 1 : 0;
}

__global__ void k_nblk(const int* __restrict__ head, const int* __restrict__ blkId, int n, Meta* meta)
{
	if (blockIdx.x == 0 && threadIdx.x == 0) meta->nblk = n > 0 ? blkId[n - 1] + head[n - 1] : 0;
}

__global__ void k_blocks(const unsigned long long* __restrict__ keys, const int* __restrict__ pvalSorted, const int* __restrict__ head,
	const int* __restrict__ blkId, const int* __restrict__ pi, const int* __restrict__ pj, int n,
	int* blkRow, int* blkCol, int* prodPtr, int* prodI, int* prodJ)
{
	const int i = blockIdx.x * blockDim.x + threadIdx.x;
	if (i > n) return;
	if (i == n) { const int nb = n > 0 ? blkId[n - 1] + head[n - 1] : 0; prodPtr[nb] = n; return; }
	if (head[i]) { const int k = blkId[i]; blkRow[k] = (int)(keys[i] >> 32); blkCol[k] = (int)(keys[i] & 0xffffffffu); prodPtr[k] = i; }
	const int s = pvalSorted[i];
	prodI[i] = pi[s]; prodJ[i] = pj[s];
}

__global__ void k_local_flag(const int* __restrict__ prodI, const int* __restrict__ prodJ, int n, int* flag)
{
	const int i = blockIdx.x * blockDim.x + threadIdx.x;
	if (i > n) return;
	flag[i] = (i < n && (prodI[i] >= 0 || prodJ[i] < 0)) ? 1 : 0;
}
__global__ void k_compact_products(const int* __restrict__ prodI, const int* __restrict__ prodJ, const int* __restrict__ flag, const int* __restrict__ pos,
	int n, int* outI, int* outJ)
{
	const int i = blockIdx.x * blockDim.x + threadIdx.x;
	if (i >= n || !flag[i]) return;
	outI[pos[i]] = prodI[i]; outJ[pos[i]] = prodJ[i];
}
__global__ void k_remap_ptr(const int* __restrict__ pos, int nblk, int* prodPtr)
{
	const int k = blockIdx.x * blockDim.x + threadIdx.x;
	if (k > nblk) return;
	prodPtr[k] = pos[prodPtr[k]];
}

__global__ void k_rowptr_from_rows(const int* __restrict__ rows, int n, int numP, int* rowPtr)
{
	const int a = blockIdx.x * blockDim.x + threadIdx.x;
	if (a > numP) return;
	int lo = 0, hi = n;
	while (lo < hi) { const int mid = (lo + hi) >> 1; if (rows[mid] < a) lo = mid + 1; else hi = mid; }
	rowPtr[a] = lo;
}

__global__ void k_full_entries(const int* __restrict__ blkRow, const int* __restrict__ blkCol, int nblk, int numP, unsigned long long* key, int* val)
{
	const int k = blockIdx.x * blockDim.x + threadIdx.x;
	if (k >= nblk) return;
	const unsigned a = (unsigned)blkRow[k], b = (unsigned)blkCol[k];
	key[2 * (size_t)k] = ((unsigned long long)a << 32) | b; val[2 * (size_t)k] = k << 1;
	key[2 * (size_t)k + 1] = a == b ? ((unsigned long long)(unsigned)numP << 32) : (((unsigned long long)b << 32) | a);
	val[2 * (size_t)k + 1] = (k << 1) | 1;
}

__global__ void k_full_finish(const unsigned long long* __restrict__ key, const int* __restrict__ val, int nfull,
	const int* __restrict__ blkRow, const int* __restrict__ blkCol, int* fColInd, int* u2f, int* u2fT)
{
	const int p = blockIdx.x * blockDim.x + threadIdx.x;
	if (p >= nfull) return;
	fColInd[p] = (int)(key[p] & 0xffffffffu);
	const int k = val[p] >> 1;
	if (val[p] & 1) u2fT[k] = p;
	else { u2f[k] = p; if (blkRow[k] == blkCol[k]) u2fT[k] = p; }
}

inline int bits_for(unsigned long long maxValue)
{
	int b = 1;
	while (b < 64 && (maxValue >> b) != 0) b++;
	return b;
}

}
}
```

### include/cuba_b200.h

```cpp
#ifndef CUBA_B200_H
#define CUBA_B200_H

#include <stddef.h>
#include <stdint.h>

#ifdef __cplusplus
extern "C" {
#endif

#define CUBA_OK 0
#define CUBA_ERR_INVALID (-1)
#define CUBA_ERR_CUDA (-2)
#define CUBA_ERR_STATE (-3)
#define CUBA_ERR_COMM (-4)

#define CUBA_ROBUST_NONE 0
#define CUBA_ROBUST_HUBER 1
#define CUBA_ROBUST_TUKEY 2

#define CUBA_EDGE_MONOCULAR 0
#define CUBA_EDGE_STEREO 1

#define CUBA_PROF_INITIALIZE 0
#define CUBA_PROF_BUILD_STRUCTURE 1
// ... 8 lines not shown
typedef struct cuba_config {
	int device;
	int use_fp32;
	int pcg_max_iters;
	double pcg_tol;
	int deterministic;
	int reserved[7];
} cuba_config;

typedef struct cuba_problem {
	int32_t Pall, numP;
	int32_t Lall, numL;
	const double* q;
	const double* t;
	const double* cam;
	const double* Xw;
	int32_t E2;
	const int32_t* idx2;
	const double* meas2;
	const double* omega2;
	int32_t E3;
	const int32_t* idx3;
	const double* meas3;
	const double* omega3;
} cuba_problem;

typedef struct cuba_iter_stat {
	int32_t iteration;
	int32_t trials;
	double chi2;
	double lambda;
	int32_t pcg_iters;
	int32_t pcg_failed;
} cuba_iter_stat;

typedef struct cuba_sizes {
	int32_t Pall, numP, Lall, numL, E2, E3;
	int32_t nhpl;
	int32_t nblk;
	int32_t nmul;
	int32_t nblk_full;
} cuba_sizes;

typedef struct cuba_engine cuba_engine;

const char* cuba_last_error(void);
int cuba_version(void);

int cuba_engine_create(const cuba_config* cfg , cuba_engine** out);
int cuba_engine_destroy(cuba_engine* e);

int cuba_engine_set_robust_kernel(cuba_engine* e, int edge_type, int kernel_type, double delta);

int cuba_comm_unique_id(void* out128);
int cuba_engine_set_comm(cuba_engine* e, int rank, int world, const void* nccl_unique_id);

int cuba_engine_set_problem(cuba_engine* e, const cuba_problem* p);
int cuba_engine_set_structure_reuse(cuba_engine* e, int enable);
int cuba_engine_get_structure_reuses(cuba_engine* e, long long* count);
int cuba_engine_set_state(cuba_engine* e, const double* q, const double* t, const double* Xw);

int cuba_engine_reset_state(cuba_engine* e);

int cuba_engine_get_sizes(const cuba_engine* e, cuba_sizes* out);
int cuba_engine_get_stream(cuba_engine* e, void** stream);
int cuba_engine_flush_l2(cuba_engine* e);

int cuba_engine_optimize(cuba_engine* e, int niterations, cuba_iter_stat* stats, int* nstats);

int cuba_engine_get_state(cuba_engine* e, double* q, double* t, double* Xw);
int cuba_engine_get_chi2(cuba_engine* e, double* per_edge);
int cuba_engine_set_edge_levels(cuba_engine* e, const uint8_t* levels);
int cuba_engine_get_edge_levels(cuba_engine* e, uint8_t* levels);

#define CUBA_CLASSIFY_DEPTH 1
#define CUBA_CLASSIFY_REINCLUDE 2
int cuba_engine_classify_edges(cuba_engine* e, double chi2_mono, double chi2_stereo, int flags, int32_t* counts);

typedef struct cuba_pose_batch {
	int32_t B, E2, E3;
	const double* q;
	const double* t;
	const double* cam;
	const int32_t* ptr2;
	const double* X2;
	const double* meas2;
	const double* omega2;
	const int32_t* ptr3;
	const double* X3;
	const double* meas3;
	const double* omega3;
} cuba_pose_batch;

#define CUBA_POSE_MAX_ROUNDS 8
typedef struct cuba_pose_round {
	int32_t iterations;
	int32_t kernel_type[2];
	double delta[2];
	int32_t restart;
	double chi2_mono, chi2_stereo;
	int32_t flags;
} cuba_pose_round;

int cuba_engine_optimize_poses(cuba_engine* e, const cuba_pose_batch* batch, int nrounds, const cuba_pose_round* rounds,
	double* q_out, double* t_out, uint8_t* levels_out, int32_t* counts, cuba_iter_stat* stats, int32_t* nstats);

typedef struct cuba_sim3_batch {
	int32_t B, N;
	const int32_t* ptr;
	const double* q;
	const double* t;
	const double* s;
	const double* cam1;
	const double* cam2;
	const int32_t* fix_scale;
	const double* X1;
	const double* X2;
	const double* obs1;
	const double* obs2;
	const double* omega1;
	const double* omega2;
} cuba_sim3_batch;

#define CUBA_SIM3_DEFAULT_CHI2 10.0
#define CUBA_SIM3_DEFAULT_ITERATIONS 5
#define CUBA_SIM3_DEFAULT_ITERATIONS_BAD 10
#define CUBA_SIM3_DEFAULT_ITERATIONS_GOOD 5
#define CUBA_SIM3_DEFAULT_MIN_PAIRS 10
typedef struct cuba_sim3_params {
	double chi2;
	int32_t iterations, iterations_bad, iterations_good, min_pairs;
} cuba_sim3_params;

int cuba_engine_optimize_sim3(cuba_engine* e, const cuba_sim3_batch* batch, const cuba_sim3_params* params, double* q_out, double* t_out,
	double* s_out, uint8_t* levels_out, int32_t* ninliers, cuba_iter_stat* stats, int32_t* nstats);

int cuba_engine_get_profile(cuba_engine* e, double* seconds);
int cuba_engine_get_launch_count(cuba_engine* e, long long* count);

int cuba_get_transfer_bytes(long long* h2d, long long* d2h);

int cuba_stage_linearize(cuba_engine* e, double* chi2);
int cuba_stage_max_diagonal(cuba_engine* e, double* maxdiag);
int cuba_stage_solve(cuba_engine* e, double lambda, int* pcg_iters, int* ok);
int cuba_stage_update(cuba_engine* e, double lambda, double* chi2_trial, double* scale);
int cuba_stage_commit(cuba_engine* e, int accept);
int cuba_stage_chi2(cuba_engine* e, double* chi2);

int cuba_debug_get_hpl_structure(cuba_engine* e, int32_t* colPtr, int32_t* rowInd, int32_t* edge2Hpl);
int cuba_debug_get_hsc_structure(cuba_engine* e, int32_t* rowPtr, int32_t* colInd);
int cuba_debug_get_system(cuba_engine* e, double* Hpp , double* bp , double* Hll ,
	double* bl , double* Hpl );
int cuba_debug_get_schur(cuba_engine* e, double* Hsc , double* bsc , double* invHll );
int cuba_debug_get_delta(cuba_engine* e, double* xp , double* xl );

#define CUBA_PCG_INFO_LEN 16
#define CUBA_PCG_KERNEL_NONE 0
#define CUBA_PCG_KERNEL_PCG 1
#define CUBA_PCG_KERNEL_PCG2 2
#define CUBA_PCG_KERNEL_PCG3 3
#define CUBA_PCG_KERNEL_PCG4 4
#define CUBA_PCG_KERNEL_PCG5 5
#define CUBA_PCG_KERNEL_PCG5_BIG 6
#define CUBA_PCG_KERNEL_PCG5T 7
#define CUBA_COARSE_KERNEL_NONE 0
#define CUBA_COARSE_KERNEL_INVERT 1
#define CUBA_COARSE_KERNEL_CLUSTER8 2
#define CUBA_COARSE_KERNEL_CLUSTER16 3
#define CUBA_COARSE_KERNEL_DENSE 4
#define CUBA_COARSE_KERNEL_PCG4_CLUSTER 5
int cuba_debug_get_pcg_info(cuba_engine* e, int32_t* info, double* coarse_lambda);
int cuba_debug_get_coarse(cuba_engine* e, int32_t* aggRow, double* AcP, float* AcInv);
int cuba_debug_coarse_inverse(cuba_engine* e, const double* AcP, int A, float* AcInv, int* info);

int cuba_debug_build_structure_host(const cuba_problem* p, int rank, int world, cuba_sizes* sizes,
	int32_t* hplColPtr , int32_t* hplRowInd , int32_t* edge2Hpl ,
	int32_t* hscRowPtr , int32_t* hscColInd ,
	int32_t* fullRowPtr , int32_t* fullColInd ,
	int32_t* shard );

int cuba_debug_pcg_partition(const cuba_problem* p, int nCtas, int maxAgg, int32_t* info);

int cuba_debug_pcg5_plan(const cuba_problem* p, int world, int numSMs, int maxAgg, int32_t* info);
int cuba_debug_pcg5_plan_apc(const cuba_problem* p, int world, int numSMs, int maxAgg, int aggsPerCta, int32_t* info, uint64_t* hash);
int cuba_debug_dropin_problem(void* dropin, cuba_problem* out);
int cuba_debug_dropin_levels(void* dropin, const uint8_t** levels, int32_t* n);

int cuba_bench_stage(cuba_engine* e, int stage, int reps, int flush_l2, double lambda, double* avg_ms);

#ifdef __cplusplus
}
#endif
#endif
```

Before: 245.6 million.

## Add dynamic work-stealing Schur kernel and row-staged Schur6 variant

Adds a Schur-complement kernel that hands out Hsc blocks through a global atomic counter. When the product counts are skewed, blocks are ordered heaviest first to reduce load imbalance across warps. It also adds an opt-in row-based Schur kernel that stages W=Hpl*invHll rows in shared memory and splits rows into balanced work items. The cost is host-side setup with device-to-host copies and one atomic per block.

```diff
diff --git a/cuda-bundle-adjustment_b200/binding.py b/cuda-bundle-adjustment_b200/binding.py
--- a/cuda-bundle-adjustment_b200/binding.py
+++ b/cuda-bundle-adjustment_b200/binding.py
@@ -106,7 +106,7 @@
     "cuba_engine_optimize", "cuba_engine_get_state", "cuba_engine_get_chi2", "cuba_engine_set_edge_levels", "cuba_engine_get_edge_levels", "cuba_engine_classify_edges", "cuba_engine_optimize_poses", "cuba_engine_optimize_sim3", "cuba_engine_get_profile",
     "cuba_engine_get_launch_count", "cuba_get_transfer_bytes", "cuba_stage_linearize", "cuba_stage_max_diagonal", "cuba_stage_solve", "cuba_stage_update",
     "cuba_stage_commit", "cuba_stage_chi2", "cuba_debug_get_hpl_structure", "cuba_debug_get_hsc_structure",
-    "cuba_debug_get_system", "cuba_debug_get_schur", "cuba_debug_get_delta", "cuba_debug_get_pcg_info", "cuba_debug_get_coarse", "cuba_debug_coarse_inverse", "cuba_debug_build_structure_host", "cuba_debug_pcg_partition", "cuba_debug_pcg5_plan", "cuba_debug_pcg5_plan_apc", "cuba_debug_dropin_problem", "cuba_debug_dropin_levels", "cuba_bench_stage",
+    "cuba_debug_get_system", "cuba_debug_get_schur", "cuba_debug_get_schur_rows", "cuba_debug_get_delta", "cuba_debug_get_pcg_info", "cuba_debug_get_coarse", "cuba_debug_coarse_inverse", "cuba_debug_build_structure_host", "cuba_debug_pcg_partition", "cuba_debug_pcg5_plan", "cuba_debug_pcg5_plan_apc", "cuba_debug_dropin_problem", "cuba_debug_dropin_levels", "cuba_bench_stage",
 ]
 
 
@@ -159,6 +159,7 @@
         "cuba_debug_get_hsc_structure": [vp, vp, vp],
         "cuba_debug_get_system": [vp, vp, vp, vp, vp, vp],
         "cuba_debug_get_schur": [vp, vp, vp, vp],
+        "cuba_debug_get_schur_rows": [vp, vp, vp, vp, vp],
         "cuba_debug_get_delta": [vp, vp, vp],
         "cuba_debug_get_pcg_info": [vp, vp, C.POINTER(d)],
         "cuba_debug_get_coarse": [vp, vp, vp, vp],
@@ -523,6 +524,16 @@
         _check(self.L.cuba_debug_get_schur(self.h, _p(Hsc), _p(bsc), _p(inv)))
         return Hsc, bsc, inv
 
+    def schur_rows(self):
+        s = self.sizes
+        info = np.zeros(5, np.int32)
+        _check(self.L.cuba_debug_get_schur_rows(self.h, None, None, None, _p(info)))
+        if not info[0]:
+            return None, None, None, info
+        rowHplPtr = np.zeros(s["numP"] + 1, np.int32); rowHpl = np.zeros(s["nhpl"], np.int32); iloc = np.zeros(max(int(info[4]), 1), np.int32)
+        _check(self.L.cuba_debug_get_schur_rows(self.h, _p(rowHplPtr), _p(rowHpl), _p(iloc), _p(info)))
+        return rowHplPtr, rowHpl, iloc[:info[4]], info
+
     def delta(self):
         s = self.sizes
         xp = np.zeros((s["numP"], 6)); xl = np.zeros((s["numL"], 3))
diff --git a/cuda-bundle-adjustment_b200/build.py b/cuda-bundle-adjustment_b200/build.py
--- a/cuda-bundle-adjustment_b200/build.py
+++ b/cuda-bundle-adjustment_b200/build.py
@@ -5,7 +5,7 @@
 CSRC = os.path.join(HERE, "csrc")
 LIB = os.path.join(HERE, "libcuba_b200.so")
 SOURCES = ["cuba_engine.cu", "cuba_structure.cpp", "cuba_api.cpp"]
-HEADERS = ["cuba_kernels.cuh", "cuba_jh4.cuh", "cuba_levels.cuh", "cuba_pose_batch.cuh", "cuba_sim3_batch.cuh", "cuba_schur3.cuh", "cuba_schur5.cuh", "cuba_pcg2.cuh", "cuba_pcg3.cuh", "cuba_pcg4.cuh", "cuba_pcg5.cuh", "cuba_pcg5t.cuh", "cuba_coarse_dense.cuh", "cuba_peer_reduce.cuh", "cuba_schur2.cuh", "cuba_structure_gpu.cuh", "cuba_math.cuh", "cuba_structure.h",
+HEADERS = ["cuba_kernels.cuh", "cuba_jh4.cuh", "cuba_levels.cuh", "cuba_pose_batch.cuh", "cuba_sim3_batch.cuh", "cuba_schur3.cuh", "cuba_schur5.cuh", "cuba_schur6.cuh", "cuba_pcg2.cuh", "cuba_pcg3.cuh", "cuba_pcg4.cuh", "cuba_pcg5.cuh", "cuba_pcg5t.cuh", "cuba_coarse_dense.cuh", "cuba_peer_reduce.cuh", "cuba_schur2.cuh", "cuba_structure_gpu.cuh", "cuba_math.cuh", "cuba_structure.h",
            "../../include/cuba_b200.h", "../../include/cuba_b200_levels.h", "../../include/cuba_b200_pose.h", "../../include/cuba_b200_sim3.h", "../../include/cuda_bundle_adjustment.h", "../../include/cuda_bundle_adjustment_types.h"]
 NVCC = os.environ.get("NVCC", "/usr/local/cuda/bin/nvcc")
 FLAGS = (["-DCUBA_JH4_DEBUG"] if os.environ.get("CUBA_JH4_DEBUG") else []) + ["-O3", "-std=c++17", "-gencode", "arch=compute_90a,code=sm_90a", "-lineinfo",
diff --git a/cuda-bundle-adjustment_b200/csrc/cuba_engine.cu b/cuda-bundle-adjustment_b200/csrc/cuba_engine.cu
--- a/cuda-bundle-adjustment_b200/csrc/cuba_engine.cu
+++ b/cuda-bundle-adjustment_b200/csrc/cuba_engine.cu
@@ -26,6 +26,7 @@
 #include "cuba_sim3_batch.cuh"
 #include "cuba_schur3.cuh"
 #include "cuba_schur5.cuh"
+#include "cuba_schur6.cuh"
 #include "cuba_structure.h"
 #include "cuba_structure_gpu.cuh"
 
@@ -201,6 +202,7 @@
 	virtual int dbg_hsc_structure(int32_t* rowPtr, int32_t* colInd) = 0;
 	virtual int dbg_system(double* Hpp, double* bp, double* Hll, double* bl, double* Hpl) = 0;
 	virtual int dbg_schur(double* Hsc, double* bsc, double* invHll) = 0;
+	virtual int dbg_schur_rows(int32_t* rowHplPtr, int32_t* rowHpl, int32_t* prodIloc, int32_t* info) = 0;
 	virtual int dbg_delta(double* xp, double* xl) = 0;
 	virtual int bench_stage(int stage, int reps, int flush, double lambda, double* ms) = 0;
 	virtual int dbg_pcg_timing(long long* out, int maxCtas) = 0;
@@ -263,6 +265,15 @@
 	bool upperReduce = false;
 	DBuf<int> prodPtr, prodI, prodJ, prodL, blkRow, blkCol, u2f, u2fT, fRowPtr, fColInd;
 	bool useSchur3 = true;
+	bool useSchur6 = false;
+	DBuf<int> rowHplPtr, rowHpl, rowLm, prodIloc;
+	DBuf<int4> s6Work;
+	bool useSchurDyn = false;
+	DBuf<int> dynOrder, dynCounter;
+	int dynGrid = 0;
+	bool dynHeavyFirst = false;
+	int s6Items = 0, s6Cap = 0, s6Fallback = 0;
+	size_t s6Smem = 0;
 	DBuf<T> pr, pz, pq, pp0, pp1, Minv;
 	DBuf<double> pcgPartial;
 	int pcgGrid = 0;
@@ -730,7 +741,7 @@
 		else CUDA_TRY(Hpl.alloc(18 * (size_t)S.nhplLocal));
 		CUDA_TRY(invHll.alloc(9 * nL));
 		CUDA_TRY(fVal.alloc(36 * (size_t)S.nfull + 6 * nP)); bsc.alias(fVal.p + 36 * (size_t)S.nfull, 6 * nP);
-		upperReduce = world > 1 && (cfg.reserved[3] == 0 || cfg.reserved[3] == 3 || cfg.use_fp32 == 2) && S.numP > 0 && S.numL > 0;
+		upperReduce = world > 1 && (cfg.reserved[3] == 0 || cfg.reserved[3] == 3 || cfg.reserved[3] == 6 || cfg.reserved[3] == 9 || cfg.use_fp32 == 2) && S.numP > 0 && S.numL > 0;
 		if (upperReduce) {
 			uCount = 36 * (size_t)S.nblk + 6 * nP;
 			const size_t need = ((uCount + 1) & ~(size_t)1) + 64;
@@ -775,12 +786,16 @@
 		jh3Grid = std::max(1, std::min(ntiles, numSMs * 4));
 		useSchur2 = cfg.reserved[3] == 2 && S.numP > 0 && S.numL > 0 && ntiles > 0;
 		useSchur5 = cfg.reserved[3] == 5 && cfg.reserved[1] != 1 && sizeof(T) == 8 && S.numP > 0 && S.numL > 0 && ntiles > 0 && S.eLocal > 0;
-		useSchur3 = cfg.reserved[3] == 0 || cfg.reserved[3] == 3 || cfg.reserved[3] == 4 || cfg.use_fp32 == 2;
+		useSchur3 = cfg.reserved[3] == 0 || cfg.reserved[3] == 3 || cfg.reserved[3] == 4 || cfg.reserved[3] == 6 || cfg.reserved[3] == 9 || cfg.use_fp32 == 2;
 		if (cfg.use_fp32 == 2) { useSchur2 = false; useSchur5 = false; }
-		if (useSchur3 && S.nmulLocal > 0) {
+		useSchur6 = world == 1 && cfg.reserved[3] == 6 && S.numP > 0 && S.numL > 0 && S.nhplLocal > 0 && S.nmulLocal > 0;
+		if (useSchur6) { int rc = setup_schur6(); if (rc) return rc; }
+		else if (useSchur3 && S.nmulLocal > 0) {
 			CUDA_TRY(prodL.alloc((size_t)S.nmulLocal));
 			KLAUNCH(schur3::k_prod_landmark, S.nmulLocal, prodI.p, hplLm.p, (int)S.nmulLocal, prodL.p);
 		}
+		useSchurDyn = world == 1 && (cfg.reserved[3] == 0 || cfg.reserved[3] == 9) && !useSchur6 && S.numP > 0 && S.numL > 0 && S.nblk > 0;
+		if (useSchurDyn) { int rc = setup_schur_dyn(); if (rc) return rc; }
 		if (useSchur5) {
 			const int tb5 = std::min(S.lmBeg, S.numL), te5 = std::min(S.lmEnd, S.numL) + (S.lmEnd > S.numL ? 1 : 0);
 			s5Ntiles = (S.eLocal + schur5::WINDOW - 1) / schur5::WINDOW;
@@ -1087,20 +1102,45 @@
 				CUDA_TRY(cudaGetLastError());
 			}
 		}
-		if (useSchur3 && S.numP > 0 && S.numL > 0) {
+		if (useSchur6) {
+			auto fill = [&](auto& r) {
+				r.invHll = invHll; r.bl = bl; r.Hpp = Hpp; r.bp = bp;
+				r.prodPtr = prodPtr; r.prodIloc = prodIloc; r.prodJ = prodJ; r.rowHplPtr = rowHplPtr; r.rowHpl = rowHpl; r.rowLm = rowLm;
+				r.work = s6Work; r.blkCol = blkCol; r.u2f = u2f; r.u2fT = u2fT; r.cap = s6Cap;
+				r.lambda = lambda; r.addDiag = 1; r.fVal = fVal; r.bsc = bsc;
+			};
+			bool done = false;
+			if constexpr (sizeof(T) == 8) {
+				if (mixed) {
+					schur6::Args<double, float> m; fill(m); m.Hpl = HplF;
+					schur6::k_schur_rows<double, float><<<s6Items, schur6::WARPS * 32, s6Smem, stream>>>(m);
+					done = true;
+				}
+			}
+			if (!done) {
+				schur6::Args<T> a; fill(a); a.Hpl = Hpl;
+				schur6::k_schur_rows<T><<<s6Items, schur6::WARPS * 32, s6Smem, stream>>>(a);
+			}
+			launches++;
+			CUDA_TRY(cudaGetLastError());
+		}
+		else if (useSchur3 && S.numP > 0 && S.numL > 0) {
 			schur3::Args<T> a;
 			a.Hpl = Hpl; a.invHll = invHll; a.bl = bl; a.Hpp = Hpp; a.bp = bp;
 			a.prodPtr = prodPtr; a.prodI = prodI; a.prodJ = prodJ; a.prodL = prodL;
 			a.blkRow = blkRow; a.blkCol = blkCol; a.u2f = u2f; a.u2fT = u2fT; a.nblk = S.nblk;
 			a.lambda = lambda; a.addDiag = rank == 0 ? 1 : 0; a.fVal = fVal; a.bsc = bsc; a.uVal = upperReduce ? uVal.p : nullptr;
+			if (useSchurDyn) CUDA_TRY(cudaMemsetAsync(dynCounter.p, 0, sizeof(int), stream));
 			if (mixed) {
 				if constexpr (sizeof(T) == 8) {
 					schur3::Args<double, float> m;
 					m.Hpl = HplF; m.invHll = invHll; m.bl = bl; m.Hpp = Hpp; m.bp = bp; m.prodPtr = prodPtr; m.prodI = prodI; m.prodJ = prodJ; m.prodL = prodL;
 					m.blkRow = blkRow; m.blkCol = blkCol; m.u2f = u2f; m.u2fT = u2fT; m.nblk = S.nblk; m.lambda = lambda; m.addDiag = a.addDiag; m.fVal = fVal; m.bsc = bsc; m.uVal = a.uVal;
-					schur3::k_schur3<double, float><<<(S.nblk + schur3::WARPS - 1) / schur3::WARPS, schur3::WARPS * 32, 0, stream>>>(m);
+					if (useSchurDyn) schur3::k_schur_dyn<double, float><<<dynGrid, schur3::WARPS * 32, 0, stream>>>(m, dynOrder.p, dynCounter.p);
+					else schur3::k_schur3<double, float><<<(S.nblk + schur3::WARPS - 1) / schur3::WARPS, schur3::WARPS * 32, 0, stream>>>(m);
 				}
 			}
+			else if (useSchurDyn) schur3::k_schur_dyn<T><<<dynGrid, schur3::WARPS * 32, 0, stream>>>(a, dynOrder.p, dynCounter.p);
 			else if (cfg.reserved[3] != 4) schur3::k_schur3<T><<<(S.nblk + schur3::WARPS - 1) / schur3::WARPS, schur3::WARPS * 32, 0, stream>>>(a);
 			else schur3::k_schur4<T><<<(S.nblk + schur3::WARPS - 1) / schur3::WARPS, schur3::WARPS * 32, 0, stream>>>(a);
 			launches++;
@@ -1184,6 +1224,91 @@
 				e_mx.p, e_my.p, e_mz.p, e_om.p, e_ip.p, e_il.p, e_hpl.p, w_tile.p, w_rec.p, w_tilePose.p, w_tilePieces.p);
 			jh4Grid = std::max(1, std::min((ntW + WARPS - 1) / WARPS, numSMs * jh4MinB));
 		}
+		return CUBA_OK;
+	}
+
+	int setup_schur_dyn()
+	{
+		const int nblk = S.nblk;
+		std::vector<int> hProd((size_t)nblk + 1), order(nblk);
+		CUDA_TRY(cudaMemcpyAsync(hProd.data(), prodPtr.p, sizeof(int) * hProd.size(), cudaMemcpyDeviceToHost, stream));
+		CUDA_TRY(cudaStreamSynchronize(stream));
+		g_d2hBytes += (long long)(sizeof(int) * hProd.size());
+		int perSM = 0;
+		if (mixed) { if constexpr (sizeof(T) == 8) CUDA_TRY(cudaOccupancyMaxActiveBlocksPerMultiprocessor(&perSM, schur3::k_schur_dyn<double, float>, schur3::WARPS * 32, 0)); }
+		else CUDA_TRY(cudaOccupancyMaxActiveBlocksPerMultiprocessor(&perSM, schur3::k_schur_dyn<T, T>, schur3::WARPS * 32, 0));
+		dynGrid = std::max(1, std::min(numSMs * std::max(perSM, 1), (nblk + schur3::WARPS - 1) / schur3::WARPS));
+		for (int k = 0; k < nblk; k++) order[k] = k;
+		int maxCount = 0;
+		for (int k = 0; k < nblk; k++) maxCount = std::max(maxCount, hProd[k + 1] - hProd[k]);
+		dynHeavyFirst = 2.0 * maxCount * dynGrid * schur3::WARPS >= (double)hProd[nblk];
+		if (dynHeavyFirst)
+			std::stable_sort(order.begin(), order.end(), [&](int x, int y) { return hProd[x + 1] - hProd[x] > hProd[y + 1] - hProd[y]; });
+		CUDA_TRY(dynOrder.upload(order.data(), order.size(), stream));
+		CUDA_TRY(dynCounter.alloc(1));
+		CUDA_TRY(cudaStreamSynchronize(stream));
+		return CUBA_OK;
+	}
+
+	int setup_schur6()
+	{
+		using namespace sgpu;
+		const int nh = S.nhplLocal, numP = S.numP, nblk = S.nblk, N = (int)S.nmulLocal, eL = S.eLocal;
+		DBuf<unsigned int> key, keyS;
+		DBuf<int> val, pos, rowBlk;
+		CUDA_TRY(key.alloc(nh)); CUDA_TRY(keyS.alloc(nh)); CUDA_TRY(val.alloc(nh)); CUDA_TRY(pos.alloc(nh));
+		CUDA_TRY(rowHplPtr.alloc((size_t)numP + 1)); CUDA_TRY(rowHpl.alloc(nh)); CUDA_TRY(rowLm.alloc(nh)); CUDA_TRY(prodIloc.alloc((size_t)N)); CUDA_TRY(rowBlk.alloc((size_t)numP + 1));
+		KLAUNCH(k_hpl_row_keys, eL, e_ip.p, e_hpl.p, eL, key.p, val.p);
+		int rc = sortPairs(key.p, keyS.p, val.p, rowHpl.p, nh, bits_for((unsigned long long)numP)); if (rc) return rc;
+		KLAUNCH(k_ptr_from_u32, numP + 1, keyS.p, nh, numP, rowHplPtr.p);
+		KLAUNCH(k_hpl_row_pos, nh, keyS.p, rowHpl.p, rowHplPtr.p, hplLm.p, nh, pos.p, rowLm.p);
+		KLAUNCH(k_prod_iloc, N, prodI.p, pos.p, N, prodIloc.p);
+		KLAUNCH(k_rowptr_from_rows, numP + 1, blkRow.p, nblk, numP, rowBlk.p);
+		std::vector<int> hRowHpl((size_t)numP + 1), hRowBlk((size_t)numP + 1), hProd((size_t)nblk + 1);
+		CUDA_TRY(cudaMemcpyAsync(hRowHpl.data(), rowHplPtr.p, sizeof(int) * hRowHpl.size(), cudaMemcpyDeviceToHost, stream));
+		CUDA_TRY(cudaMemcpyAsync(hRowBlk.data(), rowBlk.p, sizeof(int) * hRowBlk.size(), cudaMemcpyDeviceToHost, stream));
+		CUDA_TRY(cudaMemcpyAsync(hProd.data(), prodPtr.p, sizeof(int) * hProd.size(), cudaMemcpyDeviceToHost, stream));
+		CUDA_TRY(cudaStreamSynchronize(stream));
+		g_d2hBytes += (long long)(sizeof(int) * (2 * ((size_t)numP + 1) + (size_t)nblk + 1));
+		int smemSM = 0, smemRes = 0, smemOptin = 0;
+		CUDA_TRY(cudaDeviceGetAttribute(&smemSM, cudaDevAttrMaxSharedMemoryPerMultiprocessor, devOrdinal));
+		CUDA_TRY(cudaDeviceGetAttribute(&smemRes, cudaDevAttrReservedSharedMemoryPerBlock, devOrdinal));
+		CUDA_TRY(cudaDeviceGetAttribute(&smemOptin, cudaDevAttrMaxSharedMemoryPerBlockOptin, devOrdinal));
+		const int per = schur6::staged_bytes<T>(), fixed = (int)sizeof(schur6::Smem<T>);
+		const int budget = std::min(smemSM / schur6::MIN_CTAS - smemRes, smemOptin) - fixed;
+		int maxRow = 0;
+		for (int a = 0; a < numP; a++) maxRow = std::max(maxRow, hRowHpl[a + 1] - hRowHpl[a]);
+		s6Cap = std::max(0, std::min(maxRow, budget / per));
+		s6Smem = (size_t)s6Cap * per;
+		const long long total = hProd[nblk];
+		const long long target = std::max(2048LL, total / std::max(1, numSMs * schur6::MIN_CTAS * 4));
+		std::vector<int4> items;
+		items.reserve((size_t)numP + 64);
+		s6Fallback = 0;
+		for (int a = 0; a < numP; a++) {
+			const int kb0 = hRowBlk[a], kb1 = hRowBlk[a + 1];
+			const int staged = hRowHpl[a + 1] - hRowHpl[a] <= s6Cap ? 1 : 0;
+			s6Fallback += 1 - staged;
+			const long long P = hProd[kb1] - hProd[kb0];
+			const long long pieces = std::min<long long>((P + target - 1) / target, kb1 - kb0);
+			int k = kb0;
+			for (long long q = 1; q <= pieces; q++) {
+				const long long end = hProd[kb0] + P * q / pieces;
+				int k2 = k + 1;
+				while (k2 < kb1 && hProd[k2] < end) k2++;
+				if (q == pieces) k2 = kb1;
+				items.push_back(make_int4(a, k, k2, staged));
+				k = k2;
+				if (k >= kb1) break;
+			}
+		}
+		s6Items = (int)items.size();
+		CUDA_TRY(s6Work.upload(items.data(), items.size(), stream));
+		if constexpr (sizeof(T) == 8) {
+			if (mixed) CUDA_TRY(cudaFuncSetAttribute(schur6::k_schur_rows<double, float>, cudaFuncAttributeMaxDynamicSharedMemorySize, (int)s6Smem));
+		}
+		if (!mixed) CUDA_TRY(cudaFuncSetAttribute(schur6::k_schur_rows<T, T>, cudaFuncAttributeMaxDynamicSharedMemorySize, (int)s6Smem));
+		CUDA_TRY(cudaStreamSynchronize(stream));
 		return CUBA_OK;
 	}
 
@@ -2327,6 +2452,17 @@
 		if (oinv && (rc = download(invHll, 9 * (size_t)S.numL, oinv))) return rc;
 		return CUBA_OK;
 	}
+	int dbg_schur_rows(int32_t* oRowHplPtr, int32_t* oRowHpl, int32_t* oProdIloc, int32_t* info) override
+	{
+		if (!haveProblem) return fail(CUBA_ERR_STATE, "no problem");
+		if (info) { info[0] = useSchur6 ? 1 : 0; info[1] = s6Cap; info[2] = s6Fallback; info[3] = s6Items; info[4] = useSchur6 ? (int)S.nmulLocal : 0; }
+		if (!useSchur6) return CUBA_OK;
+		if (oRowHplPtr) CUDA_TRY(cudaMemcpyAsync(oRowHplPtr, rowHplPtr.p, sizeof(int) * ((size_t)S.numP + 1), cudaMemcpyDeviceToHost, stream));
+		if (oRowHpl) CUDA_TRY(cudaMemcpyAsync(oRowHpl, rowHpl.p, sizeof(int) * (size_t)S.nhplLocal, cudaMemcpyDeviceToHost, stream));
+		if (oProdIloc) CUDA_TRY(cudaMemcpyAsync(oProdIloc, prodIloc.p, sizeof(int) * (size_t)S.nmulLocal, cudaMemcpyDeviceToHost, stream));
+		CUDA_TRY(cudaStreamSynchronize(stream));
+		return CUBA_OK;
+	}
 	int dbg_delta(double* oxp, double* oxl) override
 	{
 		if (!haveProblem) return fail(CUBA_ERR_STATE, "no problem");
@@ -2686,6 +2822,7 @@
 int cuba_debug_get_hsc_structure(cuba_engine* e, int32_t* rowPtr, int32_t* colInd) { ENGINE_OR_FAIL(e); return e->impl->dbg_hsc_structure(rowPtr, colInd); }
 int cuba_debug_get_system(cuba_engine* e, double* Hpp, double* bp, double* Hll, double* bl, double* Hpl) { ENGINE_OR_FAIL(e); return e->impl->dbg_system(Hpp, bp, Hll, bl, Hpl); }
 int cuba_debug_get_schur(cuba_engine* e, double* Hsc, double* bsc, double* invHll) { ENGINE_OR_FAIL(e); return e->impl->dbg_schur(Hsc, bsc, invHll); }
+int cuba_debug_get_schur_rows(cuba_engine* e, int32_t* rowHplPtr, int32_t* rowHpl, int32_t* prodIloc, int32_t* info) { ENGINE_OR_FAIL(e); return e->impl->dbg_schur_rows(rowHplPtr, rowHpl, prodIloc, info); }
 int cuba_debug_get_delta(cuba_engine* e, double* xp, double* xl) { ENGINE_OR_FAIL(e); return e->impl->dbg_delta(xp, xl); }
 int cuba_debug_get_pcg_info(cuba_engine* e, int32_t* info, double* coarse_lambda) { ENGINE_OR_FAIL(e); return e->impl->dbg_pcg_info(info, coarse_lambda); }
 int cuba_debug_get_coarse(cuba_engine* e, int32_t* aggRow, double* AcP, float* AcInv) { ENGINE_OR_FAIL(e); return e->impl->dbg_coarse(aggRow, AcP, AcInv); }
diff --git a/cuda-bundle-adjustment_b200/csrc/cuba_schur6.cuh b/cuda-bundle-adjustment_b200/csrc/cuba_schur6.cuh
--- /dev/null
+++ b/cuda-bundle-adjustment_b200/csrc/cuba_schur6.cuh
@@ -0,0 +1,253 @@
+#pragma once
+
+#include "cuba_kernels.cuh"
+
+namespace cuba_b200 {
+namespace schur6 {
+
+constexpr int WARPS = 8;
+constexpr int SLOTS = 5;
+constexpr int MIN_CTAS = 2;
+
+template <typename T> struct Smem { T red[WARPS][SLOTS][6][8]; int next; };
+template <typename T> constexpr int staged_bytes() { return 18 * (int)sizeof(T) + (int)sizeof(int); }
+
+template <typename T, typename TH = T>
+struct Args {
+	const TH* Hpl; const T* invHll; const T* bl; const T* Hpp; const T* bp;
+	const int* prodPtr; const int* prodIloc; const int* prodJ;
+	const int* rowHplPtr; const int* rowHpl; const int* rowLm;
+	const int4* work;
+	const int* blkCol; const int* u2f; const int* u2fT;
+	int cap;
+	T lambda;
+	int addDiag;
+	T* fVal; T* bsc;
+};
+
+template <typename T, typename TH>
+__device__ __forceinline__ void w_row(const TH* __restrict__ Hpl, const T* __restrict__ invHll, int i, int l, int r, T& w0, T& w1, T& w2)
+{
+	const TH* Ai = Hpl + HplStride<T, TH>::value * (size_t)i;
+	const T* iv = invHll + 9 * (size_t)l;
+	const T a0 = ldh<T, TH>(Ai + r), a1 = ldh<T, TH>(Ai + 6 + r), a2 = ldh<T, TH>(Ai + 12 + r);
+	const T i0 = __ldg(iv), i1 = __ldg(iv + 3), i2 = __ldg(iv + 6), i3 = __ldg(iv + 4), i4 = __ldg(iv + 7), i5 = __ldg(iv + 8);
+	w0 = a0 * i0 + a1 * i1 + a2 * i2;
+	w1 = a0 * i1 + a1 * i3 + a2 * i4;
+	w2 = a0 * i2 + a1 * i4 + a2 * i5;
+}
+
+template <typename T, typename TH>
+__device__ __forceinline__ void load_b(const Args<T, TH>& a, int j, T (&B)[18])
+{
+	const TH* Aj = a.Hpl + HplStride<T, TH>::value * (size_t)j;
+#pragma unroll
+	for (int x = 0; x < 18; x += 2) ldh2<T, TH>(Aj + x, B[x], B[x + 1]);
+}
+
+template <typename T, typename TH = T>
+__global__ void __launch_bounds__(WARPS * 32, MIN_CTAS) k_schur_rows(const Args<T, TH> a)
+{
+	extern __shared__ __align__(16) unsigned char s_dyn[];
+	__shared__ Smem<T> s;
+	T* sW = reinterpret_cast<T*>(s_dyn);
+	int* sL = reinterpret_cast<int*>(sW + 18 * (size_t)a.cap);
+	const int4 w = a.work[blockIdx.x];
+	const int row = w.x, k1 = w.z;
+	const bool staged = w.w != 0;
+	const int h0 = a.rowHplPtr[row], nh = a.rowHplPtr[row + 1] - h0;
+	if (staged) {
+		constexpr int U = 4;
+		for (int e0 = threadIdx.x; e0 < 6 * nh; e0 += U * WARPS * 32) {
+			int ib[U], il[U];
+#pragma unroll
+			for (int u = 0; u < U; u++) {
+				const int e = e0 + u * WARPS * 32, b = e / 6;
+				ib[u] = -1; il[u] = 0;
+				if (e < 6 * nh) { ib[u] = a.rowHpl[h0 + b]; il[u] = a.rowLm[h0 + b]; }
+			}
+#pragma unroll
+			for (int u = 0; u < U; u++) {
+				const int e = e0 + u * WARPS * 32, b = e / 6, r = e - 6 * b;
+				if (ib[u] >= 0) {
+					T w0, w1, w2;
+					w_row(a.Hpl, a.invHll, ib[u], il[u], r, w0, w1, w2);
+					sW[18 * b + r] = w0; sW[18 * b + 6 + r] = w1; sW[18 * b + 12 + r] = w2;
+					if (r == 0) sL[b] = il[u];
+				}
+			}
+		}
+	}
+	if (threadIdx.x == 0) s.next = w.y + WARPS;
+	__syncthreads();
+
+	const int lane = threadIdx.x & 31, wid = threadIdx.x >> 5;
+	const int slot = lane / 6, r = lane - 6 * slot;
+	const bool worker = slot < SLOTS;
+	for (int k = w.y + wid; k < k1; ) {
+		const bool diag = a.blkCol[k] == row;
+		const int n0 = a.prodPtr[k], n1 = a.prodPtr[k + 1];
+		T C[6], vr = T(0);
+#pragma unroll
+		for (int c = 0; c < 6; c++) C[c] = T(0);
+		int n = n0 + slot;
+		int ci = -1, cj = -1, pi = -1, pj = -1, gi = 0, gl = 0;
+		if (worker && n < n1) { ci = a.prodIloc[n]; cj = a.prodJ[n]; }
+		if (worker && n + SLOTS < n1) { pi = a.prodIloc[n + SLOTS]; pj = a.prodJ[n + SLOTS]; }
+		T B[18];
+		if (worker && n < n1 && ci >= 0) {
+			load_b(a, cj, B);
+			if (!staged) { gi = a.rowHpl[h0 + ci]; gl = a.rowLm[h0 + ci]; }
+		}
+		for (; n0 < n1; ) {
+			const bool have = worker && n < n1 && ci >= 0;
+			const int nn = n + SLOTS;
+			T Bn[18];
+			int gin = 0, gln = 0;
+			if (worker && nn < n1 && pi >= 0) {
+				load_b(a, pj, Bn);
+				if (!staged) { gin = a.rowHpl[h0 + pi]; gln = a.rowLm[h0 + pi]; }
+			}
+			int qi = -1, qj = -1;
+			if (worker && nn + SLOTS < n1) { qi = a.prodIloc[nn + SLOTS]; qj = a.prodJ[nn + SLOTS]; }
+			if (have) {
+				T w0, w1, w2;
+				int cl;
+				if (staged) {
+					const T* Wi = sW + 18 * ci;
+					w0 = Wi[r]; w1 = Wi[6 + r]; w2 = Wi[12 + r];
+					cl = sL[ci];
+				} else {
+					cl = gl;
+					w_row(a.Hpl, a.invHll, gi, gl, r, w0, w1, w2);
+				}
+#pragma unroll
+				for (int c = 0; c < 6; c++) C[c] += w0 * B[c] + w1 * B[6 + c] + w2 * B[12 + c];
+				if (diag) {
+					const T* b3 = a.bl + 3 * (size_t)cl;
+					vr += w0 * __ldg(b3) + w1 * __ldg(b3 + 1) + w2 * __ldg(b3 + 2);
+				}
+			}
+			n = nn; ci = pi; cj = pj; pi = qi; pj = qj; gi = gin; gl = gln;
+#pragma unroll
+			for (int x = 0; x < 18; x++) B[x] = Bn[x];
+			if (__all_sync(0xffffffffu, !(worker && n < n1))) break;
+		}
+		if (worker) {
+#pragma unroll
+			for (int c = 0; c < 6; c++) s.red[wid][slot][r][c] = C[c];
+			s.red[wid][slot][r][6] = vr;
+		}
+		__syncwarp();
+		for (int e = lane; e < 42; e += 32) {
+			const int c = e < 36 ? e / 6 : 6, rr = e < 36 ? e - 6 * c : e - 36;
+			T sum = T(0);
+#pragma unroll
+			for (int q = 0; q < SLOTS; q++) sum += s.red[wid][q][rr][c];
+			if (e < 36) {
+				T val = -sum;
+				if (diag && a.addDiag) val += a.Hpp[36 * (size_t)row + e] + (rr == c ? a.lambda : T(0));
+				a.fVal[36 * (size_t)a.u2f[k] + e] = val;
+				if (!diag) a.fVal[36 * (size_t)a.u2fT[k] + rr * 6 + c] = val;
+			} else if (diag) {
+				a.bsc[6 * (size_t)row + rr] = (a.addDiag ? a.bp[6 * (size_t)row + rr] : T(0)) - sum;
+			}
+		}
+		__syncwarp();
+		int nk = 0;
+		if (lane == 0) nk = atomicAdd(&s.next, 1);
+		k = __shfl_sync(0xffffffffu, nk, 0);
+	}
+}
+
+}
+}
+
+namespace cuba_b200 {
+namespace schur3 {
+
+template <typename T, typename TH>
+__device__ __forceinline__ void schur3_block(const Args<T, TH>& a, int k, int lane, T (&red)[SLOTS][6][8])
+{
+	const int ra = a.blkRow[k], cb = a.blkCol[k];
+	const bool diag = ra == cb;
+	const int n0 = a.prodPtr[k], n1 = a.prodPtr[k + 1];
+	const int slot = lane / 6, r = lane - 6 * slot;
+	const bool worker = slot < SLOTS;
+	T C[6], vr = T(0);
+#pragma unroll
+	for (int c = 0; c < 6; c++) C[c] = T(0);
+
+	int n = n0 + slot;
+	int pi = -1, pj = -1, pl = -1;
+	if (worker && n < n1) { pi = a.prodI[n]; pj = a.prodJ[n]; pl = a.prodL[n]; }
+	for (; n0 < n1; ) {
+		const int ci = pi, cj = pj, cl = pl;
+		const bool have = worker && n < n1 && ci >= 0;
+		const int nn = n + SLOTS;
+		pi = -1; pj = -1; pl = -1;
+		if (worker && nn < n1) { pi = a.prodI[nn]; pj = a.prodJ[nn]; pl = a.prodL[nn]; }
+		if (have) {
+			const TH* Ai = a.Hpl + HplStride<T, TH>::value * (size_t)ci;
+			const TH* Aj = a.Hpl + HplStride<T, TH>::value * (size_t)cj;
+			const T* iv = a.invHll + 9 * (size_t)cl;
+			const T a0 = ldh<T, TH>(Ai + r), a1 = ldh<T, TH>(Ai + 6 + r), a2 = ldh<T, TH>(Ai + 12 + r);
+			const T i0 = __ldg(iv), i1 = __ldg(iv + 3), i2 = __ldg(iv + 6), i3 = __ldg(iv + 4), i4 = __ldg(iv + 7), i5 = __ldg(iv + 8);
+			T B[18];
+#pragma unroll
+			for (int x = 0; x < 18; x += 2) ldh2<T, TH>(Aj + x, B[x], B[x + 1]);
+			const T w0 = a0 * i0 + a1 * i1 + a2 * i2;
+			const T w1 = a0 * i1 + a1 * i3 + a2 * i4;
+			const T w2 = a0 * i2 + a1 * i4 + a2 * i5;
+#pragma unroll
+			for (int c = 0; c < 6; c++) C[c] += w0 * B[c] + w1 * B[6 + c] + w2 * B[12 + c];
+			if (diag) {
+				const T* b3 = a.bl + 3 * (size_t)cl;
+				vr += w0 * __ldg(b3) + w1 * __ldg(b3 + 1) + w2 * __ldg(b3 + 2);
+			}
+		}
+		n = nn;
+		if (__all_sync(0xffffffffu, !(worker && n < n1))) break;
+	}
+	if (worker) {
+#pragma unroll
+		for (int c = 0; c < 6; c++) red[slot][r][c] = C[c];
+		red[slot][r][6] = vr;
+	}
+	__syncwarp();
+	for (int e = lane; e < 42; e += 32) {
+		const int c = e < 36 ? e / 6 : 6, rr = e < 36 ? e - 6 * c : e - 36;
+		T s = T(0);
+#pragma unroll
+		for (int q = 0; q < SLOTS; q++) s += red[q][rr][c];
+		if (e < 36) {
+			T val = -s;
+			if (diag && a.addDiag) val += a.Hpp[36 * (size_t)ra + e] + (rr == c ? a.lambda : T(0));
+			if (a.uVal) a.uVal[36 * (size_t)k + e] = val;
+			else {
+				a.fVal[36 * (size_t)a.u2f[k] + e] = val;
+				if (!diag) a.fVal[36 * (size_t)a.u2fT[k] + rr * 6 + c] = val;
+			}
+		} else if (diag) {
+			a.bsc[6 * (size_t)ra + rr] = (a.addDiag ? a.bp[6 * (size_t)ra + rr] : T(0)) - s;
+		}
+	}
+}
+
+template <typename T, typename TH = T>
+__global__ void __launch_bounds__(WARPS * 32, 3) k_schur_dyn(const Args<T, TH> a, const int* __restrict__ order, int* __restrict__ counter)
+{
+	__shared__ T s_red[WARPS][SLOTS][6][8];
+	const int lane = threadIdx.x & 31, wid = threadIdx.x >> 5;
+	const int first = gridDim.x * WARPS;
+	for (int t = blockIdx.x * WARPS + wid; t < a.nblk; ) {
+		schur3_block(a, order[t], lane, s_red[wid]);
+		__syncwarp();
+		int nt = 0;
+		if (lane == 0) nt = first + atomicAdd(counter, 1);
+		t = __shfl_sync(0xffffffffu, nt, 0);
+	}
+}
+
+}
+}
diff --git a/cuda-bundle-adjustment_b200/csrc/cuba_structure_gpu.cuh b/cuda-bundle-adjustment_b200/csrc/cuba_structure_gpu.cuh
--- a/cuda-bundle-adjustment_b200/csrc/cuba_structure_gpu.cuh
+++ b/cuda-bundle-adjustment_b200/csrc/cuba_structure_gpu.cuh
@@ -263,6 +263,32 @@
 	rowPtr[a] = lo;
 }
 
+__global__ void k_hpl_row_keys(const int* __restrict__ e_ip, const int* __restrict__ e_hpl, int eLocal, unsigned int* key, int* val)
+{
+	const int e = blockIdx.x * blockDim.x + threadIdx.x;
+	if (e >= eLocal) return;
+	const int h = e_hpl[e];
+	if (h >= 0) { key[h] = (unsigned)(e_ip[e] & 0x7fffffff); val[h] = h; }
+}
+
+__global__ void k_hpl_row_pos(const unsigned int* __restrict__ rowS, const int* __restrict__ rowHpl, const int* __restrict__ rowHplPtr,
+	const int* __restrict__ hplLm, int nhpl, int* pos, int* rowLm)
+{
+	const int p = blockIdx.x * blockDim.x + threadIdx.x;
+	if (p >= nhpl) return;
+	const int i = rowHpl[p];
+	pos[i] = p - rowHplPtr[rowS[p]];
+	rowLm[p] = hplLm[i];
+}
+
+__global__ void k_prod_iloc(const int* __restrict__ prodI, const int* __restrict__ pos, int n, int* prodIloc)
+{
+	const int k = blockIdx.x * blockDim.x + threadIdx.x;
+	if (k >= n) return;
+	const int i = prodI[k];
+	prodIloc[k] = i >= 0 ? pos[i] : -1;
+}
+
 __global__ void k_full_entries(const int* __restrict__ blkRow, const int* __restrict__ blkCol, int nblk, int numP, unsigned long long* key, int* val)
 {
 	const int k = blockIdx.x * blockDim.x + threadIdx.x;
diff --git a/include/cuba_b200.h b/include/cuba_b200.h
--- a/include/cuba_b200.h
+++ b/include/cuba_b200.h
@@ -184,6 +184,7 @@
 int cuba_debug_get_system(cuba_engine* e, double* Hpp , double* bp , double* Hll ,
 	double* bl , double* Hpl );
 int cuba_debug_get_schur(cuba_engine* e, double* Hsc , double* bsc , double* invHll );
+int cuba_debug_get_schur_rows(cuba_engine* e, int32_t* rowHplPtr, int32_t* rowHpl, int32_t* prodIloc, int32_t* info);
 int cuba_debug_get_delta(cuba_engine* e, double* xp , double* xl );
 
 #define CUBA_PCG_INFO_LEN 16
```

Result: faster. 251.6 million (median of 6 runs) (+2.4%).
